# dalek-cryptography/zkp

Hardware: AMD Instinct MI355X
Metric: proofs/sec + batch-verifies/sec, CMZ13 10-attr credential, 1/2/4/8 MI355X (higher is better)
Workload: dtype u32x9 (29-bit limbs, u64 accumulate)

## Files before the change

### include/zkp_mi355x.h

```cpp
#ifndef ZKP_MI355X_H
#define ZKP_MI355X_H

#include <stddef.h>
#include <stdint.h>

#ifdef __cplusplus
extern "C" {
#endif

#define ZKP_OK 0
#define ZKP_ERR_HIP (-1)
#define ZKP_ERR_ARG (-2)
#define ZKP_ERR_NO_DEVICE (-3)
#define ZKP_ERR_OOM (-4)

#define ZKP_VARTIME 0
#define ZKP_CT 1

typedef struct zkp_ctx zkp_ctx;

int zkp_ctx_create(zkp_ctx** out, int device_id);
void zkp_ctx_destroy(zkp_ctx* ctx);
int zkp_ctx_set_stream(zkp_ctx* ctx, void* hip_stream);
int zkp_ctx_synchronize(zkp_ctx* ctx);
// ... 93 lines not shown
                                 uint8_t* d_transcripts, const uint8_t* d_table, const uint8_t* d_challenges,
                                 const uint8_t* d_responses, uint8_t* d_results);
int zkp_fused_batch_verify_dev(zkp_ctx* ctx, const zkp_fused_statement* st, uint32_t N, uint32_t strobe_pos,
                               uint8_t* d_transcripts, uint8_t* d_points, const uint8_t* d_commitments,
                               const uint8_t* d_responses, const uint8_t* d_weights16, uint8_t* d_out_point,
                               uint32_t* d_status);
int zkp_fused_verify_batchable_dev(zkp_ctx* ctx, const zkp_fused_statement* st, uint32_t N, uint32_t strobe_pos,
                                   uint8_t* d_transcripts, const uint8_t* d_table, const uint8_t* d_responses,
                                   const uint8_t* d_weights16, uint8_t* d_results);

int zkp_fused_batch_verify_many_dev(zkp_ctx* ctx, const zkp_fused_statement* st, uint32_t n_batches, uint32_t N_each, uint32_t strobe_pos,
                                    uint8_t* d_transcripts, uint8_t* d_points, const uint8_t* d_commitments, const uint8_t* d_responses,
                                    const uint8_t* d_weights16, uint8_t* d_out_points, uint32_t* d_status);

#define ZKP_JOB_SHARED_TRANSCRIPT 1u
int zkp_fused_prove_submit(zkp_ctx* ctx, const zkp_fused_statement* st, uint32_t N, uint32_t flags, const uint8_t* transcripts,
                           const uint8_t* secrets, const uint8_t* inst, uint32_t inst_stride, const uint8_t* common,
                           const uint8_t* entropy, const uint8_t* rng_seed , uint8_t* transcripts_out,
                           uint8_t* challenges, uint8_t* responses, uint8_t* commitments, int* invalid_point);
int zkp_fused_verify_compact_submit(zkp_ctx* ctx, const zkp_fused_statement* st, uint32_t N, uint32_t flags, const uint8_t* transcripts,
                                    const uint8_t* inst, uint32_t inst_stride, const uint8_t* common, const uint8_t* challenges,
                                    const uint8_t* responses, uint8_t* transcripts_out, uint8_t* results );
int zkp_fused_batch_verify_many_submit(zkp_ctx* ctx, const zkp_fused_statement* st, uint32_t n_batches, uint32_t N_each, uint32_t flags,
                                       const uint8_t* transcripts, const uint8_t* inst, uint32_t inst_stride, const uint8_t* common,
                                       const uint8_t* commitments, const uint8_t* responses, const uint8_t* weights16,
                                       uint32_t weights_stride, const uint8_t* rng_seed, uint8_t* transcripts_out, int* verdicts );
int zkp_fused_verify_batchable_submit(zkp_ctx* ctx, const zkp_fused_statement* st, uint32_t N, uint32_t flags, const uint8_t* transcripts,
                                      const uint8_t* inst, uint32_t inst_stride, const uint8_t* common, const uint8_t* commitments,
                                      const uint8_t* responses, const uint8_t* weights16 , const uint8_t* rng_seed,
                                      uint8_t* transcripts_out, uint8_t* results );
int zkp_ctx_job_wait(zkp_ctx* ctx);
int zkp_ctx_job_poll(zkp_ctx* ctx);
int zkp_ctx_job_pending(zkp_ctx* ctx);
int zkp_ctx_job_discard(zkp_ctx* ctx);
int zkp_ctx_job_timing(zkp_ctx* ctx, float ms[3]);

int zkp_host_alloc(void** out, size_t bytes);
int zkp_host_alloc_on(void** out, size_t bytes, int device);
int zkp_host_numa_node(int device);
int zkp_host_node_of(const void* p);
void zkp_host_free(void* p);
int zkp_host_register(void* p, size_t bytes);
int zkp_host_unregister(void* p);
int zkp_host_is_pinned(const void* p);

int zkp_chacha20_fill_dev(zkp_ctx* ctx, const uint8_t key[32], uint64_t nonce, uint64_t first_block, uint8_t* d_out, size_t bytes);

int zkp_decode_check(zkp_ctx* ctx, uint64_t n, const uint8_t* points , uint8_t* status ,
                     uint8_t* xyzt );

int zkp_encode_many(zkp_ctx* ctx, uint64_t n, const uint8_t* xyzt , uint8_t* out );

int zkp_from_uniform_bytes(zkp_ctx* ctx, uint64_t n, const uint8_t* in , uint8_t* out );
int zkp_from_uniform_bytes_dev(zkp_ctx* ctx, uint64_t n, const uint8_t* d_in , uint8_t* d_out );
int zkp_fused_hash_to_group(zkp_ctx* ctx, uint32_t N, uint8_t* transcripts , const char* label, uint8_t* out );
int zkp_fused_hash_to_group_ragged(zkp_ctx* ctx, uint32_t N, uint8_t* transcripts , const char* label, uint8_t* out );
int zkp_hash_from_bytes_sha512(zkp_ctx* ctx, uint64_t n, const uint8_t* msgs, const uint64_t* offsets , uint8_t* out );
int zkp_hash_from_bytes_sha512_dev(zkp_ctx* ctx, uint64_t n, const uint8_t* d_msgs, uint64_t msgs_len, const uint64_t* d_offsets ,
                                   uint8_t* d_out );

enum {
  ZKP_K_DECODE = 0,
  ZKP_K_TERMS = 1,
  ZKP_K_REDUCE = 2,
  ZKP_K_SORT = 3,
  ZKP_K_BUCKET = 4,
  ZKP_K_COMBINE = 5,
  ZKP_K_TRANSCRIPT = 6,
  ZKP_K_SCALARS = 7,
  ZKP_K_TABLES = 8,
  ZKP_K_COUNT = 9
};
int zkp_ctx_last_timing(zkp_ctx* ctx, float* kernel_ms , float* total_ms);
int zkp_ctx_last_kernels(zkp_ctx* ctx, int kind, char* buf, size_t cap);
int zkp_ctx_set_profiling(zkp_ctx* ctx, int enabled);

#ifdef ZKP_BUILD_TEST_HOOKS
int zkp_debug_quad_selftest(zkp_ctx* ctx, uint32_t n, const uint8_t* pairs , uint8_t* out );
int zkp_debug_row_selftest(zkp_ctx* ctx, uint32_t n, const uint8_t* pairs , uint8_t* out );
int zkp_debug_wave_cycles(zkp_ctx* ctx, uint64_t* out, uint32_t cap);
int zkp_debug_sha512(zkp_ctx* ctx, uint64_t n, const uint8_t* msgs, const uint64_t* offsets , uint8_t* out );
int zkp_debug_last_schedule(zkp_ctx* ctx, char* buf, size_t cap);
int zkp_debug_ragged_blocks(const uint8_t* transcripts, uint32_t N, uint32_t* idx, uint32_t* blocks, uint32_t cap);
enum { ZKP_TESTOPT_DUMMY_LAUNCHES = 1001, ZKP_TESTOPT_GENERIC_CLASSIFIER = 1002, ZKP_TESTOPT_WAVE_CYCLES = 1003 };
#endif

#ifdef __cplusplus
}
#endif
#endif
```

### zkp_amd/csrc/comb_tables.h

```cpp
#pragma once
#include "quad.h"
#include "stmt_pairs.h"

namespace zkp {

template <int TEETH>
struct comb_cfg {
  static_assert(TEETH == 4 || TEETH == 8 || TEETH == 16 || TEETH == 32, "teeth");
  static constexpr int BITS = 256 / TEETH;
  static constexpr int WINDOWS = BITS / 4;
  static constexpr int ENTRIES = 8 * TEETH + 1;
};
constexpr int comb_entries(int teeth) { return 8 * teeth + 1; }
constexpr int LADDER_ENTRIES = 8;

__device__ __forceinline__ void q_store_cached(dev_ext* dst, const qcached& c, int q) {
  uint32_t* w = reinterpret_cast<uint32_t*>(dst) + 9 * q;
#pragma unroll
  for (int i = 0; i < 9; ++i) w[i] = c.c.v[i];
}

__global__ void __launch_bounds__(256)
k_comb_slots(uint32_t n_points, const uint32_t* __restrict__ uses, uint32_t comb_min, uint32_t group_min, uint32_t max_tables,
             uint32_t* __restrict__ counter, uint32_t* __restrict__ slot_of, uint32_t* __restrict__ slot_pt, uint32_t* __restrict__ group_start,
// ... 151 lines not shown
                                              const dev_affine* __restrict__ pts, dev_ext* __restrict__ comb, uint32_t* hand) {
  using cfg = comb_cfg<TEETH>;
  const uint32_t wave = threadIdx.x >> 6, lane = threadIdx.x & 63u;
  const uint32_t ns = min(*n_slots, max_tables);
  const uint32_t slot = slot0 + lane;
  const bool have = slot < ns && !(slot_pt[slot < ns ? slot : 0u] & STMT_ABSORBED);
  dev_ext* tbl = comb + (size_t)(have ? slot : 0u) * cfg::ENTRIES;
  if (wave == 0) {
    ge_p3 base;
    ge_identity(base);
    if (have) load_affine(base, pts + slot_pt[slot]);
#pragma unroll 1
    for (int j = 0; j < TEETH; ++j) {
      uint32_t* h = hand + (j & 1) * 36 * 64 + lane;
#pragma unroll
      for (int i = 0; i < 9; ++i) { h[64 * i] = base.X.v[i]; h[64 * (9 + i)] = base.Y.v[i]; h[64 * (18 + i)] = base.Z.v[i]; h[64 * (27 + i)] = base.T.v[i]; }
      __syncthreads();
#pragma unroll 1
      for (int d = 0; d < cfg::BITS - 1; ++d) ge_double<false>(base, base);
      ge_double<true>(base, base);
    }
    if (have) {
      ge_cached c;
      ge_to_cached(c, base);
      store_comb_entry(tbl + 8 * TEETH, c);
    }
  } else {
#pragma unroll 1
    for (int j = 0; j < TEETH; ++j) {
      __syncthreads();
      const uint32_t* h = hand + (j & 1) * 36 * 64 + lane;
      ge_p3 base, m2, m3, m4, m;
#pragma unroll
      for (int i = 0; i < 9; ++i) { base.X.v[i] = h[64 * i]; base.Y.v[i] = h[64 * (9 + i)]; base.Z.v[i] = h[64 * (18 + i)]; base.T.v[i] = h[64 * (27 + i)]; }
      FE_TRACK(fe_set_ub_tight(base.X); fe_set_ub_tight(base.Y); fe_set_ub_tight(base.Z); fe_set_ub_tight(base.T));
      ge_cached c1, c;
      ge_to_cached(c1, base);
      ge_double<true>(m2, base);
      ge_add_cached(m3, m2, c1);
      ge_double<true>(m4, m2);
      if (have) {
        store_comb_entry(tbl + 8 * j + 0, c1);
        ge_to_cached(c, m2); store_comb_entry(tbl + 8 * j + 1, c);
        ge_to_cached(c, m3); store_comb_entry(tbl + 8 * j + 2, c);
        ge_to_cached(c, m4); store_comb_entry(tbl + 8 * j + 3, c);
      }
      ge_add_cached(m, m4, c1);
      if (have) { ge_to_cached(c, m); store_comb_entry(tbl + 8 * j + 4, c); }
      ge_double<true>(m, m3);
      if (have) { ge_to_cached(c, m); store_comb_entry(tbl + 8 * j + 5, c); }
      ge_add_cached(m, m, c1);
      if (have) { ge_to_cached(c, m); store_comb_entry(tbl + 8 * j + 6, c); }
      ge_double<true>(m, m4);
      if (have) { ge_to_cached(c, m); store_comb_entry(tbl + 8 * j + 7, c); }
    }
  }
}

__device__ __forceinline__ void load_comb_entry(ge_cached& c, const dev_ext* src) {
  uint32_t w[36];
  load_vec<9>(w, src);
  fe_set(c.YmX, w); fe_set(c.YpX, w + 9); fe_set(c.Z2, w + 18); fe_set(c.T2d, w + 27);
}

template <bool CT>
__device__ __forceinline__ void comb_select(ge_cached& sel, const dev_ext* __restrict__ row, uint32_t mag) {
  ge_cached_identity(sel);
  if (CT) {
#pragma unroll 1
    for (uint32_t h = 0; h < 4; ++h) {
      ge_cached c0, c1;
      load_comb_entry(c0, row + 2 * h + 0);
      load_comb_entry(c1, row + 2 * h + 1);
      ge_cached_cmov(sel, c0, (uint32_t)(mag == 2 * h + 1));
      ge_cached_cmov(sel, c1, (uint32_t)(mag == 2 * h + 2));
    }
  } else if (mag) {
    load_comb_entry(sel, row + (mag - 1));
  }
}

template <bool CT, int TEETH>
__device__ __forceinline__ void term_comb(uint32_t t, const uint8_t* __restrict__ scalars, const dev_ext* __restrict__ tbl,
                                          dev_ext* __restrict__ partial, uint32_t* ecol) {
  using cfg = comb_cfg<TEETH>;
  uint32_t s[8], e[8], top;
  load_vec<2>(s, scalars + 32 * (size_t)t);
  sc_add_pattern(e, top, s, 0x88888888u);
#pragma unroll
  for (int j = 0; j < 8; ++j) ecol[256 * j] = e[j];
  ge_p3 acc;
  ge_identity(acc);
  if (CT) {
    ge_cached n0, n1;
    load_comb_entry(n0, tbl + 0);
    load_comb_entry(n1, tbl + 1);
#pragma unroll 1
    for (int w = cfg::WINDOWS - 1; w >= 0; --w) {
      if (w != cfg::WINDOWS - 1) {
        ge_double4_flat(acc);
      }
#pragma unroll 1
      for (int j = 0; j < TEETH; ++j) {
        const int nidx = j * cfg::WINDOWS + w;
        const uint32_t nib = (ecol[256 * (nidx >> 3)] >> (4 * (nidx & 7))) & 15u;
        const uint32_t neg = (uint32_t)(nib < 8u);
        const uint32_t mag = neg ? 8u - nib : nib - 8u;
        const dev_ext* row = tbl + 8 * j;
        ge_cached sel;
        ge_cached_identity(sel);
        ge_cached_cmov(sel, n0, (uint32_t)(mag == 1));
        ge_cached_cmov(sel, n1, (uint32_t)(mag == 2));
#pragma unroll 1
        for (uint32_t h = 1; h < 4; ++h) {
          ge_cached c0, c1;
          load_comb_entry(c0, row + 2 * h + 0);
          load_comb_entry(c1, row + 2 * h + 1);
          ge_cached_cmov(sel, c0, (uint32_t)(mag == 2 * h + 1));
          ge_cached_cmov(sel, c1, (uint32_t)(mag == 2 * h + 2));
        }
        const dev_ext* next = (j + 1 < TEETH) ? row + 8 : tbl;
        load_comb_entry(n0, next + 0);
        load_comb_entry(n1, next + 1);
        ge_cached_cneg(sel, neg);
        ge_add_cached(acc, acc, sel);
      }
    }
  } else {
#pragma unroll 1
    for (int w = cfg::WINDOWS - 1; w >= 0; --w) {
      if (w != cfg::WINDOWS - 1) {
        ge_double4(acc);
      }
#pragma unroll 1
      for (int j = 0; j < TEETH; ++j) {
        const int nidx = j * cfg::WINDOWS + w;
        const uint32_t nib = (ecol[256 * (nidx >> 3)] >> (4 * (nidx & 7))) & 15u;
        const uint32_t neg = (uint32_t)(nib < 8u);
        const uint32_t mag = neg ? 8u - nib : nib - 8u;
        ge_cached sel;
        comb_select<false>(sel, tbl + 8 * j, mag);
        ge_cached_cneg(sel, neg);
        ge_add_cached(acc, acc, sel);
      }
    }
  }
  {
    ge_cached sel, c;
    ge_cached_identity(sel);
    load_comb_entry(c, tbl + 8 * TEETH);
    ge_cached_cmov(sel, c, top);
    ge_add_cached(acc, acc, sel);
  }
  store_ext(partial + t, acc);
}

__device__ __forceinline__ void ge_p3_dpp_from(ge_p3& r, const ge_p3& a, int ctrl_sel) {
  if (ctrl_sel == 0) { fe_dpp<ZKP_QP(1, 1, 3, 3)>(r.X, a.X); fe_dpp<ZKP_QP(1, 1, 3, 3)>(r.Y, a.Y); fe_dpp<ZKP_QP(1, 1, 3, 3)>(r.Z, a.Z); fe_dpp<ZKP_QP(1, 1, 3, 3)>(r.T, a.T); }
  else { fe_dpp<ZKP_QP(2, 2, 2, 2)>(r.X, a.X); fe_dpp<ZKP_QP(2, 2, 2, 2)>(r.Y, a.Y); fe_dpp<ZKP_QP(2, 2, 2, 2)>(r.Z, a.Z); fe_dpp<ZKP_QP(2, 2, 2, 2)>(r.T, a.T); }
}
template <int TEETH>
__device__ __forceinline__ void term_comb_split4(uint32_t t, uint32_t q, const uint8_t* __restrict__ scalars, const dev_ext* __restrict__ comb, uint32_t slot,
                                                 dev_ext* __restrict__ partial, uint32_t* ecol) {
  using cfg = comb_cfg<TEETH>;
  static_assert(cfg::WINDOWS == 4, "one lane of the quad per window");
  typedef __attribute__((address_space(3))) volatile uint32_t lds_word;
  lds_word* stash = (lds_word*)(ecol + 256 * 8);
  stash[0] = slot;
  stash[256] = t;
  const dev_ext* __restrict__ tbl = comb + (size_t)slot * cfg::ENTRIES;
  uint32_t s[8], e[8], top;
  load_vec<2>(s, scalars + 32 * (size_t)t);
  sc_add_pattern(e, top, s, 0x88888888u);
#pragma unroll
  for (int j = 0; j < 8; ++j) ecol[256 * j] = e[j];
  stash[512] = top;
  ge_p3 acc;
  ge_identity(acc);
  {
    ge_cached n0, n1;
    load_comb_entry(n0, tbl + 0);
    load_comb_entry(n1, tbl + 1);
#pragma unroll 1
    for (int j = 0; j < TEETH; ++j) {
      const uint32_t nidx = (uint32_t)j * cfg::WINDOWS + q;
      const uint32_t nib = (ecol[256 * (nidx >> 3)] >> (4 * (nidx & 7))) & 15u;
      const uint32_t neg = (uint32_t)(nib < 8u);
      const uint32_t mag = neg ? 8u - nib : nib - 8u;
      const dev_ext* row = tbl + 8 * j;
      ge_cached sel;
      ge_cached_identity(sel);
      ge_cached_cmov(sel, n0, (uint32_t)(mag == 1));
      ge_cached_cmov(sel, n1, (uint32_t)(mag == 2));
#pragma unroll 1
      for (uint32_t h = 1; h < 4; ++h) {
        ge_cached c0, c1;
        load_comb_entry(c0, row + 2 * h + 0);
        load_comb_entry(c1, row + 2 * h + 1);
        ge_cached_cmov(sel, c0, (uint32_t)(mag == 2 * h + 1));
        ge_cached_cmov(sel, c1, (uint32_t)(mag == 2 * h + 2));
      }
      const dev_ext* next = (j + 1 < TEETH) ? row + 8 : tbl;
      load_comb_entry(n0, next + 0);
      load_comb_entry(n1, next + 1);
      ge_cached_cneg(sel, neg);
      ge_add_cached(acc, acc, sel);
    }
  }
  {
    ge_p3 d = acc;
    ge_double4(d);
    fe_pick(acc.X, d.X, (q & 1u) != 0); fe_pick(acc.Y, d.Y, (q & 1u) != 0); fe_pick(acc.Z, d.Z, (q & 1u) != 0); fe_pick(acc.T, d.T, (q & 1u) != 0);
    ge_p3 o;
    ge_p3_dpp_from(o, acc, 0);
    ge_cached c;
    ge_to_cached(c, o);
    ge_add_cached(d, acc, c);
    fe_pick(acc.X, d.X, (q & 1u) == 0); fe_pick(acc.Y, d.Y, (q & 1u) == 0); fe_pick(acc.Z, d.Z, (q & 1u) == 0); fe_pick(acc.T, d.T, (q & 1u) == 0);
    d = acc;
    ge_double4(d);
    ge_double4(d);
    fe_pick(acc.X, d.X, q == 2u); fe_pick(acc.Y, d.Y, q == 2u); fe_pick(acc.Z, d.Z, q == 2u); fe_pick(acc.T, d.T, q == 2u);
    ge_p3_dpp_from(o, acc, 1);
    ge_to_cached(c, o);
    ge_add_cached(d, acc, c);
    fe_pick(acc.X, d.X, q == 0u); fe_pick(acc.Y, d.Y, q == 0u); fe_pick(acc.Z, d.Z, q == 0u); fe_pick(acc.T, d.T, q == 0u);
  }
  {
    ge_cached sel, c;
    ge_cached_identity(sel);
    load_comb_entry(c, comb + (size_t)stash[0] * cfg::ENTRIES + 8 * TEETH);
    ge_cached_cmov(sel, c, stash[512]);
    ge_add_cached(acc, acc, sel);
  }
  if (q == 0u) store_ext(partial + stash[256], acc);
}

constexpr int GROUP_RUNS = 3, GROUP_ROW_CHUNKS = 8 * 9, GROUP_IDENT_ROW = GROUP_RUNS * GROUP_ROW_CHUNKS, GROUP_CHUNK_ROWS = GROUP_IDENT_ROW + 9;
constexpr int GROUP_LDS_UINT4 = GROUP_CHUNK_ROWS * 16 + (256 + 16 * GROUP_RUNS) / 4;
static_assert(GROUP_MIN_USES >= 8, "a column of 16 consecutive grouped terms must span at most GROUP_RUNS points");

__device__ __forceinline__ void comb_group_block(uint32_t i0, uint32_t n_g, const uint32_t* __restrict__ list_g, const uint8_t* __restrict__ scalars,
                                                 const uint32_t* __restrict__ pidx, const uint32_t* __restrict__ slot_of,
                                                 const dev_ext* __restrict__ comb, dev_ext* __restrict__ partial, uint4* lds) {
  using cfg = comb_cfg<16>;
  constexpr uint32_t NONE = 0xffffffffu;
  const uint32_t tid = threadIdx.x, col = tid & 15u, k = tid >> 4;
  const uint32_t i = i0 + col * 16 + k;
  const bool listed = i < n_g;
  uint32_t t = 0, slot = NONE;
  if (listed) { t = list_g[i]; slot = slot_of[pidx[t]]; }
  uint32_t* slots = reinterpret_cast<uint32_t*>(lds + GROUP_CHUNK_ROWS * 16);
  uint32_t* colslot = slots + 256;
  slots[k * 16 + col] = slot;
  if (k < (uint32_t)GROUP_RUNS) colslot[col * GROUP_RUNS + k] = NONE;
  if (k < 9) {
    uint32_t w[36];
#pragma unroll
    for (int q = 0; q < 36; ++q) w[q] = (q == 0 || q == 9) ? 1u : (q == 18 ? 2u : 0u);
    uint4 v = make_uint4(0, 0, 0, 0);
#pragma unroll
    for (int q = 0; q < 9; ++q) if (k == (uint32_t)q) v = make_uint4(w[4 * q], w[4 * q + 1], w[4 * q + 2], w[4 * q + 3]);
    lds[(GROUP_IDENT_ROW + k) * 16 + col] = v;
  }
  __syncthreads();
  uint32_t run = 0;
  bool first = true;
#pragma unroll
  for (uint32_t kk = 1; kk < 16; ++kk) {
    const bool change = slots[kk * 16 + col] != slots[(kk - 1) * 16 + col];
    if (kk <= k) { run += change ? 1u : 0u; if (kk == k) first = change; }
  }
  if (first && run < (uint32_t)GROUP_RUNS) colslot[col * GROUP_RUNS + run] = slot;
  __syncthreads();
  const bool live = listed && slot != NONE && run < (uint32_t)GROUP_RUNS;
  const uint4* src[GROUP_RUNS];
  bool have[GROUP_RUNS];
#pragma unroll
  for (int r = 0; r < GROUP_RUNS; ++r) {
    const uint32_t sr = colslot[col * GROUP_RUNS + r];
    have[r] = sr != NONE;
    src[r] = reinterpret_cast<const uint4*>(comb + (size_t)(have[r] ? sr : 0u) * cfg::ENTRIES) + k;
  }
  const bool tail = k < (uint32_t)(GROUP_ROW_CHUNKS - 64);
  typedef __attribute__((address_space(1))) const void* gptr_t;
  typedef __attribute__((address_space(3))) void* lptr_t;
  const uint32_t wave = (uint32_t)__builtin_amdgcn_readfirstlane((int)(tid >> 6));
  auto issue = [&](uint32_t row) {
#pragma unroll
    for (int r = 0; r < GROUP_RUNS; ++r) {
      const uint4* p = src[r] + (size_t)row * GROUP_ROW_CHUNKS;
      uint4* d = lds + (size_t)(r * GROUP_ROW_CHUNKS + 4 * wave) * 16;
#pragma unroll
      for (int m = 0; m < 4; ++m)
        if (have[r]) __builtin_amdgcn_global_load_lds((gptr_t)(p + 16 * m), (lptr_t)(d + 16 * 16 * m), 16, 0, 0);
      if (have[r] && tail) __builtin_amdgcn_global_load_lds((gptr_t)(p + 64), (lptr_t)(d + 16 * 64), 16, 0, 0);
    }
  };
  uint32_t dlo[cfg::WINDOWS], dhi[cfg::WINDOWS], top = 0;
  {
    uint32_t sc[8], e[8];
#pragma unroll
    for (int q = 0; q < 8; ++q) sc[q] = 0;
    if (live) load_vec<2>(sc, scalars + 32 * (size_t)t);
    sc_add_pattern(e, top, sc, 0x88888888u);
#pragma unroll
    for (int w = 0; w < cfg::WINDOWS; ++w) {
      uint32_t lo = 0, hi = 0;
#pragma unroll
      for (int m = 0; m < 4; ++m) {
        lo |= (((e[m] >> (4 * w)) & 0xfu) | ((e[m] >> (12 + 4 * w)) & 0xf0u)) << (8 * m);
        hi |= (((e[m + 4] >> (4 * w)) & 0xfu) | ((e[m + 4] >> (12 + 4 * w)) & 0xf0u)) << (8 * m);
      }
      dlo[w] = lo; dhi[w] = hi;
    }
  }
  ge_p3 acc, lo;
  ge_identity(acc);
  ge_identity(lo);
  issue(0);
  auto pick = [&](uint32_t& c0, uint32_t& c1, ge_cached& sel, uint32_t& neg) {
    const uint32_t nib = c0 & 15u;
    c0 = __builtin_amdgcn_alignbit(c1, c0, 4);
    c1 >>= 4;
    neg = (uint32_t)(nib < 8u);
    const uint32_t mag = neg ? 8u - nib : nib - 8u;
    const uint32_t row = mag ? run * GROUP_ROW_CHUNKS + (mag - 1u) * 9u : (uint32_t)GROUP_IDENT_ROW;
    const uint4* ent = lds + (size_t)row * 16 + col;
    uint32_t wd[36];
#pragma unroll
    for (int q = 0; q < 9; ++q) {
      const uint4 x = ent[q * 16];
      wd[4 * q + 0] = x.x; wd[4 * q + 1] = x.y; wd[4 * q + 2] = x.z; wd[4 * q + 3] = x.w;
    }
    fe_set(sel.YmX, wd); fe_set(sel.YpX, wd + 9); fe_set(sel.Z2, wd + 18); fe_set(sel.T2d, wd + 27);
  };
#pragma unroll 1
  for (int pass = 0; pass < 2; ++pass) {
    if (live && pass) { ge_double4(acc); ge_double4(lo); }
    uint32_t alo = pass ? dlo[2] : dlo[3], ahi = pass ? dhi[2] : dhi[3];
    uint32_t blo = pass ? dlo[0] : dlo[1], bhi = pass ? dhi[0] : dhi[1];
#pragma unroll 1
    for (int j = 0; j < 16; ++j) {
      asm volatile("s_waitcnt vmcnt(0)\n\ts_barrier" ::: "memory");
      ge_cached sel;
      uint32_t neg = 0;
      if (live) {
        pick(alo, ahi, sel, neg);
        ge_cached_cneg(sel, neg);
        ge_add_cached(acc, acc, sel);
        pick(blo, bhi, sel, neg);
      }
      lds_barrier();
      if (pass == 0 || j != 15) issue((uint32_t)((j + 1) & 15));
      if (live) {
        ge_cached_cneg(sel, neg);
        ge_add_cached(lo, lo, sel);
      }
    }
  }
  if (live) {
    ge_double4(acc);
    ge_double4(acc);
    ge_cached c;
    ge_to_cached(c, lo);
    ge_add_cached(acc, acc, c);
  }
  if (live) {
    ge_cached sel, c;
    ge_cached_identity(sel);
    load_comb_entry(c, comb + (size_t)slot * cfg::ENTRIES + 8 * 16);
    ge_cached_cmov(sel, c, top);
    ge_add_cached(acc, acc, sel);
    store_ext(partial + t, acc);
  }
}

constexpr uint32_t XBAR_RUNS = 8;
constexpr uint32_t XBAR_HALF_TERMS = 31, XBAR_WAVE_TERMS = 2 * XBAR_HALF_TERMS, XBAR_BLOCK_TERMS = 4 * XBAR_WAVE_TERMS;
constexpr int XBAR_WAVE_UINT4 = 9 * 64;
constexpr int XBAR_LDS_UINT4 = 4 * XBAR_WAVE_UINT4;
static_assert(2 + (XBAR_WAVE_TERMS - 2) / GROUP_MIN_USES <= XBAR_RUNS, "a wavefront's consecutive grouped terms must span at most XBAR_RUNS points");
static_assert(2 + (XBAR_HALF_TERMS - 2) / GROUP_MIN_USES <= 4 && XBAR_HALF_TERMS <= 32,
              "the terms of one crossbar service group (a half of the wavefront) must span at most 4 points: sources 32 lanes apart never meet");

__device__ __forceinline__ void comb_group_xbar(uint32_t i0, uint32_t n_g, const uint32_t* __restrict__ list_g, const uint8_t* __restrict__ scalars,
                                                const uint32_t* __restrict__ pidx, const uint32_t* __restrict__ slot_of,
                                                const dev_ext* __restrict__ comb, dev_ext* __restrict__ partial, uint4* lds) {
  using cfg = comb_cfg<16>;
  constexpr uint32_t NONE = 0xffffffffu;
  const uint32_t tid = threadIdx.x, lane = tid & 63u;
  const uint32_t wave = (uint32_t)__builtin_amdgcn_readfirstlane((int)(tid >> 6));
  if (i0 + wave * XBAR_WAVE_TERMS >= n_g) return;
  const uint32_t hl = lane & 31u;
  const uint32_t i = i0 + wave * XBAR_WAVE_TERMS + (lane >> 5) * XBAR_HALF_TERMS + hl;
  const bool listed = hl < XBAR_HALF_TERMS && i < n_g;
  uint32_t t = 0, slot = NONE;
  if (listed) { t = list_g[i]; slot = slot_of[pidx[t]]; }
  uint32_t cur = slot;
  const uint32_t left = (uint32_t)__shfl_up((int)cur, 1);
  if (hl == 31u) cur = left;
  const uint32_t before = (uint32_t)__shfl_up((int)cur, 1);
  const bool change = lane == 0u || (listed && slot != before);
  const uint64_t cm = __ballot(change);
  const uint32_t run = (uint32_t)__popcll(cm & ((2ull << lane) - 1ull)) - 1u;
  const bool live = listed && slot != NONE && run < XBAR_RUNS;
  int first = -1;
  {
    uint64_t mm = cm;
#pragma unroll
    for (uint32_t r = 0; r < XBAR_RUNS; ++r) {
      const int f = mm ? (int)__ffsll((long long)mm) - 1 : -1;
      if ((lane >> 3) == r) first = f;
      mm &= mm - 1ull;
    }
  }
  uint32_t hslot = (uint32_t)__shfl((int)slot, first < 0 ? 0 : first);
  if (first < 0) hslot = NONE;
  const bool have = hslot != NONE;
  const uint4* hsrc = reinterpret_cast<const uint4*>(comb + (size_t)(have ? hslot : 0u) * cfg::ENTRIES + (lane & 7u));
  typedef __attribute__((address_space(1))) const void* gptr_t;
  typedef __attribute__((address_space(3))) void* lptr_t;
  uint4* wlds = lds + (size_t)wave * XBAR_WAVE_UINT4;
  const uint4* mine = wlds + lane;
  auto issue = [&](uint32_t row) {
    const uint4* p = hsrc + (size_t)row * (8 * 9);
    if (have) {
#pragma unroll
      for (int q = 0; q < 9; ++q) __builtin_amdgcn_global_load_lds((gptr_t)(p + q), (lptr_t)(wlds + 64 * q), 16, 0, 0);
    }
  };
  uint32_t dlo[cfg::WINDOWS], dhi[cfg::WINDOWS], top = 0;
  {
    uint32_t sc[8], e[8];
#pragma unroll
    for (int q = 0; q < 8; ++q) sc[q] = 0;
    if (live) load_vec<2>(sc, scalars + 32 * (size_t)t);
    sc_add_pattern(e, top, sc, 0x88888888u);
#pragma unroll
    for (int w = 0; w < cfg::WINDOWS; ++w) {
      uint32_t lo = 0, hi = 0;
#pragma unroll
      for (int m = 0; m < 4; ++m) {
        lo |= (((e[m] >> (4 * w)) & 0xfu) | ((e[m] >> (12 + 4 * w)) & 0xf0u)) << (8 * m);
        hi |= (((e[m + 4] >> (4 * w)) & 0xfu) | ((e[m + 4] >> (12 + 4 * w)) & 0xf0u)) << (8 * m);
      }
      dlo[w] = lo; dhi[w] = hi;
    }
  }
  ge_p3 acc, lo;
  ge_identity(acc);
  ge_identity(lo);
  issue(0);
  const uint32_t run8 = (run & (XBAR_RUNS - 1u)) * 8u;
  auto pick = [&](uint32_t& c0, uint32_t& c1, ge_cached& sel, uint32_t& neg) {
    const uint32_t nib = c0 & 15u;
    c0 = __builtin_amdgcn_alignbit(c1, c0, 4);
    c1 >>= 4;
    neg = (uint32_t)(nib < 8u);
    const uint32_t mag = neg ? 8u - nib : nib - 8u;
    const uint32_t nz = (uint32_t)(mag != 0u);
    const int src = (int)((run8 + mag - nz) << 2);
    uint32_t wd[36];
#pragma unroll
    for (int q = 0; q < 9; ++q) {
      const uint4 x = mine[q * 64];
      wd[4 * q + 0] = xbar_fetch(src, x.x); wd[4 * q + 1] = xbar_fetch(src, x.y);
      wd[4 * q + 2] = xbar_fetch(src, x.z); wd[4 * q + 3] = xbar_fetch(src, x.w);
    }
    const uint32_t m = 0u - nz, id = nz ^ 1u;
#pragma unroll
    for (int q = 0; q < 36; ++q) wd[q] &= m;
    wd[0] |= id; wd[9] |= id; wd[18] |= id << 1;
    fe_set(sel.YmX, wd); fe_set(sel.YpX, wd + 9); fe_set(sel.Z2, wd + 18); fe_set(sel.T2d, wd + 27);
  };
#pragma unroll 1
  for (int pass = 0; pass < 2; ++pass) {
    if (pass) { ge_double4(acc); ge_double4(lo); }
    uint32_t alo = pass ? dlo[2] : dlo[3], ahi = pass ? dhi[2] : dhi[3];
    uint32_t blo = pass ? dlo[0] : dlo[1], bhi = pass ? dhi[0] : dhi[1];
#pragma unroll 1
    for (int j = 0; j < 16; ++j) {
      asm volatile("s_waitcnt vmcnt(0)" ::: "memory");
      ge_cached sel;
      uint32_t neg = 0;
      pick(alo, ahi, sel, neg);
      ge_cached_cneg(sel, neg);
      ge_add_cached(acc, acc, sel);
      pick(blo, bhi, sel, neg);
      asm volatile("s_waitcnt lgkmcnt(0)" ::: "memory");
      if (pass == 0 || j != 15) issue((uint32_t)((j + 1) & 15));
      ge_cached_cneg(sel, neg);
      ge_add_cached(lo, lo, sel);
    }
  }
  ge_double4(acc);
  ge_double4(acc);
  {
    ge_cached c;
    ge_to_cached(c, lo);
    ge_add_cached(acc, acc, c);
  }
  if (live) {
    ge_cached sel, c;
    ge_cached_identity(sel);
    load_comb_entry(c, comb + (size_t)slot * cfg::ENTRIES + 8 * 16);
    ge_cached_cmov(sel, c, top);
    ge_add_cached(acc, acc, sel);
    store_ext(partial + t, acc);
  }
}

constexpr uint32_t LADDER_GROUP_UINT4 = 64u * LADDER_ENTRIES * 9u;
__device__ __forceinline__ void ladder_store_entry(uint4* __restrict__ g, int e, const ge_cached& c) {
  uint32_t w[36];
  fe_get(w, c.YmX); fe_get(w + 9, c.YpX); fe_get(w + 18, c.Z2); fe_get(w + 27, c.T2d);
#pragma unroll
  for (int q = 0; q < 9; ++q) g[(9 * e + q) * 64] = make_uint4(w[4 * q], w[4 * q + 1], w[4 * q + 2], w[4 * q + 3]);
}
__device__ __forceinline__ void ladder_load_entry(ge_cached& c, const uint4* __restrict__ g, uint32_t e) {
  uint32_t w[36];
#pragma unroll
  for (int q = 0; q < 9; ++q) {
    const uint4 v = g[(9u * e + (uint32_t)q) * 64u];
    w[4 * q] = v.x; w[4 * q + 1] = v.y; w[4 * q + 2] = v.z; w[4 * q + 3] = v.w;
  }
  fe_set(c.YmX, w); fe_set(c.YpX, w + 9); fe_set(c.Z2, w + 18); fe_set(c.T2d, w + 27);
}
template <bool CT>
__device__ __forceinline__ void ladder_select(ge_cached& sel, const uint4* __restrict__ g, uint32_t mag) {
  ge_cached_identity(sel);
  if (CT) {
#pragma unroll 1
    for (uint32_t h = 0; h < 4; ++h) {
      ge_cached c0, c1;
      ladder_load_entry(c0, g, 2 * h + 0);
      ladder_load_entry(c1, g, 2 * h + 1);
      ge_cached_cmov(sel, c0, (uint32_t)(mag == 2 * h + 1));
      ge_cached_cmov(sel, c1, (uint32_t)(mag == 2 * h + 2));
    }
  } else if (mag) {
    ladder_load_entry(sel, g, mag - 1);
  }
}

template <bool CT>
__device__ __forceinline__ void term_ladder16(uint32_t t, const uint8_t* __restrict__ scalars, const dev_affine* __restrict__ pt,
                                              uint4* __restrict__ tbl , dev_ext* __restrict__ partial, uint32_t* ecol) {
  uint32_t s[8], e[8], top;
  load_vec<2>(s, scalars + 32 * (size_t)t);
  sc_add_pattern(e, top, s, 0x88888888u);
#pragma unroll
  for (int j = 0; j < 8; ++j) ecol[256 * j] = e[j];
  ge_p3 acc;
  {
    ge_p3 P, m2, m3, m4, m;
    ge_cached c1, c;
    load_affine(P, pt);
    ge_to_cached(c1, P);
    ladder_store_entry(tbl, 0, c1);
    ge_double<true>(m2, P);
    ge_to_cached(c, m2); ladder_store_entry(tbl, 1, c);
    ge_add_cached(m3, m2, c1);
    ge_to_cached(c, m3); ladder_store_entry(tbl, 2, c);
    ge_double<true>(m4, m2);
    ge_to_cached(c, m4); ladder_store_entry(tbl, 3, c);
    ge_add_cached(m, m4, c1);
    ge_to_cached(c, m); ladder_store_entry(tbl, 4, c);
    ge_double<true>(m, m3);
    ge_to_cached(c, m); ladder_store_entry(tbl, 5, c);
    ge_add_cached(m, m, c1);
    ge_to_cached(c, m); ladder_store_entry(tbl, 6, c);
    ge_double<true>(m, m4);
    ge_to_cached(c, m); ladder_store_entry(tbl, 7, c);
    ge_cached sel;
    ge_cached_identity(sel);
    ge_cached_cmov(sel, c1, top);
    ge_identity(acc);
    ge_add_cached(acc, acc, sel);
  }
#pragma unroll 1
  for (int j = 7; j >= 0; --j) {
    uint32_t cur = ecol[256 * j];
#pragma unroll 1
    for (int k = 0; k < 8; ++k) {
      ge_double4(acc);
      const uint32_t nib = cur >> 28;
      cur <<= 4;
      const uint32_t neg = (uint32_t)(nib < 8u);
      const uint32_t mag = neg ? 8u - nib : nib - 8u;
      ge_cached sel;
      ladder_select<CT>(sel, tbl, mag);
      ge_cached_cneg(sel, neg);
      ge_add_cached(acc, acc, sel);
    }
  }
  store_ext(partial + t, acc);
}

__global__ void __launch_bounds__(256, 2)
k_rider_tables(const uint32_t* __restrict__ n_slots, uint32_t max_tables, const uint32_t* __restrict__ slot_pt, const dev_affine* __restrict__ pts,
               dev_ext* __restrict__ comb) {
  __shared__ uint32_t stage[4][36][64];
  __shared__ uint32_t live[4][64];
  const uint32_t wave = threadIdx.x >> 6, lane = threadIdx.x & 63u;
  const uint32_t slot = blockIdx.x * blockDim.x + threadIdx.x, ns = min(*n_slots, max_tables);
  const uint32_t pi = slot < ns ? slot_pt[slot] : 0u;
  const bool have = slot < ns && (pi & STMT_ABSORBED);
  live[wave][lane] = have ? 1u : 0u;
  if (!__ballot(have)) return;
  ge_p3 P, m;
  ge_identity(P);
  if (have) load_affine(P, pts + (pi & ~STMT_ABSORBED));
  dev_ext* tbl0 = comb + (size_t)(slot - lane) * comb_cfg<16>::ENTRIES;
  ge_cached c1, c;
  ge_to_cached(c1, P);
  c = c1;
  m = P;
#pragma unroll 1
  for (int k = 0; k < 128; ++k) {
    if (k) {
      ge_add_cached(m, m, c1);
      ge_to_cached(c, m);
    }
    store_entries_staged(stage[wave], live[wave], lane, tbl0, comb_cfg<16>::ENTRIES, (uint32_t)k, c);
  }
}

__device__ __forceinline__ void ladder_build8(uint4* __restrict__ tbl, ge_cached& c1, const dev_affine* __restrict__ pt) {
  ge_p3 P, m2, m3, m4, m;
  ge_cached c;
  load_affine(P, pt);
  ge_to_cached(c1, P);
  ladder_store_entry(tbl, 0, c1);
  ge_double<true>(m2, P);
  ge_to_cached(c, m2); ladder_store_entry(tbl, 1, c);
  ge_add_cached(m3, m2, c1);
  ge_to_cached(c, m3); ladder_store_entry(tbl, 2, c);
  ge_double<true>(m4, m2);
  ge_to_cached(c, m4); ladder_store_entry(tbl, 3, c);
  ge_add_cached(m, m4, c1);
  ge_to_cached(c, m); ladder_store_entry(tbl, 4, c);
  ge_double<true>(m, m3);
  ge_to_cached(c, m); ladder_store_entry(tbl, 5, c);
  ge_add_cached(m, m, c1);
  ge_to_cached(c, m); ladder_store_entry(tbl, 6, c);
  ge_double<true>(m, m4);
  ge_to_cached(c, m); ladder_store_entry(tbl, 7, c);
}
__device__ __forceinline__ void term_ladder16_joint(uint32_t t, uint32_t t2, const uint8_t* __restrict__ scalars, const dev_affine* __restrict__ pt,
                                                    const dev_affine* __restrict__ pt2, uint4* __restrict__ tbl, uint4* __restrict__ tbl2,
                                                    const dev_ext* __restrict__ rider, dev_ext* __restrict__ partial, uint32_t* ecol) {
  uint32_t top, top2;
  {
    uint32_t s[8], e[8];
    load_vec<2>(s, scalars + 32 * (size_t)t);
    sc_add_pattern(e, top, s, 0x88888888u);
#pragma unroll
    for (int j = 0; j < 8; ++j) ecol[256 * j] = e[j];
    load_vec<2>(s, scalars + 32 * (size_t)t2);
    sc_add_pattern(e, top2, s, rider ? 0x80808080u : 0x88888888u);
#pragma unroll
// ... 55 lines not shown
```

### zkp_amd/csrc/fe_constants.h

```cpp
#pragma once
#include "fe25519.h"
namespace zkp {
static constexpr fe_const FE_D = {{0x135978a3u, 0x0f5a6e50u, 0x10762addu, 0x00149a82u, 0x1e898007u, 0x003cbbbcu, 0x19ce331du, 0x1dc56dffu, 0x0052036cu}};
static constexpr fe_const FE_D2 = {{0x06b2f159u, 0x1eb4dca1u, 0x00ec55bau, 0x00293505u, 0x1d13000eu, 0x00797779u, 0x139c663au, 0x1b8adbffu, 0x002406d9u}};
static constexpr fe_const FE_SQRT_M1 = {{0x0a0ea0b0u, 0x0770d93au, 0x0bf91e31u, 0x06300d5au, 0x1d7a72f4u, 0x004c9efdu, 0x1c2cad34u, 0x1009f83bu, 0x002b8324u}};
static constexpr fe_const FE_INVSQRT_A_MINUS_D = {{0x005d40eau, 0x0e47ed54u, 0x105cafa6u, 0x1e2c2eb4u, 0x1d8409d2u, 0x1dc8ff00u, 0x12885b09u, 0x00b9f5ffu, 0x00786c89u}};
static constexpr fe_const FE_SQRT_AD_MINUS_ONE = {{0x097b2e1bu, 0x14bfb502u, 0x1e152f5fu, 0x1b1c1836u, 0x1d1fdaf9u, 0x1e6498fau, 0x02b03cf3u, 0x17e57069u, 0x00376931u}};
static constexpr fe_const FE_ONE_MINUS_D_SQ = {{0x145fc176u, 0x13e04e0cu, 0x178d43f8u, 0x0342719au, 0x0dfe42c8u, 0x15eedf38u, 0x035e6652u, 0x1516567cu, 0x00029072u}};
static constexpr fe_const FE_D_MINUS_ONE_SQ = {{0x04ed4d20u, 0x0d6ad552u, 0x0786664cu, 0x1c945960u, 0x14eebd29u, 0x0997a94du, 0x09053373u, 0x0f5ecd84u, 0x005968b3u}};
struct fe_words { uint32_t w[8]; };
static constexpr fe_words FE_W_ONE = {{0x00000001u, 0x00000000u, 0x00000000u, 0x00000000u, 0x00000000u, 0x00000000u, 0x00000000u, 0x00000000u}};
static constexpr fe_words FE_W_MINUS_ONE = {{0xffffffecu, 0xffffffffu, 0xffffffffu, 0xffffffffu, 0xffffffffu, 0xffffffffu, 0xffffffffu, 0x7fffffffu}};
static constexpr fe_words FE_W_MINUS_SQRT_M1 = {{0xb5f15f3du, 0x3b11e4d8u, 0x52d01b87u, 0xd0bce7f9u, 0xc2042858u, 0xd4b2ff66u, 0xb03e20f4u, 0x547cdb7fu}};
}
```

### zkp_amd/csrc/fused_flows.h

```cpp
#pragma once
#include "merlin_prog.h"
#include "transcript_kernels.h"

namespace zkp {

__global__ void __launch_bounds__(256)
k_wide_reduce(uint32_t n, const uint8_t* __restrict__ wide, uint8_t* __restrict__ out) {
  const uint32_t i = blockIdx.x * blockDim.x + threadIdx.x;
  if (i >= n) return;
  sc lo, hi, r;
  load_vec<2>(lo.v, wide + 64 * (size_t)i);
  load_vec<2>(hi.v, wide + 64 * (size_t)i + 32);
  sc_from_wide(r, lo, hi);
  store_vec<2>(out + 32 * (size_t)i, r.v);
}

__global__ void __launch_bounds__(256)
k_neg_reduce(uint32_t n, const uint8_t* in, uint8_t* out) {
  const uint32_t i = blockIdx.x * blockDim.x + threadIdx.x;
  if (i >= n) return;
  sc a, r;
  load_vec<2>(a.v, in + 32 * (size_t)i);
  sc_reduce(r, a);
  sc_neg(r, r);
// ... 204 lines not shown
  for (int i = 0; i < 9; ++i) {
    const int bit = 29 * i, wi = bit >> 5, sh = bit & 31;
    w[wi] |= t[i] << sh;
    if (sh > 3 && wi < 7) w[wi + 1] |= t[i] >> (32 - sh);
  }
}
__device__ __forceinline__ void fe_unpack256(fe& r, const uint32_t w[8]) {
#pragma unroll
  for (int i = 0; i < 9; ++i) {
    const int bit = 29 * i, wi = bit >> 5, sh = bit & 31;
    uint32_t x = w[wi] >> sh;
    if (sh > 3 && wi < 7) x |= w[wi + 1] << (32 - sh);
    r.v[i] = i == 8 ? x : (x & FE_M29);
  }
  FE_TRACK(fe_set_ub_tight(r));
}
__device__ __forceinline__ void store_straus_entry(straus_entry* dst, const ge_cached& c) {
  uint32_t w[32];
  fe_pack256(w, c.YpX); fe_pack256(w + 8, c.YmX); fe_pack256(w + 16, c.Z2); fe_pack256(w + 24, c.T2d);
  store_vec<8>(dst, w);
}
__device__ __forceinline__ void load_straus_entry(ge_cached& c, const straus_entry* src) {
  uint32_t w[32];
  load_vec<8>(w, src);
  fe_unpack256(c.YpX, w); fe_unpack256(c.YmX, w + 8); fe_unpack256(c.Z2, w + 16); fe_unpack256(c.T2d, w + 24);
}
__global__ void __launch_bounds__(256, 2)
k_straus_tables(uint32_t n_points, const dev_affine* __restrict__ pts, straus_entry* __restrict__ tab) {
  const uint32_t p = blockIdx.x * blockDim.x + threadIdx.x;
  if (p >= n_points) return;
  ge_p3 P, m2, m3, m4, m;
  ge_cached c1, c;
  load_affine(P, pts + p);
  straus_entry* t = tab + (size_t)p * 8;
  ge_to_cached(c1, P);
  store_straus_entry(t + 0, c1);
  ge_double<true>(m2, P);
  ge_to_cached(c, m2); store_straus_entry(t + 1, c);
  ge_add_cached(m3, m2, c1);
  ge_to_cached(c, m3); store_straus_entry(t + 2, c);
  ge_double<true>(m4, m2);
  ge_to_cached(c, m4); store_straus_entry(t + 3, c);
  ge_add_cached(m, m4, c1);
  ge_to_cached(c, m); store_straus_entry(t + 4, c);
  ge_double<true>(m, m3);
  ge_to_cached(c, m); store_straus_entry(t + 5, c);
  ge_add_cached(m, m, c1);
  ge_to_cached(c, m); store_straus_entry(t + 6, c);
  ge_double<true>(m, m4);
  ge_to_cached(c, m); store_straus_entry(t + 7, c);
}
__global__ void __launch_bounds__(256, 2)
k_straus_each(uint32_t N, uint32_t K, uint32_t L, uint32_t ns, uint32_t ni, uint32_t nc, const uint8_t* __restrict__ scalars ,
              const straus_entry* __restrict__ tab, uint32_t* __restrict__ digits, dev_ext* __restrict__ spart) {
  extern __shared__ uint32_t straus_lds[];
  uint32_t* col = straus_lds + threadIdx.x;
  const uint32_t g = blockIdx.x * blockDim.x + threadIdx.x;
  if (g >= N * L) return;
  const uint32_t j = g / L, l = g - j * L, np = ns + ni;
  const size_t base = (size_t)j * K;
  auto table_of = [&](uint32_t i) -> const straus_entry* {
    const size_t p = i < ns ? i : (i < np ? (size_t)ns + (size_t)(i - ns) * N + j : (size_t)ns + (size_t)ni * N + (size_t)j * nc + (i - np));
    return tab + p * 8;
  };
  ge_p3 acc;
  ge_identity(acc);
  bool started = false;
  uint64_t flipmask = 0;
  uint32_t oo = 0;
  for (uint32_t i = l; i < K; i += L, ++oo) {
    uint32_t sw[8], e[8], top;
    load_vec<2>(sw, scalars + 32 * (base + i));
    const uint32_t flip = sc_fold_sign(sw);
    sc_add_pattern(e, top, sw, 0x88888888u);
    uint32_t* d = digits + 9 * (base + i);
#pragma unroll
    for (int w = 0; w < 8; ++w) d[w] = e[w];
    d[8] = flip;
    flipmask |= (uint64_t)flip << oo;
    if (top) {
      ge_cached q;
      load_straus_entry(q, table_of(i));
      ge_cached_cneg(q, flip);
      ge_add_cached(acc, acc, q);
      started = true;
    }
  }
  ge_cached qn;
  uint32_t magn = 0, negn = 0;
  auto fetch = [&](uint32_t i, uint32_t o, int k) {
    const uint32_t nib = (col[256 * o] >> (4 * k)) & 15u;
    const uint32_t neg = (uint32_t)(nib < 8u);
    magn = neg ? 8u - nib : nib - 8u;
    negn = neg ^ (uint32_t)((flipmask >> o) & 1u);
    if (magn) load_straus_entry(qn, table_of(i) + (magn - 1));
  };
#pragma unroll 1
  for (int w = 7; w >= 0; --w) {
    uint32_t o = 0;
    for (uint32_t i = l; i < K; i += L, ++o) col[256 * o] = digits[9 * (base + i) + w];
#pragma unroll 1
    for (int k = 7; k >= 0; --k) {
      fetch(l, 0, k);
      if (started) ge_double4(acc);
      o = 0;
#pragma unroll 1
      for (uint32_t i = l; i < K; i += L, ++o) {
        ge_cached q = qn;
        const uint32_t mag = magn, neg = negn;
        if (i + L < K) fetch(i + L, o + 1, k);
        if (mag) {
          ge_cached_cneg(q, neg);
          ge_add_cached(acc, acc, q);
          started = true;
        }
      }
    }
  }
  store_ext(spart + g, acc);
}
__global__ void __launch_bounds__(256)
k_straus_recode(uint32_t NK, const uint8_t* __restrict__ scalars, uint32_t* __restrict__ digits) {
  const uint32_t g = blockIdx.x * blockDim.x + threadIdx.x;
  if (g >= NK) return;
  uint32_t sw[8], e[8], top;
  load_vec<2>(sw, scalars + 32 * (size_t)g);
  const uint32_t flip = sc_fold_sign(sw);
  sc_add_pattern(e, top, sw, 0x88888888u);
  uint32_t* d = digits + 9 * (size_t)g;
#pragma unroll
  for (int w = 0; w < 8; ++w) d[w] = e[w];
  d[8] = flip | (top << 1);
}
__global__ void __launch_bounds__(256, 2)
k_straus_each_win(uint32_t N, uint32_t K, uint32_t P, uint32_t ns, uint32_t ni, uint32_t nc, const straus_entry* __restrict__ tab,
                  const uint32_t* __restrict__ digits, dev_ext* __restrict__ spart) {
  extern __shared__ uint32_t straus_lds[];
  uint32_t* col = straus_lds + threadIdx.x;
  const uint32_t g = blockIdx.x * blockDim.x + threadIdx.x;
  if (g >= N * P) return;
  const uint32_t j = g / P, p = g - j * P, np = ns + ni, Wp = 64u / P;
  const uint32_t* dj = digits + 9 * (size_t)j * K;
  auto table_of = [&](uint32_t i) -> const straus_entry* {
    const size_t t = i < ns ? i : (i < np ? (size_t)ns + (size_t)(i - ns) * N + j : (size_t)ns + (size_t)ni * N + (size_t)j * nc + (i - np));
    return tab + t * 8;
  };
  ge_p3 acc;
  ge_identity(acc);
  bool started = false;
  uint64_t flipmask = 0;
  for (uint32_t i = 0; i < K; ++i) {
    const uint32_t f = dj[9 * i + 8];
    flipmask |= (uint64_t)(f & 1u) << i;
    if ((f >> 1) && p == P - 1) {
      ge_cached q;
      load_straus_entry(q, table_of(i));
      ge_cached_cneg(q, f & 1u);
      ge_add_cached(acc, acc, q);
      started = true;
    }
  }
  ge_cached qn;
  uint32_t magn = 0, negn = 0;
  auto fetch = [&](uint32_t i, int k) {
    const uint32_t nib = (col[256 * i] >> (4 * k)) & 15u;
    const uint32_t neg = (uint32_t)(nib < 8u);
    magn = neg ? 8u - nib : nib - 8u;
    negn = neg ^ (uint32_t)((flipmask >> i) & 1u);
    if (magn) load_straus_entry(qn, table_of(i) + (magn - 1));
  };
  const int w_hi = (int)(Wp * (p + 1)) - 1, w_lo = (int)(Wp * p);
#pragma unroll 1
  for (int w = w_hi; w >= w_lo; --w) {
    const int k = w & 7;
    if (k == 7 || w == w_hi)
      for (uint32_t i = 0; i < K; ++i) col[256 * i] = dj[9 * i + (w >> 3)];
    fetch(0, k);
    if (started) ge_double4(acc);
#pragma unroll 1
    for (uint32_t i = 0; i < K; ++i) {
      ge_cached q = qn;
      const uint32_t mag = magn, neg = negn;
      if (i + 1 < K) fetch(i + 1, k);
      if (mag) {
        ge_cached_cneg(q, neg);
        ge_add_cached(acc, acc, q);
        started = true;
      }
    }
  }
  store_ext(spart + g, acc);
}
__global__ void __launch_bounds__(256)
k_straus_combine_quad(uint32_t N, uint32_t P, const dev_ext* __restrict__ spart, dev_ext* __restrict__ out) {
  const uint32_t gt = blockIdx.x * blockDim.x + threadIdx.x, j = gt >> 2;
  const int q = (int)(gt & 3u);
  if (j >= N) return;
  const dev_ext* s = spart + (size_t)j * P;
  const uint32_t dbl = 4u * (64u / P);
  qpt acc;
  q_load_ext(acc, s + (P - 1), q);
#pragma unroll 1
  for (int p = (int)P - 2; p >= 0; --p) {
#pragma unroll 1
    for (uint32_t d = 0; d < dbl; ++d) q_double(acc, acc, q);
    qpt t;
    q_load_ext(t, s + p, q);
    q_add(acc, acc, t, q);
  }
  q_store_ext(out + j, acc, q);
}
__global__ void __launch_bounds__(256, 2)
k_straus_finish(uint32_t N, uint32_t K, uint32_t L, const uint32_t* __restrict__ pidx, const dev_affine* __restrict__ pts, const dev_ext* __restrict__ spart,
                uint8_t* __restrict__ out, uint8_t* __restrict__ status8) {
  const uint32_t j = blockIdx.x * blockDim.x + threadIdx.x;
  if (j >= N) return;
  ge_p3 acc;
  load_ext(acc, spart + (size_t)j * L);
  for (uint32_t l = 1; l < L; ++l) {
    ge_p3 q;
    load_ext(q, spart + (size_t)j * L + l);
    ge_add_p3(acc, acc, q);
  }
  uint32_t bad = 0;
  for (uint32_t i = 0; i < K; ++i) bad |= pts[pidx[(size_t)j * K + i]].valid ^ 1u;
  uint32_t w[8];
#pragma unroll
  for (int k = 0; k < 8; ++k) w[k] = 0;
  if (!bad) w[0] = (fe_iszero(acc.X) | fe_iszero(acc.Y)) ^ 1u;
  store_vec<2>(out + 32 * (size_t)j, w);
  status8[j] = (uint8_t)bad;
}

__global__ void __launch_bounds__(256)
k_batch_after_transcript(uint32_t N, uint32_t N_each, uint32_t nc, uint32_t m, const uint32_t* __restrict__ failed, uint32_t* __restrict__ any, uint32_t any_stride,
                         uint32_t any_bit, const uint8_t* __restrict__ wchal, uint8_t* __restrict__ minus_c, const uint8_t* __restrict__ coms,
                         uint8_t* __restrict__ rows, const uint8_t* __restrict__ responses) {
  const size_t g = (size_t)blockIdx.x * blockDim.x + threadIdx.x;
  if (g < N) {
    if (failed[g]) atomicOr(any + (g / N_each) * any_stride, any_bit);
    sc lo, hi, r;
    load_vec<2>(lo.v, wchal + 64 * g);
    load_vec<2>(hi.v, wchal + 64 * g + 32);
    sc_from_wide(r, lo, hi);
    sc_neg(r, r);
    store_vec<2>(minus_c + 32 * g, r.v);
  }
  if (coms && g < (size_t)N * nc) {
    const size_t j = g / nc, k = g % nc;
    uint32_t w[8];
    load_vec<2>(w, coms + 32 * g);
    store_vec<2>(rows + 32 * (k * N + j), w);
  }
  if (g < (size_t)N * m) {
    uint32_t w[8];
    load_vec<2>(w, responses + 32 * g);
    if (sc_not_canonical(w)) atomicOr(any + ((g / m) / N_each) * any_stride, any_bit);
  }
}

__global__ void k_any_nonzero(uint32_t n, const uint32_t* __restrict__ flags, uint32_t* __restrict__ any) {
  const uint32_t i = blockIdx.x * blockDim.x + threadIdx.x;
  if (i < n && flags[i]) *any = 1;
}

}

namespace {
using namespace zkp;
// ... 468 lines not shown
  c->prof_suspended = false;
  c->stream = main;
  HIP_TRY(hipEventRecord(c->ev_join, c->side_stream));
  return ZKP_OK;
}
int side_join(zkp_ctx* c, bool overlap) {
  if (side_forks(c, overlap)) HIP_TRY(hipStreamWaitEvent(c->stream, c->ev_join, 0));
  return ZKP_OK;
}

struct ws_view {
  char* base;
  uint8_t* u8(size_t o) const { return reinterpret_cast<uint8_t*>(base + o); }
  uint32_t* u32(size_t o) const { return reinterpret_cast<uint32_t*>(base + o); }
};

struct prove_inter { size_t saved, failed, wide, blind, off, sc, pidx, wchal, img, end; };
prove_inter prove_carve(const fused_plan& pl, size_t start) {
  const size_t N = pl.N, m = pl.s.m, nc = pl.s.nc, T = pl.T1;
  carve cv;
  cv.off = start;
  prove_inter o;
  o.saved = cv.take(N * 25 * 8);
  o.failed = cv.take(N * 4 + 4);
  o.wide = cv.take(N * m * 64 + 64);
  o.blind = cv.take(N * m * 32 + 32);
  o.off = cv.take((N * nc + 1) * 4);
  o.sc = cv.take(N * T * 32 + 32);
  o.pidx = cv.take(N * T * 4 + 4);
  o.wchal = cv.take(N * 64 + 64);
  o.img = cv.take(pl.img_bytes);
  o.end = cv.off;
  return o;
}
terms_cfg prove_terms_cfg(const zkp_ctx* c, const fused_plan& pl, bool throughput) {
  return cfg_from_terms(pl.tpt.data(), pl.T1, pl.s.ns, pl.s.np, pl.N, c->ct_comb_min(throughput, (size_t)pl.N * pl.T1));
}
int prove_core(zkp_ctx* c, const fused_plan& pl, const prove_inter& o, size_t ws_bound, uint8_t* d_ts, const uint8_t* d_sec, const uint8_t* d_tbl,
               const uint8_t* d_ent, uint8_t* d_chal, uint8_t* d_resp, uint8_t* d_coms, uint8_t* d_st8, bool overlap, bool throughput,
               const std::function<int()>* late_inputs = nullptr, const std::function<int()>* early_outputs = nullptr, bool late_early = false) {
  const uint32_t N = pl.N, m = pl.s.m, nc = pl.s.nc, T = pl.T1, n_points = pl.s.ns + pl.s.ni * N;
  const ws_view w{static_cast<char*>(c->ws)};
  tr_bufs hb{};
  hb.src[SRC_TABLE] = d_tbl; hb.src[SRC_SECRETS] = d_sec; hb.src[SRC_ENTROPY] = d_ent; hb.src[SRC_COMS] = d_coms;
  hb.dst[DST_WIDE] = w.u8(o.wide); hb.dst[DST_CHAL] = w.u8(o.wchal);
  uint64_t* d_saved = reinterpret_cast<uint64_t*>(w.base + o.saved);
  prof_begin(c);
  const size_t lanes = std::max<size_t>((size_t)N * T, (size_t)N * nc) + 1;
  terms_cfg tk = prove_terms_cfg(c, pl, throughput);
  if (o.end + terms_path_ws(n_points, N * T, N * nc, tk) > ws_bound)
    return fail(ZKP_ERR_ARG, "internal: prove_core's term path does not fit the workspace its caller sized");
  tk.throughput = throughput;
  if (pl.d_order) { tk.map.N = N; tk.map.nc = nc; tk.map.order = pl.d_order; }
  tk.stmt.toff = pl.d_tarr; tk.stmt.tpt = pl.d_tarr + nc + 1 + T; tk.stmt.N = N; tk.stmt.T = T; tk.stmt.nc = nc; tk.stmt.ns = pl.s.ns; tk.stmt.np = pl.s.np;
  tk.stmt.off = w.u32(o.off); tk.stmt.pidx = w.u32(o.pidx); tk.stmt.on = c->stmt_classify;
#ifdef ZKP_BUILD_TEST_HOOKS
  for (int q = 0; q < c->debug_dummy_launches; ++q) hipLaunchKernelGGL(k_noop, dim3(1), dim3(64), 0, c->stream, (uint32_t*)nullptr);
#endif
  uint64_t* d_img = pl.img_bytes ? reinterpret_cast<uint64_t*>(w.base + o.img) : nullptr;
  offer_program(c, pl.a, N, hb, d_ts, d_saved, w.u32(o.failed), throughput, overlap, d_img);
  {
    hipStream_t main;
    int rc = side_begin(c, &main, overlap);
    if (rc) { c->pending_tr.offered = c->pending_tr.active = false; return rc; }
    if (late_inputs && late_early) {
      hipStream_t cur = c->stream;
      c->stream = main;
      rc = (*late_inputs)();
      c->stream = cur;
      late_inputs = nullptr;
      if (rc) { (void)side_end(c, main, overlap); c->pending_tr.offered = c->pending_tr.active = false; return rc; }
    }
    if (!(nc && stmt_classify_applies(tk, N * T)))
      hipLaunchKernelGGL(k_stmt_index, grid1(lanes, 256), dim3(256), 0, c->stream, N, T, nc, pl.s.ns, pl.d_tarr, pl.d_tarr + nc + 1 + T, w.u32(o.off), w.u32(o.pidx));
    if (nc) rc = msm_terms_path(c, N * nc, w.u32(o.off), nullptr, w.u32(o.pidx), d_tbl, n_points, N * T, ZKP_CT, d_coms, d_st8, nullptr, o.end, false, PH_POINTS, tk);
    const int rc2 = side_end(c, main, overlap);
    if (rc || rc2) { c->pending_tr.offered = c->pending_tr.active = false; return rc ? rc : rc2; }
  }
  if (late_inputs) { const int rc = (*late_inputs)(); if (rc) return rc; }
  run_program_pending(c, pl.a, N, hb, d_ts, d_saved, w.u32(o.failed), throughput, d_img);
  prof_mark(c, ZKP_K_TRANSCRIPT);

  tk.prehalved = nc && terms_batched_encode(c, N * T, N * nc, tk.throughput);
  if (m && std::max(m, T) <= 256) {
    const uint32_t P = 256 / std::max(m, T);
    hipLaunchKernelGGL(k_blind_scalars, dim3((N + P - 1) / P), dim3(256), 0, c->stream, N, T, m, P, pl.d_tarr + nc + 1, w.u8(o.wide), w.u8(o.blind), w.u8(o.sc),
                       tk.prehalved ? 1u : 0u);
  } else if (m) {
    hipLaunchKernelGGL(k_wide_reduce, grid1((size_t)N * m, 256), dim3(256), 0, c->stream, N * m, w.u8(o.wide), w.u8(o.blind));
    if (T) hipLaunchKernelGGL(k_stmt_scalars, grid1((size_t)N * T, 256), dim3(256), 0, c->stream, N, T, m, pl.d_tarr + nc + 1, w.u8(o.blind), (const uint8_t*)nullptr, w.u8(o.sc),
                              tk.prehalved ? 1u : 0u);
  }
  prof_mark(c, ZKP_K_SCALARS);
  HIP_TRY(hipGetLastError());
  {
    int rc = side_join(c, overlap);
    if (rc) return rc;
    if (nc) rc = msm_terms_path(c, N * nc, w.u32(o.off), w.u8(o.sc), w.u32(o.pidx), d_tbl, n_points, N * T, ZKP_CT, d_coms, d_st8, nullptr, o.end, false, PH_SCALARS, tk);
    if (rc) return rc;
    if (early_outputs) { rc = (*early_outputs)(); if (rc) return rc; }
  }
  run_program(c, pl.b, N, hb, d_ts, d_saved, w.u32(o.failed), throughput, d_img);
  prof_mark(c, ZKP_K_TRANSCRIPT);
  if (m && m <= 256) {
    const uint32_t P = 256 / m;
    hipLaunchKernelGGL(k_responses, dim3((N + P - 1) / P), dim3(256), 0, c->stream, N, m, P, d_sec, w.u8(o.wchal), d_chal, w.u8(o.blind), d_resp);
  } else {
    hipLaunchKernelGGL(k_wide_reduce, grid1(N, 256), dim3(256), 0, c->stream, N, w.u8(o.wchal), d_chal);
    if (m) hipLaunchKernelGGL(k_responses_wide, grid1((size_t)N * m, 256), dim3(256), 0, c->stream, N, m, d_sec, d_chal, w.u8(o.blind), d_resp);
  }
  prof_mark(c, ZKP_K_SCALARS);
  HIP_TRY(hipGetLastError());
  return ZKP_OK;
}

struct verify_inter { size_t failed, mc, off, sc, pidx, coms, st8, wchal, chal, img, end; };
verify_inter verify_carve(const fused_plan& pl, size_t start) {
  const size_t N = pl.N, nc = pl.s.nc, T1 = pl.T1;
  carve cv;
  cv.off = start;
  verify_inter o;
  o.failed = cv.take(N * 4 + 4);
  o.mc = cv.take(N * 32 + 32);
  o.off = cv.take((N * nc + 1) * 4);
  o.sc = cv.take(N * T1 * 32 + 32);
  o.pidx = cv.take(N * T1 * 4 + 4);
  o.coms = cv.take(N * nc * 32 + 32);
  o.st8 = cv.take(N * nc + 4);
  o.wchal = cv.take(N * 64 + 64);
  o.chal = cv.take(N * 32 + 32);
  o.img = cv.take(pl.img_bytes);
  o.end = cv.off;
  return o;
}
constexpr uint32_t kRiderLatencyProofs = 16384;
inline bool verify_riders(uint32_t N, bool throughput) { return throughput || N >= kRiderLatencyProofs; }
terms_cfg verify_terms_cfg(const zkp_ctx* c, const fused_plan& pl, bool riders = true) {
  const uint32_t N = pl.N, nc = pl.s.nc, T1 = pl.T1;
  terms_cfg tk = cfg_from_terms(pl.tpt.data(), T1, pl.s.ns, pl.s.np, N, 2);
  tk.stmt.toff = pl.d_tarr; tk.stmt.tpt = pl.d_tarr + nc + 1 + T1; tk.stmt.N = N; tk.stmt.T = T1; tk.stmt.nc = nc; tk.stmt.ns = pl.s.ns; tk.stmt.np = pl.s.np;
  tk.stmt.on = c->stmt_classify;
  if (c->joint_ladder && pl.d_pair && stmt_classify_applies(tk, N * T1)) {
    riders = riders && c->rider_tables;
    const terms_cfg paired = cfg_from_terms(pl.tpt.data(), T1, pl.s.ns, pl.s.np, N, 2, pl.pair.data(), riders);
    tk.max_tables = paired.max_tables; tk.max_ladder = paired.max_ladder; tk.teeth = paired.teeth;
    tk.stmt.pair = pl.d_pair;
    tk.rider_tables = riders;
  }
  return tk;
}
int verify_core(zkp_ctx* c, const fused_plan& pl, const verify_inter& o, size_t ws_bound, uint8_t* d_ts, const uint8_t* d_tbl, const uint8_t* d_claim,
                const uint8_t* d_resp, uint8_t* d_results, bool overlap, bool throughput, const std::function<int()>* late_inputs = nullptr, bool late_early = false) {
  const uint32_t N = pl.N, m = pl.s.m, nc = pl.s.nc, T1 = pl.T1, n_points = pl.s.ns + pl.s.ni * N;
  terms_cfg tk = verify_terms_cfg(c, pl, verify_riders(N, throughput));
  if (o.end + terms_path_ws(n_points, N * T1, N * nc, tk) > ws_bound)
    return fail(ZKP_ERR_ARG, "internal: verify_core's term path does not fit the workspace its caller sized");
  const ws_view w{static_cast<char*>(c->ws)};
  tr_bufs hb{};
  hb.src[SRC_TABLE] = d_tbl; hb.src[SRC_COMS] = w.u8(o.coms);
  hb.dst[DST_CHAL] = w.u8(o.wchal);
  HIP_TRY(hipMemsetAsync(w.base + o.failed, 0, (size_t)N * 4, c->stream));
  prof_begin(c);
  const size_t lanes = std::max<size_t>((size_t)N * T1, (size_t)N * nc) + 1;
  tk.throughput = throughput;
  if (pl.d_order) { tk.map.N = N; tk.map.nc = nc; tk.map.order = pl.d_order; }
  tk.stmt.off = w.u32(o.off); tk.stmt.pidx = w.u32(o.pidx);
// ... 504 lines not shown
```

### zkp_amd/csrc/ge25519.h

```cpp
#pragma once
#include "fe25519.h"
#include "fe_constants.h"

namespace zkp {

struct ge_p3 { fe X, Y, Z, T; };
struct ge_cached { fe YpX, YmX, Z2, T2d; };
struct ge_niels { fe ypx, ymx, xy2d; };

ZKP_HD void ge_identity(ge_p3& r) {
  fe_0(r.X);
  fe_1(r.Y);
  fe_1(r.Z);
  fe_0(r.T);
}
ZKP_HD void ge_cached_identity(ge_cached& r) {
  fe_1(r.YpX);
  fe_1(r.YmX);
  fe_0(r.Z2);
  r.Z2.v[0] = 2;
  FE_TRACK(fe_set_ub_exact(r.Z2));
  fe_0(r.T2d);
}
ZKP_HD void ge_niels_identity(ge_niels& r) {
// ... 19 lines not shown
  fe_add(t, p.Y, p.X);
  fe_carry(r.ypx, t);
  fe_sub(t, p.Y, p.X);
  fe_carry(r.ymx, t);
  fe_from_const(d2, FE_D2);
  fe_mul(r.xy2d, p.T, d2);
}

ZKP_HD void ge_add_cached(ge_p3& r, const ge_p3& p, const ge_cached& q) {
  fe a, b, c, d, e, f, g, h, t;
  fe_sub(t, p.Y, p.X);
  fe_mul(a, t, q.YmX);
  fe_add(t, p.Y, p.X);
  fe_mul(b, t, q.YpX);
  fe_mul(c, p.T, q.T2d);
  fe_mul(d, p.Z, q.Z2);
  fe_sub(e, b, a);
  fe_sub(t, d, c);
  fe_carry(f, t);
  fe_add(g, d, c);
  fe_add(h, b, a);
  fe_mul(r.X, e, f);
  fe_mul(r.Y, g, h);
  fe_mul(r.Z, f, g);
  fe_mul(r.T, e, h);
}

ZKP_HD void ge_sub_cached(ge_p3& r, const ge_p3& p, const ge_cached& q) {
  fe a, b, c, d, e, f, g, h, t;
  fe_sub(t, p.Y, p.X);
  fe_mul(a, t, q.YpX);
  fe_add(t, p.Y, p.X);
  fe_mul(b, t, q.YmX);
  fe_mul(c, p.T, q.T2d);
  fe_mul(d, p.Z, q.Z2);
  fe_sub(e, b, a);
  fe_add(t, d, c);
  fe_carry(f, t);
  fe_sub(g, d, c);
  fe_add(h, b, a);
  fe_mul(r.X, e, f);
  fe_mul(r.Y, g, h);
  fe_mul(r.Z, f, g);
  fe_mul(r.T, e, h);
}

ZKP_HD void ge_madd(ge_p3& r, const ge_p3& p, const ge_niels& q) {
  fe a, b, c, d, e, f, g, h, t;
  fe_sub(t, p.Y, p.X);
  fe_mul(a, t, q.ymx);
  fe_add(t, p.Y, p.X);
  fe_mul(b, t, q.ypx);
  fe_mul(c, p.T, q.xy2d);
  fe_add(d, p.Z, p.Z);
  fe_sub(e, b, a);
  fe_sub(t, d, c);
  fe_carry(f, t);
  fe_add(g, d, c);
  fe_add(h, b, a);
  fe_mul(r.X, e, f);
  fe_mul(r.Y, g, h);
  fe_mul(r.Z, f, g);
  fe_mul(r.T, e, h);
}

ZKP_HD void ge_msub(ge_p3& r, const ge_p3& p, const ge_niels& q) {
  fe a, b, c, d, e, f, g, h, t;
  fe_sub(t, p.Y, p.X);
  fe_mul(a, t, q.ypx);
  fe_add(t, p.Y, p.X);
  fe_mul(b, t, q.ymx);
  fe_mul(c, p.T, q.xy2d);
  fe_add(d, p.Z, p.Z);
  fe_sub(e, b, a);
  fe_add(t, d, c);
  fe_carry(f, t);
  fe_sub(t, d, c);
  fe_carry(g, t);
  fe_add(h, b, a);
  fe_mul(r.X, e, f);
  fe_mul(r.Y, g, h);
  fe_mul(r.Z, f, g);
  fe_mul(r.T, e, h);
}

template <bool WITH_T = true>
ZKP_HD void ge_double(ge_p3& r, const ge_p3& p) {
  fe xx, yy, zz2, xpy, e, g, f, h, t;
  fe_sq(xx, p.X);
  fe_sq(yy, p.Y);
  fe_sq(t, p.Z);
  fe_add(zz2, t, t);
  fe_add(t, p.X, p.Y);
  fe_sq(xpy, t);
  fe_add(h, yy, xx);
  fe_sub(g, yy, xx);
  fe_sub4(t, xpy, h);
  fe_carry(e, t);
  fe_sub4(t, zz2, g);
  fe_carry(f, t);
  fe_mul(r.X, e, f);
  fe_mul(r.Y, h, g);
  fe_mul(r.Z, g, f);
  if (WITH_T) fe_mul(r.T, e, h);
}

ZKP_HD void ge_double4(ge_p3& acc) {
#pragma unroll 1
  for (int k = 0; k < 3; ++k) ge_double<false>(acc, acc);
  ge_double<true>(acc, acc);
}

ZKP_HD void ge_double4_flat(ge_p3& acc) {
  ge_double<false>(acc, acc);
  ge_double<false>(acc, acc);
  ge_double<false>(acc, acc);
  ge_double<true>(acc, acc);
}

ZKP_HD void ge_neg(ge_p3& r, const ge_p3& p) {
  fe t;
  fe_neg(t, p.X);
  fe_carry(r.X, t);
  r.Y = p.Y;
  r.Z = p.Z;
  fe_neg(t, p.T);
  fe_carry(r.T, t);
}

ZKP_HD void ge_cached_cneg(ge_cached& q, uint32_t flag) {
  fe_cswap(q.YpX, q.YmX, flag);
  fe n;
  fe_neg(n, q.T2d);
  fe_cmov(q.T2d, n, flag);
}
ZKP_HD void ge_niels_cneg(ge_niels& q, uint32_t flag) {
  fe_cswap(q.ypx, q.ymx, flag);
  fe n;
  fe_neg(n, q.xy2d);
  fe_cmov(q.xy2d, n, flag);
}
ZKP_HD void ge_cached_cmov(ge_cached& r, const ge_cached& q, uint32_t flag) {
  fe_cmov(r.YpX, q.YpX, flag);
  fe_cmov(r.YmX, q.YmX, flag);
  fe_cmov(r.Z2, q.Z2, flag);
  fe_cmov(r.T2d, q.T2d, flag);
}

ZKP_HD uint32_t fe_words_eq(const uint32_t w[8], const fe_words& c) {
  uint32_t x = 0;
#pragma unroll
  for (int i = 0; i < 8; ++i) x |= w[i] ^ c.w[i];
  return (uint32_t)(x == 0);
}

ZKP_HD uint32_t fe_invsqrt(fe& r, const fe& v) {
  fe t, v3, c;
  fe_sq(t, v);
  fe_mul(v3, t, v);
  fe_sq(t, v3);
  fe_mul(t, t, v);
  fe_pow22523(t, t);
  fe_mul(r, t, v3);
  fe_sq(t, r);
  fe_mul(t, t, v);
  uint32_t cw[8];
// ... 246 lines not shown
```

### zkp_amd/csrc/hot_tables.h

```cpp
#pragma once
#include "dev_layout.h"
#include "stmt_pairs.h"

namespace zkp {

#ifndef ZKP_HOT_W
#define ZKP_HOT_W 7
#endif
constexpr int HOT_W = ZKP_HOT_W;
constexpr int HOT_WINDOWS = (257 + HOT_W - 1) / HOT_W;
constexpr int HOT_HALF = 1 << (HOT_W - 1);
constexpr int HOT_ROW = HOT_HALF + 1;
constexpr int HOT_SLOTS = 64;
constexpr int HOT_CLASSES = HOT_SLOTS + 3;
constexpr int CLASS_COMB = HOT_SLOTS, CLASS_LADDER = HOT_SLOTS + 1, CLASS_GROUP = HOT_SLOTS + 2;
constexpr uint32_t GROUP_MIN_USES = 10;
constexpr size_t HOT_SLOT_NIELS = (size_t)HOT_WINDOWS * HOT_ROW;
constexpr int HOT_ROW_CHUNKS = HOT_ROW * (int)(sizeof(dev_niels) / 16);
constexpr int HOT_COPIES = 16;
static_assert(HOT_W >= 6 && HOT_W <= 7 && HOT_W * HOT_WINDOWS >= 258, "fixed-base window shape");
constexpr bool HOT_LDS_ROWS = HOT_ROW_CHUNKS <= 256;

constexpr uint32_t hot_pattern_word(int i) {
  uint32_t v = 0;
// ... 307 lines not shown
    const int32_t c = cls_p[p];
    const bool cold = c >= HOT_SLOTS;
    const uint64_t u = cold ? (p < ns ? (uint64_t)cnt[p] * N : cnt[p]) : 0;
    uses[g] = (uint32_t)(u > 0xffffffffull ? 0xffffffffull : u);
    uint32_t slot = NONE;
    if (rank_p[p] != NONE) slot = p < ns ? rank_p[p] : sh[0] + rank_p[p] * N + j;
    if (slot != NONE && slot >= max_tables) slot = NONE;
    const bool rider = slot != NONE && stmt_rider(rider_ok, p, ns, cnt[p], acnt[p]);
    slot_of[g] = rider ? (slot | STMT_ABSORBED) : slot;
    if (slot != NONE) slot_pt[slot] = rider ? ((uint32_t)g | STMT_ABSORBED) : (uint32_t)g;
  }
  if (g < (size_t)N * sj.nc) sj.off[g] = (uint32_t)((g / sj.nc) * T + sj.toff[g % sj.nc]);
  if (g == 0) sj.off[(size_t)N * sj.nc] = N * T;
  if (g < n_terms) {
    const uint32_t j = (uint32_t)(g / T), k = (uint32_t)(g % T);
    const uint32_t p = sj.tpt[k];
    sj.pidx[g] = p < ns ? p : ns + (p - ns) * N + j;
    if (stmt_absorbed(sj.pair, k)) return;
    const int32_t c = cls_p[p];
    size_t pos;
    if (c == CLASS_GROUP) {
      pos = p < ns ? (size_t)goff_p[p] * N + (size_t)j * cnt[p] + pos_k[k]
                   : (size_t)sh[2] * N + (size_t)j * sh[3] + goff_p[p] + pos_k[k];
    } else if (c == CLASS_LADDER) {
      pos = (pos_k[k] & STMT_ABSORBED) ? (size_t)j * sh[4] + (pos_k[k] & ~STMT_ABSORBED) : (size_t)N * sh[4] + (size_t)j * (cc[c] - sh[4]) + pos_k[k];
    } else {
      pos = (size_t)j * cc[c] + pos_k[k];
    }
    list[cstart[c] + pos] = (uint32_t)g;
  }
}

__device__ __forceinline__ void lds_barrier() { asm volatile("s_waitcnt lgkmcnt(0)\n\ts_barrier" ::: "memory"); }

template <bool SCAN = false>
__device__ __forceinline__ void fixed_base_block(ge_p3& acc, uint32_t e[9], bool live, const uint4* __restrict__ rows, uint4* rep) {
  const uint32_t tid = threadIdx.x, copy = tid & (HOT_COPIES - 1);
  const bool loader = tid < (uint32_t)HOT_ROW_CHUNKS;
  uint4 v = make_uint4(0, 0, 0, 0);
  if (loader) v = rows[tid];
#pragma unroll 1
  for (int w = 0; w < HOT_WINDOWS; ++w) {
    lds_barrier();
    if (loader) {
#pragma unroll
      for (uint32_t i = 0; i < (uint32_t)HOT_COPIES; ++i) rep[tid * HOT_COPIES + ((i + tid) & (HOT_COPIES - 1))] = v;
      if (w + 1 < HOT_WINDOWS) v = rows[(size_t)(w + 1) * HOT_ROW_CHUNKS + tid];
    }
    lds_barrier();
    if (live) {
      uint32_t mag, neg;
      hot_next_digit(e, mag, neg);
      uint32_t wd[28];
      if constexpr (SCAN) {
        const uint4* ent = rep + copy;
#pragma unroll
        for (int i = 0; i < 7; ++i) {
          const uint4 x = ent[i * HOT_COPIES];
          wd[4 * i + 0] = x.x; wd[4 * i + 1] = x.y; wd[4 * i + 2] = x.z; wd[4 * i + 3] = x.w;
        }
#pragma unroll 1
        for (uint32_t k = 1; k <= (uint32_t)HOT_HALF; ++k) {
          const uint4* ek = rep + (size_t)k * (sizeof(dev_niels) / 16) * HOT_COPIES + copy;
          const uint32_t m = 0u - (uint32_t)(k == mag);
#pragma unroll
          for (int i = 0; i < 7; ++i) {
            uint4 x = ek[i * HOT_COPIES];
            asm volatile("" : "+v"(x.x), "+v"(x.y), "+v"(x.z), "+v"(x.w));
            wd[4 * i + 0] = (wd[4 * i + 0] & ~m) | (x.x & m); wd[4 * i + 1] = (wd[4 * i + 1] & ~m) | (x.y & m);
            wd[4 * i + 2] = (wd[4 * i + 2] & ~m) | (x.z & m); wd[4 * i + 3] = (wd[4 * i + 3] & ~m) | (x.w & m);
          }
        }
      } else {
        const uint4* ent = rep + (size_t)mag * (sizeof(dev_niels) / 16) * HOT_COPIES + copy;
#pragma unroll
        for (int i = 0; i < 7; ++i) {
          const uint4 x = ent[i * HOT_COPIES];
          wd[4 * i + 0] = x.x; wd[4 * i + 1] = x.y; wd[4 * i + 2] = x.z; wd[4 * i + 3] = x.w;
        }
      }
      ge_niels q;
      fe_set(q.ypx, wd); fe_set(q.ymx, wd + 9); fe_set(q.xy2d, wd + 18);
      ge_niels_cneg(q, neg);
      ge_madd(acc, acc, q);
    }
  }
}

__device__ __forceinline__ uint32_t xbar_fetch(int src_lane_x4, uint32_t v) { return (uint32_t)__builtin_amdgcn_ds_bpermute(src_lane_x4, (int)v); }

__device__ __forceinline__ void fixed_base_xbar(ge_p3& acc, uint32_t e[9], const uint4* __restrict__ rows) {
  const uint32_t lane = threadIdx.x & 63u;
  constexpr int SETS = HOT_HALF / 32;
  static_assert(HOT_HALF == 32 * SETS && SETS >= 1 && SETS <= 2, "the crossbar walk holds sets of 32 entries");
  const uint4* my = rows + (size_t)(1u + (lane & 31u)) * 7u + (lane >> 5) * 4u;
  const uint32_t last = lane < 32u ? 3u : 2u;
  uint4 r[SETS][4];
#pragma unroll
  for (int s = 0; s < SETS; ++s)
#pragma unroll
    for (int q = 0; q < 4; ++q) r[s][q] = my[(size_t)s * 32 * 7 + (q < 3 ? (uint32_t)q : last)];
#pragma unroll 1
  for (int w = 0; w < HOT_WINDOWS; ++w) {
    uint32_t mag, neg;
    hot_next_digit(e, mag, neg);
    const uint32_t nz = (uint32_t)(mag != 0u);
    const uint32_t m1 = mag - nz;
    const int src = (int)((m1 & 31u) << 2);
    uint32_t wd[28];
#pragma unroll
    for (int s = 0; s < SETS; ++s) {
      uint32_t t[28];
#pragma unroll
      for (int q = 0; q < 4; ++q) {
        t[4 * q + 0] = xbar_fetch(src, r[s][q].x); t[4 * q + 1] = xbar_fetch(src, r[s][q].y);
        t[4 * q + 2] = xbar_fetch(src, r[s][q].z); t[4 * q + 3] = xbar_fetch(src, r[s][q].w);
      }
#pragma unroll
      for (int q = 0; q < 3; ++q) {
        t[16 + 4 * q + 0] = xbar_fetch(src + 128, r[s][q].x); t[16 + 4 * q + 1] = xbar_fetch(src + 128, r[s][q].y);
        t[16 + 4 * q + 2] = xbar_fetch(src + 128, r[s][q].z);
        if (q < 2) t[16 + 4 * q + 3] = xbar_fetch(src + 128, r[s][q].w);
      }
      if (s == 0) {
#pragma unroll
        for (int i = 0; i < 27; ++i) wd[i] = t[i];
      } else {
        const bool hi = m1 >= 32u;
#pragma unroll
        for (int i = 0; i < 27; ++i) wd[i] = hi ? t[i] : wd[i];
      }
    }
    if (w + 1 < HOT_WINDOWS) {
      const uint4* nx = my + (size_t)(w + 1) * HOT_ROW_CHUNKS;
#pragma unroll
      for (int s = 0; s < SETS; ++s)
#pragma unroll
        for (int q = 0; q < 4; ++q) r[s][q] = nx[(size_t)s * 32 * 7 + (q < 3 ? (uint32_t)q : last)];
    }
    const uint32_t m = 0u - nz;
#pragma unroll
    for (int i = 0; i < 27; ++i) wd[i] &= m;
    wd[0] |= nz ^ 1u;
    wd[9] |= nz ^ 1u;
    ge_niels q;
    fe_set(q.ypx, wd); fe_set(q.ymx, wd + 9); fe_set(q.xy2d, wd + 18);
    ge_niels_cneg(q, neg);
    ge_madd(acc, acc, q);
  }
}

}
```

### zkp_amd/csrc/zkp_kernels.hip

```cpp
#include <hip/hip_runtime.h>
#include <sys/syscall.h>
#include <unistd.h>
#include <cctype>
#include <cstdio>
#include <cstring>
#include <algorithm>
#include <atomic>
#include <functional>
#include <map>
#include <memory>
#include <mutex>
#include <set>
#include <string>
#include <vector>
#include "../../include/zkp_mi355x.h"
#include "dev_layout.h"

using namespace zkp;

__device__ __forceinline__ void sc_add_pattern(uint32_t e[8], uint32_t& top, const uint32_t s[8], uint32_t pattern) {
  uint64_t c = 0;
#pragma unroll
  for (int i = 0; i < 8; ++i) {
    c += (uint64_t)s[i] + pattern;
// ... 18 lines not shown
#include "transcript_kernels.h"
#include "sha512.h"

__global__ void __launch_bounds__(256, 2)
k_decode_affine(uint32_t n, const uint8_t* __restrict__ enc, dev_affine* __restrict__ out, const uint32_t* __restrict__ only) {
  const uint32_t i = blockIdx.x * blockDim.x + threadIdx.x;
  if (i >= n) return;
  if (only && !only[i]) { out[i].valid = 1; return; }
  uint32_t w[8];
  load_vec<2>(w, enc + 32 * (size_t)i);
  ge_p3 p;
  const uint32_t ok = ristretto_decode(p, w);
  store_affine(out + i, p, ok);
}

__device__ __forceinline__ void term_generic(uint32_t t, const uint8_t* __restrict__ scalars, const uint32_t* __restrict__ pidx,
                                             uint32_t n_points, const dev_affine* __restrict__ pts, dev_ext* __restrict__ partial) {
  uint32_t s[8], e[8], top;
  load_vec<2>(s, scalars + 32 * (size_t)t);
  sc_add_pattern(e, top, s, 0xAAAAAAAAu);
  ge_p3 P, P2, acc;
  const uint32_t pi = pidx[t];
  load_affine(P, pts + (pi < n_points ? pi : 0u));
  ge_cached c1, c2;
  ge_to_cached(c1, P);
  ge_double<true>(P2, P);
  ge_to_cached(c2, P2);
  ge_identity(acc);
  fe_cmov(acc.X, P.X, top);
  fe_cmov(acc.Y, P.Y, top);
  fe_cmov(acc.T, P.T, top);
#pragma unroll 1
  for (int j = 7; j >= 0; --j) {
    uint32_t cur = sel8(e, j);
#pragma unroll 1
    for (int k = 0; k < 16; ++k) {
      const uint32_t d = cur >> 30;
      cur <<= 2;
      ge_double<false>(acc, acc);
      ge_double<true>(acc, acc);
      const uint32_t neg = (uint32_t)(d < 2);
      const uint32_t mag = neg ? 2u - d : d - 2u;
      ge_cached sel;
      ge_cached_identity(sel);
      ge_cached_cmov(sel, c1, (uint32_t)(mag == 1));
      ge_cached_cmov(sel, c2, (uint32_t)(mag == 2));
      ge_cached_cneg(sel, neg);
      ge_add_cached(acc, acc, sel);
    }
  }
  store_ext(partial + t, acc);
}

__global__ void __launch_bounds__(256, 2)
k_terms_r4(uint32_t n_terms, const uint8_t* __restrict__ scalars, const uint32_t* __restrict__ pidx,
           uint32_t n_points, const dev_affine* __restrict__ pts, dev_ext* __restrict__ partial) {
  const uint32_t t = blockIdx.x * blockDim.x + threadIdx.x;
  if (t < n_terms) term_generic(t, scalars, pidx, n_points, pts, partial);
}

#ifdef ZKP_BUILD_TEST_HOOKS
__device__ uint64_t* g_wave_cycles = nullptr;
__device__ uint32_t g_wave_cycles_cap = 0;
#define ZKP_WAVE_T0 const uint64_t wave_t0_ = __builtin_readcyclecounter();
#define ZKP_WAVE_T1(cls) do { const uint64_t dt_ = __builtin_readcyclecounter() - wave_t0_; const uint32_t wi_ = blockIdx.x * 4 + (threadIdx.x >> 6); \
  if (g_wave_cycles && (threadIdx.x & 63u) == 0 && wi_ < g_wave_cycles_cap) g_wave_cycles[wi_] = ((uint64_t)(cls) << 56) | (dt_ & 0x00ffffffffffffffull); } while (0)
#else
#define ZKP_WAVE_T0
#define ZKP_WAVE_T1(cls)
#endif

enum : int { LOOKUP_XBAR = 0, LOOKUP_SCAN = 1, LOOKUP_LDS = 2 };
template <int LOOKUP>
constexpr int terms_lds_uint4() {
  if (LOOKUP == LOOKUP_XBAR) return XBAR_LDS_UINT4 > 512 ? XBAR_LDS_UINT4 : 512;
  return HOT_ROW_CHUNKS * HOT_COPIES > GROUP_LDS_UINT4 ? HOT_ROW_CHUNKS * HOT_COPIES : GROUP_LDS_UINT4;
}
template <bool CT, int TEETH, bool LADDER, int LOOKUP = LOOKUP_XBAR, bool SPLIT = false>
__global__ void __launch_bounds__(256, 2)
k_terms_split(const uint8_t* __restrict__ scalars, const uint32_t* __restrict__ pidx, uint32_t n_points,
              const dev_ext* __restrict__ comb, const uint32_t* __restrict__ slot_of, const uint32_t* __restrict__ class_start,
              const uint32_t* __restrict__ blk_start, const uint32_t* __restrict__ list, const dev_niels* __restrict__ tables,
              const dev_affine* __restrict__ pts, dev_ext* __restrict__ ladder_rw, uint32_t max_ladder, dev_ext* __restrict__ partial,
              uint32_t ladder_stride, const uint32_t* __restrict__ pair, uint32_t stmt_T) {
  static_assert(LOOKUP == LOOKUP_XBAR || HOT_LDS_ROWS, "7-bit fixed-base windows exist on the crossbar only");
  __shared__ uint4 hot_lds[terms_lds_uint4<LOOKUP>()];
  uint32_t* ecol = reinterpret_cast<uint32_t*>(hot_lds) + threadIdx.x;
  const uint32_t n_hot = class_start[CLASS_COMB], n_comb = class_start[CLASS_LADDER] - n_hot;
  const uint32_t n_ladder = LADDER ? class_start[CLASS_GROUP] - class_start[CLASS_LADDER] : 0u;
  const uint32_t n_group = (CT && TEETH == 16) ? class_start[HOT_CLASSES] - class_start[CLASS_GROUP] : 0u;
  const uint32_t ladder_blocks = (n_ladder + blockDim.x - 1) / blockDim.x;
  const uint32_t comb_lanes = SPLIT ? 4u * n_comb : n_comb;
  const uint32_t comb_blocks = (comb_lanes + blockDim.x - 1) / blockDim.x;
  const uint32_t group_terms = LOOKUP == LOOKUP_XBAR ? XBAR_BLOCK_TERMS : 256u;
  const uint32_t group_blocks = (n_group + group_terms - 1) / group_terms;
  uint32_t vb = blockIdx.x;
  if (LADDER && ladder_stride > 1) {
    const uint32_t q = blockIdx.x / ladder_stride, r = blockIdx.x - q * ladder_stride;
    if (r == 0 && q < ladder_blocks) vb = q;
    else vb = ladder_blocks + blockIdx.x - min((blockIdx.x + ladder_stride - 1) / ladder_stride, ladder_blocks);
  }
  ZKP_WAVE_T0
  if (LADDER && vb < ladder_blocks) {
    if constexpr (LADDER) {
      const uint32_t i = vb * blockDim.x + threadIdx.x;
      if (i < n_ladder && i < max_ladder) {
        const uint32_t t = list[n_hot + n_comb + i];
        const uint32_t pi = pidx[t];
        uint4* tbl = reinterpret_cast<uint4*>(ladder_rw) + (size_t)(i >> 6) * LADDER_GROUP_UINT4 + (i & 63u);
        bool joint = false;
        static_assert(CT || terms_lds_uint4<LOOKUP>() >= 1024, "variable-time ladder blocks need LDS for two recoded scalars");
        if constexpr (!CT && terms_lds_uint4<LOOKUP>() >= 1024) {
          const uint32_t k2 = pair ? pair[t % stmt_T] : STMT_UNPAIRED;
          if (k2 != STMT_UNPAIRED) {
            const uint32_t t2 = t - t % stmt_T + k2, i2 = i + ((max_ladder + 63u) & ~63u), pi2 = pidx[t2];
            const uint32_t s2 = slot_of[pi2];
            const dev_ext* rider = (s2 != 0xffffffffu && (s2 & STMT_ABSORBED)) ? comb + (size_t)(s2 & ~STMT_ABSORBED) * comb_cfg<16>::ENTRIES : nullptr;
            term_ladder16_joint(t, t2, scalars, pts + pi, pts + pi2, tbl, reinterpret_cast<uint4*>(ladder_rw) + (size_t)(i2 >> 6) * LADDER_GROUP_UINT4 + (i2 & 63u), rider, partial, ecol);
            joint = true;
          }
        }
        if (!joint) term_ladder16<CT>(t, scalars, pts + pi, tbl, partial, ecol);
      }
    }
    ZKP_WAVE_T1(1);
  } else if (vb < ladder_blocks + comb_blocks) {
    const uint32_t i = (vb - ladder_blocks) * blockDim.x + threadIdx.x;
    if constexpr (SPLIT) {
      {
        const uint32_t ti = i >> 2;
        if (ti < n_comb) {
          const uint32_t t = list[n_hot + ti];
          const uint32_t pi = pidx[t];
          if (pi < n_points) {
            const uint32_t slot = slot_of[pi];
            if (slot != 0xffffffffu) term_comb_split4<TEETH>(t, i & 3u, scalars, comb, slot, partial, ecol);
          }
        }
        ZKP_WAVE_T1(2);
        return;
      }
    }
    if (i < n_comb) {
      const uint32_t t = list[n_hot + i];
      const uint32_t pi = pidx[t];
      if (pi < n_points) {
        const uint32_t slot = slot_of[pi];
        if (slot != 0xffffffffu) term_comb<CT, TEETH>(t, scalars, comb + (size_t)slot * comb_cfg<TEETH>::ENTRIES, partial, ecol);
      }
    }
    ZKP_WAVE_T1(2);
  } else if (vb < ladder_blocks + comb_blocks + group_blocks) {
    if constexpr (CT && TEETH == 16) {
      if constexpr (LOOKUP == LOOKUP_XBAR)
        comb_group_xbar((vb - ladder_blocks - comb_blocks) * XBAR_BLOCK_TERMS, n_group, list + class_start[CLASS_GROUP], scalars, pidx, slot_of, comb, partial, hot_lds);
      else
        comb_group_block((vb - ladder_blocks - comb_blocks) * 256u, n_group, list + class_start[CLASS_GROUP], scalars, pidx, slot_of, comb, partial, hot_lds);
    }
    ZKP_WAVE_T1(3);
  } else {
    const uint32_t hb = vb - ladder_blocks - comb_blocks - group_blocks;
    if (hb >= blk_start[HOT_SLOTS]) return;
    uint32_t c = 0;
    while (blk_start[c + 1] <= hb) ++c;
    const uint4* src = reinterpret_cast<const uint4*>(tables + (size_t)c * HOT_SLOT_NIELS);
    const uint32_t i = (hb - blk_start[c]) * 256 + threadIdx.x;
    const bool live = i < class_start[c + 1] - class_start[c];
    const uint32_t t = live ? list[class_start[c] + i] : 0u;
    uint32_t s[8], e[9];
    ge_p3 acc;
    ge_identity(acc);
    if constexpr (LOOKUP == LOOKUP_XBAR) {
      if (hb * 256u + (threadIdx.x & ~63u) - blk_start[c] * 256u >= class_start[c + 1] - class_start[c]) return;
#pragma unroll
      for (int q = 0; q < 8; ++q) s[q] = 0;
      if (live) load_vec<2>(s, scalars + 32 * (size_t)t);
      hot_recode(e, s);
      fixed_base_xbar(acc, e, src);
    } else {
      if (live) {
        load_vec<2>(s, scalars + 32 * (size_t)t);
        hot_recode(e, s);
      }
      fixed_base_block<LOOKUP == LOOKUP_SCAN>(acc, e, live, src, hot_lds);
    }
    if (live) store_ext(partial + t, acc);
    ZKP_WAVE_T1(4);
  }
}

struct msm_map {
  uint32_t N = 0, nc = 0;
  const uint32_t* order = nullptr;
};
__device__ __forceinline__ uint32_t msm_of_lane(const msm_map& m, uint32_t p) {
  if (!m.order) return p;
  const uint32_t q = p / m.N;
  return (p - q * m.N) * m.nc + m.order[q];
}

template <typename STATUS_T>
__global__ void __launch_bounds__(256, 2)
k_reduce_encode(uint32_t n_msm, const uint32_t* __restrict__ off, const uint32_t* __restrict__ pidx,
                uint32_t n_points, const dev_affine* __restrict__ pts, const dev_ext* __restrict__ partial,
                uint8_t* __restrict__ out, STATUS_T* __restrict__ status, const msm_map map) {
  const uint32_t lane = blockIdx.x * blockDim.x + threadIdx.x;
  if (lane >= n_msm) return;
  const uint32_t i = msm_of_lane(map, lane);
  const uint32_t b = off[i], e = off[i + 1];
  ge_p3 acc;
  ge_identity(acc);
  uint32_t bad = 0;
#pragma unroll 1
  for (uint32_t t = b; t < e; ++t) {
    ge_p3 q;
    load_ext(q, partial + t);
    ge_add_p3(acc, acc, q);
    const uint32_t pi = pidx[t];
    bad |= pi < n_points ? (pts[pi].valid ^ 1u) : 1u;
  }
  uint32_t w[8];
  ristretto_encode(w, acc);
  if (bad) {
#pragma unroll
    for (int k = 0; k < 8; ++k) w[k] = 0;
  }
  store_vec<2>(out + 32 * (size_t)i, w);
  status[i] = (STATUS_T)bad;
}

__global__ void __launch_bounds__(256)
k_halve_scalars(uint32_t n, const uint8_t* __restrict__ in, uint8_t* __restrict__ out) {
  const uint32_t i = blockIdx.x * blockDim.x + threadIdx.x;
  if (i >= n) return;
  sc a, r;
  load_vec<2>(a.v, in + 32 * (size_t)i);
  sc_halve(r, a);
  store_vec<2>(out + 32 * (size_t)i, r.v);
}

constexpr int ENC_BLOCK = 256;
struct enc_tree { uint32_t node[2 * ENC_BLOCK][9]; };
__device__ __forceinline__ void tree_get(fe& r, const enc_tree& t, int n) {
#pragma unroll
  for (int i = 0; i < 9; ++i) r.v[i] = t.node[n][i];
  FE_TRACK(fe_set_ub_tight(r));
}
__device__ __forceinline__ void tree_put(enc_tree& t, int n, const fe& a) {
#pragma unroll
  for (int i = 0; i < 9; ++i) t.node[n][i] = a.v[i];
}
__device__ __forceinline__ void tree_up(enc_tree& t, int tid) {
  for (int w = ENC_BLOCK / 2; w >= 1; w >>= 1) {
    if (tid < w) {
      fe a, b, c;
      tree_get(a, t, 2 * (w + tid));
      tree_get(b, t, 2 * (w + tid) + 1);
      fe_mul(c, a, b);
      tree_put(t, w + tid, c);
    }
    __syncthreads();
  }
}
__device__ __forceinline__ void tree_down(enc_tree& t, int tid) {
  for (int w = 1; w <= ENC_BLOCK / 2; w <<= 1) {
    if (tid < w) {
      fe p, a, b, ia, ib;
      tree_get(p, t, w + tid);
      tree_get(a, t, 2 * (w + tid));
      tree_get(b, t, 2 * (w + tid) + 1);
      fe_mul(ia, p, b);
      fe_mul(ib, p, a);
      tree_put(t, 2 * (w + tid), ia);
      tree_put(t, 2 * (w + tid) + 1, ib);
    }
    __syncthreads();
  }
}

__device__ __forceinline__ uint32_t msm_sum(ge_p3& acc, uint32_t i, const uint32_t* __restrict__ off, const uint32_t* __restrict__ pidx,
                                            uint32_t n_points, const dev_affine* __restrict__ pts, const dev_ext* __restrict__ partial) {
  const uint32_t b = off[i], e = off[i + 1];
  ge_identity(acc);
  uint32_t bad = 0;
#pragma unroll 1
  for (uint32_t t = b; t < e; ++t) {
    ge_p3 q;
    load_ext(q, partial + t);
    ge_add_p3(acc, acc, q);
    const uint32_t pi = pidx[t];
    bad |= pi < n_points ? (pts[pi].valid ^ 1u) : 1u;
  }
  return bad;
}

__device__ __forceinline__ void encode_invert_block(enc_tree& tree, int tid, uint32_t b, uint32_t n_blocks, const uint32_t* __restrict__ bprod,
                                                    uint32_t* __restrict__ binv) {
  fe x;
  fe_1(x);
  if (b < n_blocks) {
#pragma unroll
    for (int k = 0; k < 9; ++k) x.v[k] = bprod[(size_t)b * 9 + k];
    FE_TRACK(fe_set_ub_tight(x));
  }
  tree_put(tree, ENC_BLOCK + tid, x);
  __syncthreads();
  tree_up(tree, tid);
#ifdef ZKP_AB_LANE_INVERT
  if (tid == 0) {
    fe r, inv;
    tree_get(r, tree, 1);
    fe_pin_vgpr(r);
    fe_invert(inv, r);
    tree_put(tree, 1, inv);
  }
#else
  if (tid < 64) {
    rowctx rc;
    row_init(rc);
    const uint32_t z = rc.live ? tree.node[1][rc.k] : 0u;
    const uint32_t inv = row_invert(rc, z);
    if (rc.live && rc.r == 0u) tree.node[1][rc.k] = inv;
  }
#endif
  __syncthreads();
  tree_down(tree, tid);
  if (b < n_blocks) {
#pragma unroll
    for (int k = 0; k < 9; ++k) binv[(size_t)b * 9 + k] = tree.node[ENC_BLOCK + tid][k];
  }
}
template <typename STATUS_T>
__global__ void __launch_bounds__(ENC_BLOCK, 2)
k_encode_prepare(uint32_t n_msm, const uint32_t* __restrict__ off, const uint32_t* __restrict__ pidx, uint32_t n_points,
                 const dev_affine* __restrict__ pts, const dev_ext* __restrict__ partial, uint32_t* __restrict__ states ,
                 uint32_t* __restrict__ xs , uint32_t* __restrict__ bprod , uint8_t* __restrict__ zflag,
                 STATUS_T* __restrict__ status, const msm_map map) {
  __shared__ enc_tree tree;
  const int tid = threadIdx.x;
  const uint32_t i = blockIdx.x * ENC_BLOCK + tid;
  fe x;
  fe_1(x);
  if (i < n_msm) {
    ge_p3 acc;
    const uint32_t g = msm_of_lane(map, i);
    const uint32_t bad = msm_sum(acc, g, off, pidx, n_points, pts, partial);
    status[g] = (STATUS_T)bad;
    ristretto_dc_state s;
    ristretto_dc_prepare(s, x, acc);
    const uint32_t zero = fe_iszero(x);
    zflag[i] = (uint8_t)zero;
    if (zero) fe_1(x);
    uint32_t* st = states + (size_t)i * 54;
#pragma unroll
    for (int k = 0; k < 9; ++k) {
      st[k] = s.e.v[k]; st[9 + k] = s.f.v[k]; st[18 + k] = s.g.v[k]; st[27 + k] = s.h.v[k]; st[36 + k] = s.eg.v[k]; st[45 + k] = s.fh.v[k];
      xs[(size_t)i * 9 + k] = x.v[k];
    }
  }
  tree_put(tree, ENC_BLOCK + tid, x);
  __syncthreads();
  tree_up(tree, tid);
  if (tid < 9) bprod[(size_t)blockIdx.x * 9 + tid] = tree.node[1][tid];
}

__global__ void __launch_bounds__(ENC_BLOCK)
k_encode_invert(uint32_t n_blocks, const uint32_t* __restrict__ bprod, uint32_t* __restrict__ binv) {
  __shared__ enc_tree tree;
  encode_invert_block(tree, threadIdx.x, blockIdx.x * ENC_BLOCK + threadIdx.x, n_blocks, bprod, binv);
}

__global__ void __launch_bounds__(ENC_BLOCK, 2)
// ... 229 lines not shown
  uint32_t run = start[g], t = 0;
  for (; t + 8 <= tiles; t += 8) {
    uint32_t v[8];
#pragma unroll
    for (int k = 0; k < 8; ++k) v[k] = p[(size_t)(t + k) * bins];
#pragma unroll
    for (int k = 0; k < 8; ++k) { p[(size_t)(t + k) * bins] = run; run += v[k]; }
  }
  for (; t < tiles; ++t) {
    const uint32_t c = p[(size_t)t * bins];
    p[(size_t)t * bins] = run;
    run += c;
  }
}

template <int C>
__global__ void __launch_bounds__(sort_cfg<C>::THREADS)
k_pip_tile_scatter(uint32_t n, const uint32_t* __restrict__ digits, const uint32_t* __restrict__ tilehist,
                   uint32_t* __restrict__ sorted) {
  using cfg = pip_cfg<C>;
  __shared__ uint32_t base[cfg::B1];
  const uint32_t tiles = gridDim.x, WK = gridDim.y, lin = blockIdx.x + blockIdx.y * tiles, full = (WK & ~7u) * tiles;
  uint32_t w, t;
#ifdef ZKP_AB_PLAIN_SCATTER
  if (false) {
#else
  if (lin < full) {
#endif
    const uint32_t grp = lin / (8u * tiles), r = lin - grp * 8u * tiles;
    w = grp * 8u + (r & 7u);
    t = r >> 3;
  } else {
    w = blockIdx.y;
    t = blockIdx.x;
  }
  const uint32_t* in = tilehist + ((size_t)w * tiles + t) * cfg::B1;
  for (uint32_t b = threadIdx.x; b < cfg::B1; b += blockDim.x) base[b] = in[b];
  __syncthreads();
  const uint32_t lo = t * sort_cfg<C>::TILE, hi = min(n, lo + sort_cfg<C>::TILE);
  const uint32_t* d = digits + (size_t)w * n;
  uint32_t* out = sorted + (size_t)w * n;
  for (uint32_t i = lo + threadIdx.x; i < hi; i += blockDim.x) {
    const uint32_t key = d[i], mag = key & 0x7fffffffu;
    if (mag) out[atomicAdd(&base[mag], 1u)] = i | (key & 0x80000000u);
  }
}

__global__ void __launch_bounds__(256)
k_pip_vmap(uint32_t bins, uint32_t total, uint32_t vmax, const uint32_t* __restrict__ vstart, uint32_t* __restrict__ vmap) {
  const uint32_t g = blockIdx.x * blockDim.x + threadIdx.x;
  uint32_t w = 0, b = 0, v0 = 0, v1 = 0;
  if (g < total) {
    w = g / bins; b = g - w * bins;
    const uint32_t* vs = vstart + (size_t)w * (bins + 1);
    v0 = vs[b]; v1 = vs[b + 1];
  }
  uint64_t bigmask = __ballot(v1 - v0 > 64u);
  while (bigmask) {
    const int src = __ffsll((unsigned long long)bigmask) - 1;
    bigmask &= bigmask - 1;
    const uint32_t bw = (uint32_t)__shfl((int)w, src), bb = (uint32_t)__shfl((int)b, src), b0 = (uint32_t)__shfl((int)v0, src), b1 = (uint32_t)__shfl((int)v1, src);
    for (uint32_t v = b0 + (threadIdx.x & 63u); v < b1; v += 64) vmap[(size_t)bw * vmax + v] = bb;
  }
  if (v1 - v0 <= 64u)
    for (uint32_t v = v0; v < v1; ++v) vmap[(size_t)w * vmax + v] = b;
}

__global__ void __launch_bounds__(256, 2)
k_pip_bucket_part(uint32_t n, uint32_t W1, uint32_t bins, uint32_t L, uint32_t vmax, const uint32_t* __restrict__ start,
                  const uint32_t* __restrict__ hist, const uint32_t* __restrict__ vstart, const uint32_t* __restrict__ vmap,
                  const uint32_t* __restrict__ sorted, const dev_niels* __restrict__ niels,
                  dev_ext* __restrict__ parts) {
  const uint32_t v = blockIdx.x * blockDim.x + threadIdx.x;
  const uint32_t w = blockIdx.y;
  const uint32_t* vs = vstart + (size_t)w * (bins + 1);
  if (v >= vs[bins]) return;
  const uint32_t b = vmap[(size_t)w * vmax + v], g = w * bins + b;
  const uint32_t pl = part_len(hist[g], L);
  const uint32_t first = (v - vs[b]) * pl;
  const uint32_t cnt = min(pl, hist[g] - first);
  const uint32_t* lst = sorted + (size_t)w * n + start[g] + first;
  niels += (size_t)(w / W1) * n;
  ge_p3 acc;
  ge_identity(acc);
  ge_niels qa, qb;
  uint32_t ia = 0, ib = 0;
  if (cnt) { ia = lst[0]; load_niels(qa, niels + (ia & 0x7fffffffu)); }
#pragma unroll 1
  for (uint32_t k = 0; k < cnt; k += 2) {
    if (k + 1 < cnt) { ib = lst[k + 1]; load_niels(qb, niels + (ib & 0x7fffffffu)); }
    ge_niels_cneg(qa, ia >> 31);
    ge_madd(acc, acc, qa);
    if (k + 1 < cnt) {
      if (k + 2 < cnt) { ia = lst[k + 2]; load_niels(qa, niels + (ia & 0x7fffffffu)); }
      ge_niels_cneg(qb, ib >> 31);
      ge_madd(acc, acc, qb);
    }
  }
  store_ext(parts + (size_t)w * vmax + v, acc);
}

constexpr uint32_t kMergeSeqParts = 128;
__global__ void __launch_bounds__(256, 2)
k_pip_bucket_merge(uint32_t bins, uint32_t total, uint32_t vmax, const uint32_t* __restrict__ vstart,
                   const dev_ext* __restrict__ parts, dev_ext* __restrict__ buckets) {
  __shared__ uint32_t big[64];
  __shared__ uint32_t n_big;
  __shared__ uint32_t red[64][4][9];
  const uint32_t gt = blockIdx.x * blockDim.x + threadIdx.x;
  const uint32_t g = gt >> 2, qi = threadIdx.x >> 2;
  const int q = (int)(gt & 3u);
  if (threadIdx.x == 0) n_big = 0;
  __syncthreads();
  if (g < total) {
    const uint32_t w = g / bins, b = g - w * bins;
    const uint32_t* vs = vstart + (size_t)w * (bins + 1);
    const uint32_t v0 = vs[b], v1 = vs[b + 1];
    const dev_ext* p = parts + (size_t)w * vmax;
    if (v1 - v0 > kMergeSeqParts) {
      if (q == 0) big[atomicAdd(&n_big, 1u)] = g;
    } else {
      qpt acc;
      if (v1 == v0) {
        q_identity(acc, q);
      } else {
        q_load_ext(acc, p + v0, q);
#pragma unroll 1
        for (uint32_t v = v0 + 1; v < v1; ++v) {
          qpt t;
          q_load_ext(t, p + v, q);
          q_add(acc, acc, t, q);
        }
      }
      q_store_ext(buckets + g, acc, q);
    }
  }
  __syncthreads();
  const uint32_t nb = n_big;
#pragma unroll 1
  for (uint32_t i = 0; i < nb; ++i) {
    const uint32_t gb = big[i], w = gb / bins, b = gb - w * bins;
    const uint32_t* vs = vstart + (size_t)w * (bins + 1);
    const uint32_t v0 = vs[b], v1 = vs[b + 1];
    const dev_ext* p = parts + (size_t)w * vmax;
    qpt acc;
    q_identity(acc, q);
    if (v0 + qi < v1) q_load_ext(acc, p + v0 + qi, q);
#pragma unroll 1
    for (uint32_t v = v0 + qi + 64; v < v1; v += 64) {
      qpt t;
      q_load_ext(t, p + v, q);
      q_add(acc, acc, t, q);
    }
#pragma unroll
    for (int k = 0; k < 9; ++k) red[qi][q][k] = acc.c.v[k];
    __syncthreads();
#pragma unroll 1
    for (uint32_t d = 32; d >= 1; d >>= 1) {
      if (qi < d) {
        qpt t;
#pragma unroll
        for (int k = 0; k < 9; ++k) t.c.v[k] = red[qi + d][q][k];
        q_add(acc, acc, t, q);
#pragma unroll
        for (int k = 0; k < 9; ++k) red[qi][q][k] = acc.c.v[k];
      }
      __syncthreads();
    }
    if (qi == 0) q_store_ext(buckets + gb, acc, q);
    __syncthreads();
  }
}

__device__ __forceinline__ void pip_reduce_quad(uint32_t g, int q, uint32_t n_out, uint32_t in_stride, uint32_t out_stride, int level, int m, int shift,
                                                const dev_ext* __restrict__ A_in, const dev_ext* __restrict__ R_in,
                                                dev_ext* __restrict__ A_out, dev_ext* __restrict__ R_out) {
  const uint32_t w = g / n_out, j = g - w * n_out;
  const dev_ext* rin = R_in + (size_t)w * in_stride + (size_t)m * j;
  qpt run, U, t;
  q_identity(run, q);
  q_identity(U, q);
  if (level == 0 && j == n_out - 1) {
    q_load_ext(run, rin + m, q);
    U = run;
  }
#pragma unroll 1
  for (int i = m - 1; i >= 1; --i) {
    q_load_ext(t, rin + i, q);
    q_add(run, run, t, q);
    q_add(U, U, run, q);
  }
  q_load_ext(t, rin, q);
  q_add(run, run, t, q);
#pragma unroll 1
  for (int k = 0; k < shift; ++k) q_double(U, U, q);
  if (level > 0) {
    const dev_ext* ain = A_in + (size_t)w * in_stride + (size_t)m * j;
#pragma unroll 1
    for (int i = 0; i < m; ++i) {
      q_load_ext(t, ain + i, q);
      q_add(U, U, t, q);
    }
  }
// ... 276 lines not shown
  ge_p3 p;
  fe_fromwords(p.X, w); fe_fromwords(p.Y, w + 8); fe_fromwords(p.Z, w + 16); fe_fromwords(p.T, w + 24);
  uint32_t o[8];
  ristretto_encode(o, p);
  store_vec<2>(out + 32 * (size_t)i, o);
}

__global__ void __launch_bounds__(256, 2)
k_from_uniform(uint32_t n, const uint8_t* __restrict__ in, uint8_t* __restrict__ out) {
  for (uint32_t i = blockIdx.x * blockDim.x + threadIdx.x; i < n; i += gridDim.x * blockDim.x) {
    uint32_t w[16];
    load_vec<4>(w, in + 64 * (size_t)i);
    ge_p3 p;
    ristretto_from_uniform_words(p, w);
    uint32_t o[8];
    ristretto_encode(o, p);
    store_vec<2>(out + 32 * (size_t)i, o);
  }
}

__global__ void __launch_bounds__(256)
k_sha512_csr(uint32_t n, const uint8_t* __restrict__ msgs, uint64_t msgs_len, const uint64_t* __restrict__ offsets, uint8_t* __restrict__ out) {
  for (uint32_t i = blockIdx.x * blockDim.x + threadIdx.x; i < n; i += gridDim.x * blockDim.x) {
    uint64_t H[8];
    sha512_range(H, msgs, msgs_len, offsets[i], offsets[i + 1]);
    uint32_t w[16];
    sha512_digest_words(w, H);
    store_vec<4>(out + 64 * (size_t)i, w);
  }
}

static thread_local std::string g_last_error = "";
struct zkp_ctx;
static std::mutex g_ctx_mu;
static std::set<zkp_ctx*> g_live_ctx;
static std::atomic<uint64_t> g_ctx_next_id{1};

static int fail(int code, const std::string& msg) {
  g_last_error = msg;
  return code;
}
#define HIP_TRY(expr)                                                                          \
  do {                                                                                         \
    hipError_t e_ = (expr);                                                                    \
    if (e_ != hipSuccess)                                                                      \
      return fail(e_ == hipErrorOutOfMemory ? ZKP_ERR_OOM : ZKP_ERR_HIP,                       \
                  std::string(#expr) + ": " + hipGetErrorString(e_));                          \
  } while (0)

constexpr int kMaxEvents = 32;
struct zkp_ctx {
  uint64_t uid = 0;
  int device = 0;
  hipStream_t own_stream = nullptr;
  hipStream_t stream = nullptr;
  hipStream_t side_stream = nullptr;
  hipEvent_t ev_fork = nullptr, ev_join = nullptr;
  bool prof_suspended = false;
  bool capturing = false;
  uint64_t batch_encode_min = 65536;
  bool batch_encode_user = false;
  int comb_teeth = 4;
  int ct_single_use_tables = -1;
  struct { bool offered = false, active = false; const tr_op* ops = nullptr; uint32_t n_ops = 0; const uint64_t* tables = nullptr; uint32_t N = 0; tr_bufs bufs{};
           uint8_t* ts = nullptr; uint32_t* saved = nullptr; uint32_t* failed = nullptr; uint32_t tail = 0;
           bool steps = false; tr_steps_dev sd; uint64_t* img = nullptr; } pending_tr;
  int debug_dummy_launches = 0;
  bool stmt_classify = true;
  int fuse_tables_transcript = -1;
  int tables_lane = -1;
  int comb_split = -1;
  int grouped_comb = -1;
  int ladder_interleave = -1;
  static constexpr uint32_t kInterleaveLadderBlocks = 256;
  bool each_straus = true;
  uint32_t each_straus_lanes = 0;
  uint32_t each_straus_wins = 0;
  int ct_lookup = 0;
#ifdef ZKP_BUILD_TEST_HOOKS
  uint64_t* wave_cycles = nullptr;
  static constexpr uint32_t kWaveCyclesCap = 1u << 20;
  enum { SCH_BATCH_ENCODE, SCH_ENC_GROUPS, SCH_OPT_PIP, SCH_PIP_C, SCH_PIP_PART, SCH_STATUS_SHARED, SCH_LAT_SPLIT, SCH_GROUPED, SCH_COMB_MIN,
         SCH_LADDER_INTERLEAVE, SCH_RIDERS, SCH_STRAUS_LANES, SCH_STRAUS_WINS, SCH_TR_LANES, SCH_TR_STEPS, SCH_FUSE_TT, SCH_TERMS_SPLIT,
         SCH_RAGGED_CLASSES, SCH_RAGGED_COMPILED, SCH_RAGGED_BASE, SCH_FUSED_PLANS, SCH_COUNT };
  int64_t sched[SCH_COUNT] = {-1, -1, -1, -1, -1, -1, -1, -1, -1, -1, -1, -1, -1, -1, -1, -1, -1, -1, -1, -1, -1};
#endif
  static constexpr size_t kGroupedCombTerms = 400000;
  static constexpr size_t kSplitCombTerms = 8192;
  bool dev_overlap = false;
  bool dev_latency = false;
  bool rider_tables = true;
  bool joint_ladder = true;
  bool tr_steps = true;
  int tr_lanes = -1;
  static constexpr size_t kWideCallTerms = 250000, kWideCallProofs = 8192;
  static constexpr size_t kVeryWideCallProofs = 65536;
  uint32_t ct_comb_min(bool throughput, size_t n_terms) const {
    return ct_single_use_tables < 0 ? (throughput && n_terms >= kWideCallTerms ? 2u : 1u) : (ct_single_use_tables ? 1u : 2u);
  }
  void* ws = nullptr;
  size_t ws_bytes = 0;
  uint64_t ws_generation = 0, plans_generation = 0;
  bool profiling = false;
  hipEvent_t ev[kMaxEvents] = {};
  int ev_kind[kMaxEvents] = {};
  int n_ev = 0;
  float kernel_ms[ZKP_K_COUNT] = {};
  float total_ms = 0;
  std::string kernel_names[ZKP_K_COUNT];
  dev_niels* hot_tables = nullptr;
  uint32_t* hot_reg_words = nullptr;
  int32_t* hot_reg_slot = nullptr;
  char* hot_scratch = nullptr;
  std::string hot_key[HOT_SLOTS];
  uint64_t hot_used[HOT_SLOTS] = {};
  uint64_t hot_tick = 0;
  uint32_t hot_nreg = 0;
  std::map<std::string, void*> fused_plans;
  std::map<std::string, void*> ragged_progs, ragged_bases;
  uint64_t ragged_tick = 0;
  struct job_t {
    char kind = 0;
    hipEvent_t done = nullptr;
    uint8_t* pin = nullptr;
    size_t pin_bytes = 0;
    uint32_t K = 0;
    int* verdicts = nullptr;
    int* invalid_point = nullptr;
    uint8_t* results = nullptr;
    size_t n_results = 0;
    hipError_t copy_err = hipSuccess;
    hipEvent_t tev[4] = {};
    bool timed = false;
    float ms[3] = {};
    struct out_copy { void* dst; const void* src; size_t bytes; };
    std::vector<out_copy> outs;
    hipEvent_t copied = nullptr;
    bool copies_issued = false;
    bool inline_out = false;
  } job;
  int defer_d2h = -1;
  bool sync_throughput = false;
  size_t ws_limit = 0;
  bool hot_registry_uploaded = false;
};
void free_fused_plans(zkp_ctx* c);
void free_ragged_progs(zkp_ctx* c);

namespace {

struct carve {
  size_t off = 0;
  size_t take(size_t bytes) {
    const size_t o = off;
    off += (bytes + 255) & ~(size_t)255;
    return o;
  }
};

int ensure_ws(zkp_ctx* c, size_t bytes) {
  if (c->job.kind) return fail(ZKP_ERR_ARG, "a submitted job is pending on this context: zkp_ctx_job_wait first");
  if (bytes <= c->ws_bytes) return ZKP_OK;
  if (c->ws_limit && bytes + bytes / 8 > c->ws_limit)
    return fail(ZKP_ERR_OOM, "the call needs a workspace of " + std::to_string(bytes + bytes / 8) + " bytes, ZKP_OPT_WS_LIMIT_BYTES allows " + std::to_string(c->ws_limit));
  if (c->capturing) return fail(ZKP_ERR_ARG, "graph capture: the workspace would grow -- run the same calls once before capturing them");
  if (c->ws) {
    HIP_TRY(hipStreamSynchronize(c->stream));
    HIP_TRY(hipFree(c->ws));
    c->ws = nullptr;
    c->ws_bytes = 0;
    ++c->ws_generation;
  }
  const size_t want = bytes + bytes / 8;
  HIP_TRY(hipMalloc(&c->ws, want));
  c->ws_bytes = want;
  return ZKP_OK;
}

void prof_note(zkp_ctx* c, int kind, const std::string& name) {
  if (!c->profiling || c->capturing || c->prof_suspended) return;
  std::string& s = c->kernel_names[kind];
  if ((";" + s + ";").find(";" + name + ";") == std::string::npos) s += (s.empty() ? "" : ";") + name;
}
#ifdef ZKP_BUILD_TEST_HOOKS
#define ZKP_SCHED(c, key, v) ((c)->sched[zkp_ctx::SCH_##key] = (int64_t)(v))
#else
#define ZKP_SCHED(c, key, v) ((void)0)
#endif
void prof_begin(zkp_ctx* c) {
#ifdef ZKP_BUILD_TEST_HOOKS
  for (int64_t& v : c->sched) v = -1;
#endif
  c->n_ev = 0;
  if (c->profiling && !c->capturing) for (auto& s : c->kernel_names) s.clear();
  if (c->profiling && !c->capturing) { hipEventRecord(c->ev[0], c->stream); c->ev_kind[0] = -1; c->n_ev = 1; }
}
void prof_mark(zkp_ctx* c, int kind) {
  if (c->profiling && !c->capturing && !c->prof_suspended && c->n_ev < kMaxEvents) {
    hipEventRecord(c->ev[c->n_ev], c->stream);
    c->ev_kind[c->n_ev] = kind;
    c->n_ev++;
  }
}

inline dim3 grid1(size_t n, int block) { return dim3((unsigned)((n + block - 1) / block)); }
inline bool aligned16(const void* p) { return (reinterpret_cast<uintptr_t>(p) & 15) == 0; }

struct terms_cfg {
  int teeth = 4;
  uint32_t max_tables = 0xffffffffu, max_ladder = 0xffffffffu;
  bool throughput = false;
  uint32_t comb_min = 2;
  msm_map map;
  bool prehalved = false;
  stmt_job stmt;
  bool rider_tables = false;
};
inline bool stmt_classify_applies(const terms_cfg& k, uint32_t n_terms) {
  return k.stmt.on && n_terms >= 1024 && k.stmt.T <= STMT_MAX_TERMS && k.stmt.np <= STMT_MAX_POINTS && k.stmt.T && k.stmt.N;
}
inline terms_cfg terms_cfg_clamped(terms_cfg k, uint32_t n_points, uint32_t n_terms) {
  if (k.comb_min != 1) k.comb_min = 2;
  k.max_tables = std::min(k.max_tables, std::min(n_points, n_terms / k.comb_min));
  k.max_ladder = k.comb_min == 1 ? 0u : std::min(k.max_ladder, std::min(n_points, n_terms));
  if (k.teeth != 16) k.teeth = 4;
  return k;
}
constexpr uint64_t kThroughputEncodeMin = 2048;
inline int pick_teeth(uint64_t n_tab, uint64_t tab_terms) {
  if (!n_tab || tab_terms < 2 * n_tab) return 4;
  return n_tab * comb_entries(16) * sizeof(dev_ext) <= (64ull << 30) ? 16 : 4;
}

struct terms_layout { size_t pts, part, hot, cls, list, needs, slot_of, slot_pt, gstart, gfill, comb, ladder, half, states, xs, bprod, zflag, end; };
terms_layout terms_carve(size_t start, uint32_t n_points, uint32_t n_terms, uint32_t n_msm, const terms_cfg& k) {
  carve cv;
  cv.off = start;
  terms_layout o;
  const bool split = n_terms >= 1024;
  o.pts = cv.take((size_t)n_points * sizeof(dev_affine));
  o.part = cv.take((size_t)n_terms * sizeof(dev_ext));
  o.hot = cv.take((size_t)n_points * 4);
  o.cls = cv.take(512 * 4);
  o.needs = cv.take((size_t)n_points * 4);
  o.gfill = cv.take(split ? (size_t)n_points * 4 : 0);
  o.list = cv.take((size_t)n_terms * 4);
  o.slot_of = cv.take(split ? (size_t)n_points * 4 : 0);
  o.slot_pt = cv.take(split ? (size_t)k.max_tables * 4 : 0);
  o.gstart = cv.take(split ? (size_t)n_points * 4 : 0);
  o.comb = cv.take(split ? (size_t)k.max_tables * comb_entries(k.teeth) * sizeof(dev_ext) : 0);
  o.ladder = cv.take(split ? (((size_t)k.max_ladder + 63) / 64) * (k.stmt.pair ? 2 : 1) * LADDER_GROUP_UINT4 * sizeof(uint4) : 0);
  const uint32_t enc_blocks = (n_msm + ENC_BLOCK - 1) / ENC_BLOCK;
  o.half = cv.take(split ? (size_t)n_terms * 32 : 0);
  o.states = cv.take(split ? (size_t)n_msm * 54 * 4 : 0);
  o.xs = cv.take(split ? (size_t)n_msm * 9 * 4 : 0);
  o.bprod = cv.take(split ? (size_t)enc_blocks * 9 * 4 * 2 : 0);
  o.zflag = cv.take(split ? (size_t)n_msm : 0);
  o.end = cv.off;
  return o;
}
size_t terms_path_ws(uint32_t n_points, uint32_t n_terms, uint32_t n_msm, const terms_cfg& k = terms_cfg()) {
  return terms_carve(0, n_points, n_terms, n_msm, terms_cfg_clamped(k, n_points, n_terms)).end;
}

inline bool terms_batched_encode(const zkp_ctx* c, uint32_t n_terms, uint32_t n_msm, bool throughput) {
  return n_terms >= 1024 && (uint64_t)n_msm >= ((throughput && !c->batch_encode_user) ? kThroughputEncodeMin : c->batch_encode_min);
}

template <bool CT, int TEETH, int LOOKUP>
void launch_terms_split(zkp_ctx* c, dim3 grid, bool ladder, const uint8_t* d_scalars, const uint32_t* d_pidx, uint32_t n_points, const dev_ext* comb,
                        const uint32_t* slot_of, const uint32_t* class_start, const uint32_t* blk_start, const uint32_t* list,
                        const dev_affine* pts, dev_ext* ladder_rw, uint32_t max_ladder, dev_ext* part, uint32_t comb_split, const uint32_t* pair, uint32_t stmt_T) {
  uint32_t stride = 0;
  const uint32_t lb = (max_ladder + 255) / 256;
  const bool interleave = ladder && lb && (c->ladder_interleave < 0 ? lb >= zkp_ctx::kInterleaveLadderBlocks : c->ladder_interleave != 0);
  if (ladder && lb) ZKP_SCHED(c, LADDER_INTERLEAVE, interleave);
  if (interleave) {
    stride = (grid.x / 2) / lb;
    if (stride % 2 == 0 && stride) --stride;
    if (stride < 2) stride = 0;
  }
  const bool split_kernel = CT && TEETH == 16 && LOOKUP == LOOKUP_XBAR && comb_split && !ladder;
  prof_note(c, ZKP_K_TERMS, std::string("k_terms_split<") + (CT ? "true" : "false") + ", " + std::to_string(TEETH) + ", " + (ladder ? "true" : "false") + ", " + std::to_string(LOOKUP) + ", " +
                            (split_kernel ? "true" : "false") + ">");
  if constexpr (CT && TEETH == 16 && LOOKUP == LOOKUP_XBAR) {
    if (comb_split && !ladder) {
      hipLaunchKernelGGL((k_terms_split<CT, TEETH, false, LOOKUP, true>), grid, dim3(256), 0, c->stream, d_scalars, d_pidx, n_points, comb, slot_of, class_start, blk_start, list,
                         c->hot_tables, pts, ladder_rw, max_ladder, part, stride, pair, stmt_T);
      return;
    }
  }
  if (ladder)
    hipLaunchKernelGGL((k_terms_split<CT, TEETH, true, LOOKUP>), grid, dim3(256), 0, c->stream, d_scalars, d_pidx, n_points, comb, slot_of, class_start, blk_start, list,
                       c->hot_tables, pts, ladder_rw, max_ladder, part, stride, pair, stmt_T);
  else
    hipLaunchKernelGGL((k_terms_split<CT, TEETH, false, LOOKUP>), grid, dim3(256), 0, c->stream, d_scalars, d_pidx, n_points, comb, slot_of, class_start, blk_start, list,
                       c->hot_tables, pts, ladder_rw, max_ladder, part, stride, pair, stmt_T);
}

enum : int { PH_POINTS = 1, PH_SCALARS = 2, PH_ALL = 3 };
int msm_terms_path(zkp_ctx* c, uint32_t n_msm, const uint32_t* d_off, const uint8_t* d_scalars,
                   const uint32_t* d_pidx, const uint8_t* d_points, uint32_t n_points, uint32_t n_terms, int flags,
                   uint8_t* d_out, uint8_t* d_status8, uint32_t* d_status32, size_t ws_reserved, bool decode_all = false,
                   int phase = PH_ALL, const terms_cfg& cfg_in = terms_cfg()) {
  const terms_cfg k = terms_cfg_clamped(cfg_in, n_points, n_terms);
  const terms_layout o = terms_carve(ws_reserved, n_points, n_terms, n_msm, k);
  const bool batched_encode = terms_batched_encode(c, n_terms, n_msm, k.throughput);
  const uint32_t enc_blocks = (n_msm + ENC_BLOCK - 1) / ENC_BLOCK;
  if (o.end > c->ws_bytes) return fail(ZKP_ERR_ARG, "internal: workspace too small");
  const bool terms_split = n_terms >= 1024;
  const uint32_t enc_groups = (enc_blocks + ENC_BLOCK - 1) / ENC_BLOCK;
  if (phase & PH_SCALARS) {
    ZKP_SCHED(c, TERMS_SPLIT, terms_split);
    ZKP_SCHED(c, BATCH_ENCODE, batched_encode);
    if (batched_encode) ZKP_SCHED(c, ENC_GROUPS, enc_groups);
  }
  char* base = static_cast<char*>(c->ws);
  dev_affine* pts = reinterpret_cast<dev_affine*>(base + o.pts);
  dev_ext* part = reinterpret_cast<dev_ext*>(base + o.part);
  if (terms_split) {
    int32_t* hotmap = reinterpret_cast<int32_t*>(base + o.hot);
    uint32_t* cls = reinterpret_cast<uint32_t*>(base + o.cls);
    uint32_t* class_cnt = cls, *class_start = cls + 80, *cursor = cls + 160, *any_hot = cls + 240, *n_slots = cls + 241, *blk_start = cls + 256;
    uint32_t* list = reinterpret_cast<uint32_t*>(base + o.list);
    uint32_t* needs = reinterpret_cast<uint32_t*>(base + o.needs);
    uint32_t* slot_of = reinterpret_cast<uint32_t*>(base + o.slot_of);
    uint32_t* slot_pt = reinterpret_cast<uint32_t*>(base + o.slot_pt);
    dev_ext* comb = reinterpret_cast<dev_ext*>(base + o.comb);
    dev_ext* ladder = reinterpret_cast<dev_ext*>(base + o.ladder);
    const uint32_t comb_min = k.comb_min;
    const bool lat_split = c->comb_split < 0 ? (!k.throughput && flags == ZKP_CT && k.teeth == 16 && n_terms >= zkp_ctx::kSplitCombTerms && n_terms < zkp_ctx::kGroupedCombTerms) : c->comb_split != 0;
    const bool group_on = (HOT_LDS_ROWS && c->ct_lookup == LOOKUP_SCAN) ? false
                          : c->grouped_comb < 0 ? (n_terms >= (k.throughput ? zkp_ctx::kWideCallTerms : zkp_ctx::kGroupedCombTerms) || lat_split) : c->grouped_comb != 0;
    const bool comb_split = lat_split && flags == ZKP_CT && k.teeth == 16 && !(HOT_LDS_ROWS && c->ct_lookup != LOOKUP_XBAR);
    const uint32_t group_min = (flags == ZKP_CT && k.teeth == 16 && group_on && k.max_tables) ? GROUP_MIN_USES : 0xffffffffu;
    ZKP_SCHED(c, LAT_SPLIT, lat_split);
    ZKP_SCHED(c, GROUPED, group_on);
    ZKP_SCHED(c, COMB_MIN, comb_min);
    const bool pair_on = k.stmt.pair && flags == ZKP_VARTIME && stmt_classify_applies(k, n_terms);
    if (k.stmt.pair && !pair_on) return fail(ZKP_ERR_ARG, "paired terms outside the statement classifier");
    if (pair_on && !decode_all) return fail(ZKP_ERR_ARG, "paired terms need decode_all");
    const bool rider_ok = pair_on && k.teeth == 16 && k.rider_tables;
    if (pair_on) ZKP_SCHED(c, RIDERS, rider_ok);
    uint32_t* gstart = reinterpret_cast<uint32_t*>(base + o.gstart);
    uint32_t* gfill = reinterpret_cast<uint32_t*>(base + o.gfill);
    if ((phase & PH_POINTS) && stmt_classify_applies(k, n_terms)) {
      const size_t lanes = std::max<size_t>(std::max<size_t>(n_terms, n_points), (size_t)k.stmt.N * k.stmt.nc + 1);
      hipLaunchKernelGGL(k_stmt_classify, grid1(lanes, 256), dim3(256), 0, c->stream, k.stmt, d_points, c->hot_nreg, c->hot_reg_words, c->hot_reg_slot, comb_min, group_min,
                         k.max_tables, needs, class_start, blk_start, n_slots, slot_of, slot_pt, list, rider_ok ? 1u : 0u);
      prof_mark(c, ZKP_K_SORT);
      hipLaunchKernelGGL(k_decode_affine, grid1(n_points, 256), dim3(256), 0, c->stream, n_points, d_points, pts, decode_all ? (const uint32_t*)nullptr : needs);
      prof_mark(c, ZKP_K_DECODE);
    } else if (phase & PH_POINTS) {
    HIP_TRY(hipMemsetAsync(cls, 0, o.list - o.cls, c->stream));
    if (c->hot_nreg)
      hipLaunchKernelGGL(k_hot_match, grid1(n_points, 256), dim3(256), 0, c->stream, n_points, d_points, c->hot_nreg, c->hot_reg_words, c->hot_reg_slot, hotmap, any_hot);
    else
      HIP_TRY(hipMemsetAsync(hotmap, 0xff, (size_t)n_points * 4, c->stream));
    hipLaunchKernelGGL(k_use_count, grid1(n_terms, 256), dim3(256), 0, c->stream, n_terms, d_pidx, n_points, hotmap, needs);
    hipLaunchKernelGGL(k_class_count, grid1(n_terms, 256), dim3(256), 0, c->stream, n_terms, d_pidx, n_points, hotmap, needs, comb_min, group_min, class_cnt);
    prof_mark(c, ZKP_K_SORT);
    hipLaunchKernelGGL(k_decode_affine, grid1(n_points, 256), dim3(256), 0, c->stream, n_points, d_points, pts, decode_all ? (const uint32_t*)nullptr : needs);
    prof_mark(c, ZKP_K_DECODE);
    hipLaunchKernelGGL(k_class_scan, dim3(1), dim3(64), 0, c->stream, class_cnt, class_start, cursor, blk_start);
    if (k.max_tables)
      hipLaunchKernelGGL(k_comb_slots, grid1(n_points, 256), dim3(256), 0, c->stream, n_points, needs, comb_min, group_min, k.max_tables, n_slots, slot_of, slot_pt, gstart, pts);
    hipLaunchKernelGGL(k_class_scatter, grid1(n_terms, 256), dim3(256), 0, c->stream, n_terms, d_pidx, n_points, hotmap, needs, comb_min, group_min, class_start, gstart, gfill,
                       cursor, list);
    prof_mark(c, ZKP_K_SORT);
    }
    if ((phase & PH_POINTS) && k.max_tables) {
      if (c->tables_lane < 0 ? k.throughput : c->tables_lane != 0) {
        if (k.teeth == 16 && c->pending_tr.active) {
          const auto& t = c->pending_tr;
          const uint32_t tr_blocks = (t.N + TR_BLOCK / 2 - 1) / (TR_BLOCK / 2);
          if (t.steps) {
            const uint32_t rows = t.sd.n_img * 3u + ((t.sd.n_chk || (t.sd.tail >> 31)) ? 1u : 0u);
            if (rows) hipLaunchKernelGGL(k_transcript_assemble, dim3((t.N + TA_BLOCK - 1) / TA_BLOCK, rows), dim3(TA_BLOCK), 0, c->stream, t.sd, t.N, t.bufs, t.img, t.failed);
            hipLaunchKernelGGL(k_tables_chain_pc<16>, dim3((tr_blocks + 1) / 2 + (k.max_tables + 63) / 64), dim3(2 * TR_BLOCK), 0, c->stream, tr_blocks, t.sd,
                               reinterpret_cast<const uint32_t*>(t.img), t.N, t.bufs, t.ts, t.saved, n_slots, k.max_tables, slot_pt, pts, comb);
          } else
            hipLaunchKernelGGL(k_tables_transcript_pc<16>, dim3((tr_blocks + 1) / 2 + (k.max_tables + 63) / 64), dim3(2 * TR_BLOCK), 0, c->stream, tr_blocks, t.ops, t.n_ops,
                               t.tables, t.N, t.bufs, t.ts, t.saved, t.failed, t.tail, n_slots, k.max_tables, slot_pt, pts, comb);
          c->pending_tr.active = false;
          prof_note(c, ZKP_K_TABLES, t.steps ? "zkp::k_tables_chain_pc<16>" : "zkp::k_tables_transcript_pc<16>");
        } else if (k.teeth == 16) hipLaunchKernelGGL(k_comb_tables_lane<16>, grid1(k.max_tables, 256), dim3(256), 0, c->stream, n_slots, k.max_tables, slot_pt, pts, comb);
        else hipLaunchKernelGGL(k_comb_tables_lane<4>, grid1(k.max_tables, 256), dim3(256), 0, c->stream, n_slots, k.max_tables, slot_pt, pts, comb);
      } else {
        if (k.teeth == 16) hipLaunchKernelGGL(k_comb_tables<16>, grid1((size_t)k.max_tables * 4, 256), dim3(256), 0, c->stream, n_slots, k.max_tables, slot_pt, pts, comb);
        else hipLaunchKernelGGL(k_comb_tables<4>, grid1((size_t)k.max_tables * 4, 256), dim3(256), 0, c->stream, n_slots, k.max_tables, slot_pt, pts, comb);
      }
    }
    if ((phase & PH_POINTS) && k.max_tables && rider_ok)
      hipLaunchKernelGGL(k_rider_tables, grid1(k.max_tables, 256), dim3(256), 0, c->stream, n_slots, k.max_tables, slot_pt, pts, comb);
    if ((phase & PH_POINTS) && k.max_tables && c->kernel_names[ZKP_K_TABLES].find("k_tables_transcript") == std::string::npos && c->kernel_names[ZKP_K_TABLES].find("k_tables_chain") == std::string::npos)
      prof_note(c, ZKP_K_TABLES, std::string((c->tables_lane < 0 ? k.throughput : c->tables_lane != 0) ? "zkp::k_comb_tables_lane<" : "zkp::k_comb_tables<") + (k.teeth == 16 ? "16>" : "4>"));
    if (phase & PH_POINTS) prof_mark(c, ZKP_K_TABLES);
    const dim3 grid((unsigned)((n_terms + XBAR_BLOCK_TERMS - 1) / XBAR_BLOCK_TERMS + 4 + HOT_SLOTS + (comb_split ? 3 * ((n_terms + 255) / 256) + 1 : 0)));
    if (batched_encode) {
      uint8_t* d_half = reinterpret_cast<uint8_t*>(base + o.half);
      if (!k.prehalved) {
        if (phase & PH_SCALARS) hipLaunchKernelGGL(k_halve_scalars, grid1(n_terms, 256), dim3(256), 0, c->stream, n_terms, d_scalars, d_half);
        d_scalars = d_half;
      }
    }
    if (phase & PH_SCALARS) {
      const int lookup = (!HOT_LDS_ROWS || c->ct_lookup == LOOKUP_XBAR) ? LOOKUP_XBAR : (flags == ZKP_CT ? c->ct_lookup : LOOKUP_LDS);
#define ZKP_LAUNCH_TERMS(CT_, TEETH_, LK_) launch_terms_split<CT_, TEETH_, LK_>(c, grid, k.max_ladder != 0, d_scalars, d_pidx, n_points, comb, slot_of, class_start, blk_start, list, pts, ladder, k.max_ladder, part, comb_split ? 1u : 0u, pair_on ? k.stmt.pair : (const uint32_t*)nullptr, k.stmt.T)
      if (lookup == LOOKUP_XBAR) {
        if (flags == ZKP_CT) { if (k.teeth == 16) ZKP_LAUNCH_TERMS(true, 16, LOOKUP_XBAR); else ZKP_LAUNCH_TERMS(true, 4, LOOKUP_XBAR); }
        else { if (k.teeth == 16) ZKP_LAUNCH_TERMS(false, 16, LOOKUP_XBAR); else ZKP_LAUNCH_TERMS(false, 4, LOOKUP_XBAR); }
      }
#if ZKP_HOT_W <= 6
      else if (lookup == LOOKUP_SCAN) {
        if (k.teeth == 16) ZKP_LAUNCH_TERMS(true, 16, LOOKUP_SCAN); else ZKP_LAUNCH_TERMS(true, 4, LOOKUP_SCAN);
      } else {
        if (flags == ZKP_CT) { if (k.teeth == 16) ZKP_LAUNCH_TERMS(true, 16, LOOKUP_LDS); else ZKP_LAUNCH_TERMS(true, 4, LOOKUP_LDS); }
        else { if (k.teeth == 16) ZKP_LAUNCH_TERMS(false, 16, LOOKUP_LDS); else ZKP_LAUNCH_TERMS(false, 4, LOOKUP_LDS); }
      }
#endif
#undef ZKP_LAUNCH_TERMS
    }
  } else {
    if (n_points && (phase & PH_POINTS)) hipLaunchKernelGGL(k_decode_affine, grid1(n_points, 256), dim3(256), 0, c->stream, n_points, d_points, pts, (const uint32_t*)nullptr);
    prof_mark(c, ZKP_K_DECODE);
    if (n_terms && (phase & PH_SCALARS)) hipLaunchKernelGGL(k_terms_r4, grid1(n_terms, 256), dim3(256), 0, c->stream, n_terms, d_scalars, d_pidx, n_points, pts, part);
  }
  if (!(phase & PH_SCALARS)) { HIP_TRY(hipGetLastError()); return ZKP_OK; }
  prof_mark(c, ZKP_K_TERMS);
  if (n_msm && batched_encode) {
    uint32_t* states = reinterpret_cast<uint32_t*>(base + o.states);
    uint32_t* xs = reinterpret_cast<uint32_t*>(base + o.xs);
    uint32_t* bprod = reinterpret_cast<uint32_t*>(base + o.bprod);
    uint32_t* binv = bprod + (size_t)enc_blocks * 9;
    uint8_t* zflag = reinterpret_cast<uint8_t*>(base + o.zflag);
    if (d_status8)
      hipLaunchKernelGGL(k_encode_prepare<uint8_t>, dim3(enc_blocks), dim3(ENC_BLOCK), 0, c->stream, n_msm, d_off, d_pidx, n_points, pts, part, states, xs, bprod, zflag, d_status8, k.map);
    else
      hipLaunchKernelGGL(k_encode_prepare<uint32_t>, dim3(enc_blocks), dim3(ENC_BLOCK), 0, c->stream, n_msm, d_off, d_pidx, n_points, pts, part, states, xs, bprod, zflag, d_status32, k.map);
    hipLaunchKernelGGL(k_encode_invert, dim3(enc_groups), dim3(ENC_BLOCK), 0, c->stream, enc_blocks, bprod, binv);
    hipLaunchKernelGGL(k_encode_finish, dim3(enc_blocks), dim3(ENC_BLOCK), 0, c->stream, n_msm, d_off, d_pidx, n_points, pts, part, states, xs, binv, zflag,
                       (const uint8_t*)d_status8, (const uint32_t*)d_status32, d_out, k.map);
  } else if (n_msm) {
    if (d_status8)
      hipLaunchKernelGGL(k_reduce_encode<uint8_t>, grid1(n_msm, 256), dim3(256), 0, c->stream, n_msm, d_off, d_pidx, n_points, pts, part, d_out, d_status8, k.map);
    else
      hipLaunchKernelGGL(k_reduce_encode<uint32_t>, grid1(n_msm, 256), dim3(256), 0, c->stream, n_msm, d_off, d_pidx, n_points, pts, part, d_out, d_status32, k.map);
  }
  prof_mark(c, ZKP_K_REDUCE);
  HIP_TRY(hipGetLastError());
  return ZKP_OK;
}

inline uint32_t pip_part_len(uint64_t n) { return n < (1u << 18) ? 16u : (n < (1u << 21) ? 32u : 64u); }
template <int C>
size_t pip_vmax(uint64_t n) { return (size_t)(n / pip_part_len(n)) + pip_cfg<C>::B1 + 1; }

template <int C>
uint32_t pip_tiles(uint64_t n) { return (uint32_t)((n + sort_cfg<C>::TILE - 1) / sort_cfg<C>::TILE); }

template <int C>
size_t pip_ws(uint64_t n, uint32_t K = 1) {
  using cfg = pip_cfg<C>;
  const size_t WK = (size_t)cfg::W1 * K;
  carve cv;
  cv.take((size_t)K * n * sizeof(dev_niels));
  cv.take(WK * n * 4);
  cv.take(WK * n * 4);
  cv.take(WK * cfg::B1 * 4 * 3);
  cv.take(WK * (cfg::B1 + 1) * 4);
  cv.take(WK * pip_tiles<C>(n) * cfg::B1 * 4);
  cv.take(WK * pip_vmax<C>(n) * sizeof(dev_ext));
  cv.take(WK * pip_vmax<C>(n) * 4);
  cv.take((size_t)K * 4 + 256);
  cv.take(WK * cfg::B1 * sizeof(dev_ext));
  cv.take(WK * (cfg::B + 8) * sizeof(dev_ext) * 2);
  return cv.off;
}

template <int C>
int pip_run(zkp_ctx* c, uint32_t n, const uint8_t* d_scalars, const uint8_t* d_points, uint8_t* d_out,
            uint32_t* d_status, size_t ws_reserved, uint32_t* shared_flags, const pip_seg seg = pip_seg(), int phases = 3) {
  using cfg = pip_cfg<C>;
  const uint32_t K = seg.K;
  const size_t WK = (size_t)cfg::W1 * K;
  if (WK > 65535) return fail(ZKP_ERR_ARG, "too many batches in one call");
  carve cv;
  cv.off = ws_reserved;
  char* base = static_cast<char*>(c->ws);
  dev_niels* niels = reinterpret_cast<dev_niels*>(base + cv.take((size_t)K * n * sizeof(dev_niels)));
  uint32_t* digits = reinterpret_cast<uint32_t*>(base + cv.take(WK * n * 4));
  uint32_t* sorted = reinterpret_cast<uint32_t*>(base + cv.take(WK * n * 4));
  const size_t nb = WK * cfg::B1;
  if (nb * 4 > 0xffffffffull) return fail(ZKP_ERR_ARG, "too many batches in one call");
  uint32_t* hist = reinterpret_cast<uint32_t*>(base + cv.take(nb * 4 * 3));
  uint32_t* start = hist + nb;
  uint32_t* cursor = start + nb;
  uint32_t* vstart = reinterpret_cast<uint32_t*>(base + cv.take(WK * (cfg::B1 + 1) * 4));
  const uint32_t tiles = pip_tiles<C>(n);
  uint32_t* tilehist = reinterpret_cast<uint32_t*>(base + cv.take(WK * tiles * cfg::B1 * 4));
  const uint32_t L = pip_part_len(n);
  const size_t vmax = pip_vmax<C>(n);
  ZKP_SCHED(c, PIP_C, C);
  ZKP_SCHED(c, PIP_PART, L);
  dev_ext* parts = reinterpret_cast<dev_ext*>(base + cv.take(WK * vmax * sizeof(dev_ext)));
  uint32_t* vmap = reinterpret_cast<uint32_t*>(base + cv.take(WK * vmax * 4));
  uint32_t* invalid = reinterpret_cast<uint32_t*>(base + cv.take((size_t)K * 4 + 256));
  if (shared_flags) invalid = shared_flags;
  dev_ext* buckets = reinterpret_cast<dev_ext*>(base + cv.take(nb * sizeof(dev_ext)));
  const size_t lvl_cap = WK * (cfg::B + 8);
  dev_ext* lvlA = reinterpret_cast<dev_ext*>(base + cv.take(lvl_cap * sizeof(dev_ext) * 2));
  dev_ext* lvlR = lvlA + lvl_cap;
  if (cv.off > c->ws_bytes) return fail(ZKP_ERR_ARG, "internal: workspace too small");

  if (phases == 1) {
    if (!shared_flags) return fail(ZKP_ERR_ARG, "internal: split prepare without the caller's flag words");
    hipLaunchKernelGGL((k_pip_prepare<C, 1>), dim3((n + 255) / 256, K), dim3(256), 0, c->stream, n, seg, d_scalars, d_points, niels, digits, invalid);
    HIP_TRY(hipGetLastError());
    return ZKP_OK;
  }
  if (!shared_flags) HIP_TRY(hipMemsetAsync(invalid, 0, (size_t)K * 4, c->stream));
  prof_note(c, ZKP_K_DECODE, "k_pip_prepare<" + std::to_string(C) + ">");
  if (phases == 2) hipLaunchKernelGGL((k_pip_prepare<C, 2>), dim3((n + 255) / 256, K), dim3(256), 0, c->stream, n, seg, d_scalars, d_points, niels, digits, invalid);
  else hipLaunchKernelGGL((k_pip_prepare<C, 3>), dim3((n + 255) / 256, K), dim3(256), 0, c->stream, n, seg, d_scalars, d_points, niels, digits, invalid);
  prof_mark(c, ZKP_K_DECODE);
  hipLaunchKernelGGL(k_pip_tile_hist<C>, dim3(tiles, (unsigned)WK), dim3(sort_cfg<C>::THREADS), 0, c->stream, n, digits, tilehist);
  hipLaunchKernelGGL(k_pip_tile_total, grid1(nb, 256), dim3(256), 0, c->stream, cfg::B1, tiles, (uint32_t)nb, tilehist, hist);
  hipLaunchKernelGGL(k_pip_scan, dim3((unsigned)WK), dim3(256), 0, c->stream, cfg::B1, L, hist, start, cursor, vstart);
  hipLaunchKernelGGL(k_pip_tile_base, grid1(nb, 256), dim3(256), 0, c->stream, cfg::B1, tiles, (uint32_t)nb, start, tilehist);
  hipLaunchKernelGGL(k_pip_tile_scatter<C>, dim3(tiles, (unsigned)WK), dim3(sort_cfg<C>::THREADS), 0, c->stream, n, digits, tilehist, sorted);
  prof_mark(c, ZKP_K_SORT);
  hipLaunchKernelGGL(k_pip_vmap, grid1(nb, 256), dim3(256), 0, c->stream, cfg::B1, (uint32_t)nb, (uint32_t)vmax, vstart, vmap);
  hipLaunchKernelGGL(k_pip_bucket_part, dim3((unsigned)((vmax + 255) / 256), (unsigned)WK), dim3(256), 0, c->stream, n, (uint32_t)cfg::W1, cfg::B1, L, (uint32_t)vmax,
                     start, hist, vstart, vmap, sorted, niels, parts);
  hipLaunchKernelGGL(k_pip_bucket_merge, grid1(nb * 4, 256), dim3(256), 0, c->stream, cfg::B1, (uint32_t)nb, (uint32_t)vmax, vstart, parts, buckets);
  prof_mark(c, ZKP_K_BUCKET);
  const dev_ext* Ain = nullptr;
  const dev_ext* Rin = buckets;
  uint32_t in_stride = cfg::B1, n_in = cfg::B;
  size_t lvl_off = 0;
  int level = 0;
  int shift = 0;
  static_assert(cfg::W1 <= 64, "k_pip_combine runs the last tree level with one quad per window in one 256-lane block");
  while (n_in > 1) {
    int lg = 0;
    while ((1u << lg) < n_in) ++lg;
    const int mbits = (level == 0 && lg % 3) ? lg % 3 : 3;
    const uint32_t m = 1u << mbits, n_out = n_in >> mbits;
    dev_ext* Aout = lvlA + lvl_off;
    dev_ext* Rout = lvlR + lvl_off;
    const uint32_t total = (uint32_t)WK * n_out;
    if (n_out == 1) {
      hipLaunchKernelGGL(k_pip_combine, dim3(K), dim3(256), 0, c->stream, cfg::W1, C, in_stride, level, (int)m, shift, Ain, Rin, Aout, invalid, d_out, d_status, shared_flags ? 1u : 0u);
      break;
    }
    hipLaunchKernelGGL(k_pip_reduce_lvl, grid1((size_t)total * 4, 256), dim3(256), 0, c->stream, n_out, total, in_stride, n_out, level, (int)m, shift,
                       Ain, Rin, Aout, Rout);
    Ain = Aout;
    Rin = Rout;
    in_stride = n_out;
    n_in = n_out;
    lvl_off += total;
    shift += mbits;
    ++level;
  }
  prof_mark(c, ZKP_K_COMBINE);
  HIP_TRY(hipGetLastError());
  return ZKP_OK;
}

int pick_c(uint64_t n) {
  if (n < (1u << 12)) return 7;
  if (n < (1u << 13)) return 10;
  if (n < (1u << 21)) return 11;
  return 16;
}
constexpr uint64_t kSmallOptional = 192;

terms_cfg host_terms_cfg(const zkp_ctx* c, uint32_t n_terms, const uint32_t* pidx, const uint8_t* points, uint32_t n_points, uint32_t comb_min) {
  std::vector<uint32_t> uses(n_points, 0);
  for (uint32_t t = 0; t < n_terms; ++t) ++uses[pidx[t]];
  std::vector<std::pair<uint64_t, int>> hot;
  for (int sl = 0; sl < HOT_SLOTS; ++sl)
    if (!c->hot_key[sl].empty()) { uint64_t w; memcpy(&w, c->hot_key[sl].data(), 8); hot.emplace_back(w, sl); }
  std::sort(hot.begin(), hot.end());
  std::vector<char> is_hot(n_points, 0);
  bool shared = false;
  for (uint32_t p = 0; p < n_points; ++p) {
    if (!uses[p] || hot.empty()) continue;
    uint64_t w;
    memcpy(&w, points + 32 * (size_t)p, 8);
    for (auto it = std::lower_bound(hot.begin(), hot.end(), std::make_pair(w, -1)); it != hot.end() && it->first == w; ++it)
      if (memcmp(c->hot_key[it->second].data(), points + 32 * (size_t)p, 32) == 0) { is_hot[p] = 1; break; }
  }
  for (uint32_t p = 0; p < n_points; ++p) shared |= !is_hot[p] && uses[p] >= 2;
  if (comb_min == 1 && !shared) comb_min = 2;
  uint64_t n_tab = 0, n_lad = 0, tab_terms = 0;
  for (uint32_t p = 0; p < n_points; ++p) {
    if (!uses[p] || is_hot[p]) continue;
    if (uses[p] >= comb_min) { ++n_tab; tab_terms += uses[p]; } else ++n_lad;
  }
  terms_cfg k;
  k.comb_min = comb_min;
  k.max_tables = (uint32_t)n_tab;
  k.max_ladder = (uint32_t)n_lad;
  k.teeth = pick_teeth(n_tab, tab_terms);
  return k;
}

int launch_from_uniform(zkp_ctx* c, uint64_t n, const uint8_t* d_in, uint8_t* d_out) {
  constexpr uint64_t kMaxBlocks = 2048;
  const unsigned blocks = (unsigned)std::min<uint64_t>(kMaxBlocks, (n + 255) / 256);
  hipLaunchKernelGGL(k_from_uniform, dim3(blocks), dim3(256), 0, c->stream, (uint32_t)n, d_in, d_out);
  prof_mark(c, ZKP_K_DECODE);
  HIP_TRY(hipGetLastError());
  return ZKP_OK;
}

// ... 41 lines not shown
  HIP_TRY(hipStreamSynchronize(c->stream));
  return ZKP_OK;
}

}

extern "C" {

const char* zkp_last_error(void) { return g_last_error.c_str(); }
#ifdef ZKP_BUILD_TEST_HOOKS
#define ZKP_VERSION_TEXT_(w) "zkp-mi355x 0.5 gfx950 (9x29-bit limbs, v_mad_u64_u32; " #w "-bit fixed-base windows)"
#define ZKP_VERSION_TEXT(w) ZKP_VERSION_TEXT_(w)
const char* zkp_version(void) { return ZKP_VERSION_TEXT(ZKP_HOT_W) " +test-hooks"; }
#else
#define ZKP_VERSION_TEXT_(w) "zkp-mi355x 0.5 gfx950 (9x29-bit limbs, v_mad_u64_u32; " #w "-bit fixed-base windows)"
#define ZKP_VERSION_TEXT(w) ZKP_VERSION_TEXT_(w)
const char* zkp_version(void) { return ZKP_VERSION_TEXT(ZKP_HOT_W); }
#endif

int zkp_ctx_create(zkp_ctx** out, int device_id) {
  if (!out) return fail(ZKP_ERR_ARG, "zkp_ctx_create: out is NULL");
  *out = nullptr;
  int count = 0;
  if (hipGetDeviceCount(&count) != hipSuccess || count == 0) return fail(ZKP_ERR_NO_DEVICE, "no HIP device visible");
  if (device_id < 0 || device_id >= count) return fail(ZKP_ERR_ARG, "device_id out of range");
  HIP_TRY(hipSetDevice(device_id));
  hipDeviceProp_t prop;
  HIP_TRY(hipGetDeviceProperties(&prop, device_id));
  if (std::string(prop.gcnArchName).rfind("gfx950", 0) != 0)
    return fail(ZKP_ERR_NO_DEVICE, std::string("device is ") + prop.gcnArchName + ", this library is built for gfx950 only");
  zkp_ctx* c = new zkp_ctx();
  c->uid = g_ctx_next_id.fetch_add(1);
  c->device = device_id;
  if (hipStreamCreateWithFlags(&c->own_stream, hipStreamNonBlocking) != hipSuccess) { delete c; return fail(ZKP_ERR_HIP, "hipStreamCreate failed"); }
  c->stream = c->own_stream;
  for (auto& e : c->ev)
    if (hipEventCreate(&e) != hipSuccess) { delete c; return fail(ZKP_ERR_HIP, "hipEventCreate failed"); }
  { std::lock_guard<std::mutex> lk(g_ctx_mu); g_live_ctx.insert(c); }
  *out = c;
  return ZKP_OK;
}

void zkp_ctx_destroy(zkp_ctx* c) {
  if (!c) return;
  { std::lock_guard<std::mutex> lk(g_ctx_mu); g_live_ctx.erase(c); }
  hipSetDevice(c->device);
  if (c->capturing) { hipGraph_t g = nullptr; hipStreamEndCapture(c->stream, &g); if (g) hipGraphDestroy(g); c->capturing = false; }
  hipStreamSynchronize(c->stream);
  if (c->job.done) hipEventDestroy(c->job.done);
  if (c->job.copied) hipEventDestroy(c->job.copied);
  for (auto& e : c->job.tev) if (e) hipEventDestroy(e);
  if (c->job.pin) hipHostFree(c->job.pin);
  if (c->ws) hipFree(c->ws);
  if (c->hot_tables) hipFree(c->hot_tables);
  if (c->hot_reg_words) hipFree(c->hot_reg_words);
  if (c->hot_reg_slot) hipFree(c->hot_reg_slot);
  if (c->hot_scratch) hipFree(c->hot_scratch);
#ifdef ZKP_BUILD_TEST_HOOKS
  if (c->wave_cycles) { uint64_t* z = nullptr; (void)hipMemcpyToSymbol(HIP_SYMBOL(g_wave_cycles), &z, sizeof(z)); hipFree(c->wave_cycles); }
#endif
  free_fused_plans(c);
  free_ragged_progs(c);
  if (c->side_stream) hipStreamDestroy(c->side_stream);
  if (c->ev_fork) hipEventDestroy(c->ev_fork);
  if (c->ev_join) hipEventDestroy(c->ev_join);
  for (auto& e : c->ev) if (e) hipEventDestroy(e);
  if (c->own_stream) hipStreamDestroy(c->own_stream);
  delete c;
}

int zkp_ctx_set_stream(zkp_ctx* c, void* s) {
  if (!c) return fail(ZKP_ERR_ARG, "ctx is NULL");
  c->stream = s ? static_cast<hipStream_t>(s) : c->own_stream;
  return ZKP_OK;
}
int zkp_ctx_set_option(zkp_ctx* c, int option, uint64_t value) {
  if (!c) return fail(ZKP_ERR_ARG, "ctx is NULL");
  switch (option) {
    case ZKP_OPT_BATCH_ENCODE_MIN: c->batch_encode_min = value; c->batch_encode_user = true; return ZKP_OK;
    case ZKP_OPT_CT_SINGLE_USE_TABLES: c->ct_single_use_tables = value == ~0ull ? -1 : (value ? 1 : 0); return ZKP_OK;
    case ZKP_OPT_DEV_OVERLAP: c->dev_overlap = value != 0 && value != ~0ull; c->dev_latency = value == 2; return ZKP_OK;
#ifdef ZKP_BUILD_TEST_HOOKS
    case ZKP_TESTOPT_GENERIC_CLASSIFIER: c->stmt_classify = value == 0; return ZKP_OK;
    case ZKP_TESTOPT_DUMMY_LAUNCHES: c->debug_dummy_launches = (int)std::min<uint64_t>(value, 1000); return ZKP_OK;
    case ZKP_TESTOPT_WAVE_CYCLES: {
      HIP_TRY(hipSetDevice(c->device));
      HIP_TRY(hipStreamSynchronize(c->stream));
      uint64_t* p = nullptr;
      uint32_t cap = 0;
      if (value) {
        if (!c->wave_cycles) HIP_TRY(hipMalloc(&c->wave_cycles, sizeof(uint64_t) * zkp_ctx::kWaveCyclesCap));
        HIP_TRY(hipMemset(c->wave_cycles, 0, sizeof(uint64_t) * zkp_ctx::kWaveCyclesCap));
        p = c->wave_cycles;
        cap = zkp_ctx::kWaveCyclesCap;
      }
      HIP_TRY(hipMemcpyToSymbol(HIP_SYMBOL(g_wave_cycles), &p, sizeof(p)));
      HIP_TRY(hipMemcpyToSymbol(HIP_SYMBOL(g_wave_cycles_cap), &cap, sizeof(cap)));
      return ZKP_OK;
    }
#endif
    case ZKP_OPT_FUSE_TABLES_TRANSCRIPT: c->fuse_tables_transcript = value == ~0ull ? -1 : (value ? 1 : 0); return ZKP_OK;
    case ZKP_OPT_TABLES_LANE: c->tables_lane = value == ~0ull ? -1 : (value ? 1 : 0); return ZKP_OK;
    case ZKP_OPT_GROUPED_COMB: c->grouped_comb = value == ~0ull ? -1 : (value ? 1 : 0); return ZKP_OK;
    case ZKP_OPT_JOINT_LADDER: c->joint_ladder = value != 0; c->rider_tables = value != 2; return ZKP_OK;
    case ZKP_OPT_COMB_SPLIT: c->comb_split = value == ~0ull ? -1 : (value ? 1 : 0); return ZKP_OK;
    case ZKP_OPT_CT_LOOKUP:
      if (value == ~0ull) value = 0;
      if (value > 2 || (value && !HOT_LDS_ROWS)) return fail(ZKP_ERR_ARG, "ZKP_OPT_CT_LOOKUP: 0 (lane crossbar), 1 (masked scans), 2 (LDS rows); 1 and 2 exist for 6-bit fixed-base windows only");
      c->ct_lookup = (int)value; return ZKP_OK;
    case ZKP_OPT_LADDER_INTERLEAVE: c->ladder_interleave = value == ~0ull ? -1 : value != 0; return ZKP_OK;
    case ZKP_OPT_JOB_DEFER_D2H: c->defer_d2h = value == ~0ull ? -1 : (value ? 1 : 0); return ZKP_OK;
    case ZKP_OPT_SYNC_SCHEDULE: c->sync_throughput = value != 0 && value != ~0ull; return ZKP_OK;
    case ZKP_OPT_WS_LIMIT_BYTES: c->ws_limit = value == ~0ull ? 0 : (size_t)value; return ZKP_OK;
    case ZKP_OPT_EACH_STRAUS:
    {
      const bool wins = value > 0x200 && value <= 0x200 + 64 && ((value - 0x200) & (value - 0x201)) == 0;
      if (value != ~0ull && value > 8 && !wins)
        return fail(ZKP_ERR_ARG, "ZKP_OPT_EACH_STRAUS: 0 (off), 1 .. 8 lanes per proof, 0x200 + (1, 2, 4 .. 64) window parts per proof, or UINT64_MAX (default)");
      c->each_straus = value != 0;
      c->each_straus_lanes = (value == ~0ull || value == 0 || value > 8) ? 0u : (uint32_t)value;
      c->each_straus_wins = wins ? (uint32_t)(value - 0x200) : 0u;
      return ZKP_OK;
    }
    case ZKP_OPT_TRANSCRIPT_STEPS: c->tr_steps = value != 0; return ZKP_OK;
    case ZKP_OPT_TRANSCRIPT_LANES:
      if (value != ~0ull && value != 1 && value != 2) return fail(ZKP_ERR_ARG, "ZKP_OPT_TRANSCRIPT_LANES: 1, 2 or UINT64_MAX");
      c->tr_lanes = value == ~0ull ? -1 : (int)value;
      return ZKP_OK;
    case ZKP_OPT_COMB_TEETH:
      if (value != 4 && value != 16) return fail(ZKP_ERR_ARG, "ZKP_OPT_COMB_TEETH must be 4 or 16");
      c->comb_teeth = (int)value;
      return ZKP_OK;
    default: return fail(ZKP_ERR_ARG, "unknown option");
  }
}
int zkp_ctx_synchronize(zkp_ctx* c) {
  if (!c) return fail(ZKP_ERR_ARG, "ctx is NULL");
  HIP_TRY(hipStreamSynchronize(c->stream));
  return ZKP_OK;
}
int zkp_ctx_set_profiling(zkp_ctx* c, int enabled) {
  if (!c) return fail(ZKP_ERR_ARG, "ctx is NULL");
  c->profiling = enabled != 0;
  return ZKP_OK;
}
struct zkp_graph {
  hipGraph_t graph = nullptr;
  hipGraphExec_t exec = nullptr;
  int device = 0;
  zkp_ctx* ctx = nullptr;
  uint64_t ctx_uid = 0;
  uint64_t ws_generation = 0, plans_generation = 0;
};

int zkp_ctx_capture_begin(zkp_ctx* c) {
  if (!c) return fail(ZKP_ERR_ARG, "ctx is NULL");
  if (c->capturing) return fail(ZKP_ERR_ARG, "capture already in progress");
  HIP_TRY(hipSetDevice(c->device));
  HIP_TRY(hipStreamBeginCapture(c->stream, hipStreamCaptureModeThreadLocal));
  c->capturing = true;
  return ZKP_OK;
}
int zkp_ctx_capture_end(zkp_ctx* c, zkp_graph** out) {
  if (!c || !out) return fail(ZKP_ERR_ARG, "NULL pointer");
  *out = nullptr;
  if (!c->capturing) return fail(ZKP_ERR_ARG, "no capture in progress");
// ... 324 lines not shown
  if (n == 0) return ZKP_OK;
  if (!points || !status) return fail(ZKP_ERR_ARG, "NULL pointer");
  if (n > 0x7fffffffull) return fail(ZKP_ERR_ARG, "n too large");
  HIP_TRY(hipSetDevice(c->device));
  carve cv;
  const size_t o_pts = cv.take((size_t)n * 32);
  const size_t o_st = cv.take((size_t)n);
  const size_t o_xyzt = cv.take(xyzt ? (size_t)n * 128 : 0);
  const int rc = ensure_ws(c, cv.off);
  if (rc) return rc;
  char* base = static_cast<char*>(c->ws);
  HIP_TRY(hipMemcpyAsync(base + o_pts, points, (size_t)n * 32, hipMemcpyHostToDevice, c->stream));
  prof_begin(c);
  hipLaunchKernelGGL(k_decode_check, grid1(n, 256), dim3(256), 0, c->stream, (uint32_t)n, reinterpret_cast<uint8_t*>(base + o_pts),
                     reinterpret_cast<uint8_t*>(base + o_st), xyzt ? reinterpret_cast<uint8_t*>(base + o_xyzt) : nullptr);
  prof_mark(c, ZKP_K_DECODE);
  HIP_TRY(hipGetLastError());
  HIP_TRY(hipMemcpyAsync(status, base + o_st, (size_t)n, hipMemcpyDeviceToHost, c->stream));
  if (xyzt) HIP_TRY(hipMemcpyAsync(xyzt, base + o_xyzt, (size_t)n * 128, hipMemcpyDeviceToHost, c->stream));
  HIP_TRY(hipStreamSynchronize(c->stream));
  return ZKP_OK;
}

int zkp_from_uniform_bytes_dev(zkp_ctx* c, uint64_t n, const uint8_t* d_in, uint8_t* d_out) {
  if (!c) return fail(ZKP_ERR_ARG, "ctx is NULL");
  if (n == 0) return ZKP_OK;
  if (!d_in || !d_out) return fail(ZKP_ERR_ARG, "NULL device pointer");
  if (n > 0x7fffffffull) return fail(ZKP_ERR_ARG, "n too large");
  if (!aligned16(d_in) || !aligned16(d_out)) return fail(ZKP_ERR_ARG, "device buffers must be 16-byte aligned");
  HIP_TRY(hipSetDevice(c->device));
  prof_begin(c);
  return launch_from_uniform(c, n, d_in, d_out);
}

int zkp_from_uniform_bytes(zkp_ctx* c, uint64_t n, const uint8_t* in, uint8_t* out) {
  if (!c) return fail(ZKP_ERR_ARG, "ctx is NULL");
  if (n == 0) return ZKP_OK;
  if (!in || !out) return fail(ZKP_ERR_ARG, "NULL pointer");
  if (n > 0x7fffffffull) return fail(ZKP_ERR_ARG, "n too large");
  HIP_TRY(hipSetDevice(c->device));
  carve cv;
  const size_t o_in = cv.take((size_t)n * 64);
  const size_t o_out = cv.take((size_t)n * 32);
  int rc = ensure_ws(c, cv.off);
  if (rc) return rc;
  char* base = static_cast<char*>(c->ws);
  HIP_TRY(hipMemcpyAsync(base + o_in, in, (size_t)n * 64, hipMemcpyHostToDevice, c->stream));
  prof_begin(c);
  rc = launch_from_uniform(c, n, reinterpret_cast<uint8_t*>(base + o_in), reinterpret_cast<uint8_t*>(base + o_out));
  if (rc) return rc;
  HIP_TRY(hipMemcpyAsync(out, base + o_out, (size_t)n * 32, hipMemcpyDeviceToHost, c->stream));
  HIP_TRY(hipStreamSynchronize(c->stream));
  return ZKP_OK;
}

int zkp_hash_from_bytes_sha512(zkp_ctx* c, uint64_t n, const uint8_t* msgs, const uint64_t* offsets, uint8_t* out) {
  return hash_from_bytes_host(c, n, msgs, offsets, out, true);
}

int zkp_hash_from_bytes_sha512_dev(zkp_ctx* c, uint64_t n, const uint8_t* d_msgs, uint64_t msgs_len, const uint64_t* d_offsets, uint8_t* d_out) {
  if (!c) return fail(ZKP_ERR_ARG, "ctx is NULL");
  if (n == 0) return ZKP_OK;
  if ((!d_msgs && msgs_len) || !d_offsets || !d_out) return fail(ZKP_ERR_ARG, "NULL device pointer");
  if (n > 0x7fffffffull) return fail(ZKP_ERR_ARG, "n too large");
  if ((reinterpret_cast<uintptr_t>(d_offsets) & 7) || !aligned16(d_out))
    return fail(ZKP_ERR_ARG, "d_offsets must be 8-byte and d_out 16-byte aligned");
  HIP_TRY(hipSetDevice(c->device));
  carve cv;
  const size_t o_wide = cv.take((size_t)n * 64);
  int rc = ensure_ws(c, cv.off);
  if (rc) return rc;
  uint8_t* d_wide = static_cast<uint8_t*>(c->ws) + o_wide;
  prof_begin(c);
  rc = launch_sha512(c, n, d_msgs, msgs_len, d_offsets, d_wide);
  if (rc) return rc;
  return launch_from_uniform(c, n, d_wide, d_out);
}

#ifdef ZKP_BUILD_TEST_HOOKS
int zkp_debug_last_schedule(zkp_ctx* c, char* buf, size_t cap) {
  if (!c || !buf || !cap) return fail(ZKP_ERR_ARG, "bad argument");
  static const char* const names[zkp_ctx::SCH_COUNT] = {"batch_encode", "enc_groups", "opt_pip", "pip_c", "pip_part", "status_shared", "lat_split", "grouped", "comb_min",
                                                        "ladder_interleave", "riders", "straus_lanes", "straus_wins", "tr_lanes", "tr_steps", "fuse_tt", "terms_split",
                                                        "ragged_classes", "ragged_compiled", "ragged_base", "fused_plans"};
  std::string s;
  for (int i = 0; i < zkp_ctx::SCH_COUNT; ++i)
    if (c->sched[i] >= 0) s += (s.empty() ? "" : " ") + std::string(names[i]) + "=" + std::to_string(c->sched[i]);
  const size_t n = std::min(s.size(), cap - 1);
  memcpy(buf, s.data(), n);
  buf[n] = 0;
  return (int)s.size();
}

int zkp_debug_sha512(zkp_ctx* c, uint64_t n, const uint8_t* msgs, const uint64_t* offsets, uint8_t* out) {
  return hash_from_bytes_host(c, n, msgs, offsets, out, false);
}
#endif

#ifdef ZKP_BUILD_TEST_HOOKS
int zkp_debug_quad_selftest(zkp_ctx* c, uint32_t n, const uint8_t* pairs, uint8_t* out) {
  if (!c || !pairs || !out) return fail(ZKP_ERR_ARG, "NULL pointer");
  if (n == 0) return ZKP_OK;
  HIP_TRY(hipSetDevice(c->device));
  carve cv;
  const size_t o_in = cv.take((size_t)n * 64);
  const size_t o_out = cv.take((size_t)n * 128);
  const int rc = ensure_ws(c, cv.off);
  if (rc) return rc;
  char* base = static_cast<char*>(c->ws);
  HIP_TRY(hipMemcpyAsync(base + o_in, pairs, (size_t)n * 64, hipMemcpyHostToDevice, c->stream));
  hipLaunchKernelGGL(k_debug_quad, grid1((size_t)n * 4, 256), dim3(256), 0, c->stream, n, reinterpret_cast<uint8_t*>(base + o_in), reinterpret_cast<uint8_t*>(base + o_out));
  HIP_TRY(hipGetLastError());
  HIP_TRY(hipMemcpyAsync(out, base + o_out, (size_t)n * 128, hipMemcpyDeviceToHost, c->stream));
  HIP_TRY(hipStreamSynchronize(c->stream));
  return ZKP_OK;
}
#endif

#ifdef ZKP_BUILD_TEST_HOOKS
int zkp_debug_row_selftest(zkp_ctx* c, uint32_t n, const uint8_t* pairs, uint8_t* out) {
  if (!c || !pairs || !out) return fail(ZKP_ERR_ARG, "NULL pointer");
  if (n == 0) return ZKP_OK;
  HIP_TRY(hipSetDevice(c->device));
  carve cv;
  const size_t o_in = cv.take((size_t)n * 64);
  const size_t o_out = cv.take((size_t)n * 96);
  const int rc = ensure_ws(c, cv.off);
  if (rc) return rc;
  char* base = static_cast<char*>(c->ws);
  HIP_TRY(hipMemcpyAsync(base + o_in, pairs, (size_t)n * 64, hipMemcpyHostToDevice, c->stream));
  hipLaunchKernelGGL(k_debug_row, dim3(n), dim3(64), 0, c->stream, n, reinterpret_cast<uint8_t*>(base + o_in), reinterpret_cast<uint8_t*>(base + o_out));
  HIP_TRY(hipGetLastError());
  HIP_TRY(hipMemcpyAsync(out, base + o_out, (size_t)n * 96, hipMemcpyDeviceToHost, c->stream));
  HIP_TRY(hipStreamSynchronize(c->stream));
  return ZKP_OK;
}
#endif

#ifdef ZKP_BUILD_TEST_HOOKS
int zkp_debug_wave_cycles(zkp_ctx* c, uint64_t* out, uint32_t cap) {
  if (!c || !out) return fail(ZKP_ERR_ARG, "NULL pointer");
  if (!c->wave_cycles) return fail(ZKP_ERR_ARG, "ZKP_TESTOPT_WAVE_CYCLES is off");
  HIP_TRY(hipSetDevice(c->device));
  HIP_TRY(hipStreamSynchronize(c->stream));
  const uint32_t n = std::min(cap, zkp_ctx::kWaveCyclesCap);
  HIP_TRY(hipMemcpy(out, c->wave_cycles, sizeof(uint64_t) * n, hipMemcpyDeviceToHost));
  HIP_TRY(hipMemset(c->wave_cycles, 0, sizeof(uint64_t) * zkp_ctx::kWaveCyclesCap));
  return (int)n;
}
#endif

int zkp_encode_many(zkp_ctx* c, uint64_t n, const uint8_t* xyzt, uint8_t* out) {
  if (!c) return fail(ZKP_ERR_ARG, "ctx is NULL");
  if (n == 0) return ZKP_OK;
  if (!xyzt || !out) return fail(ZKP_ERR_ARG, "NULL pointer");
  if (n > 0x7fffffffull) return fail(ZKP_ERR_ARG, "n too large");
  HIP_TRY(hipSetDevice(c->device));
  carve cv;
  const size_t o_in = cv.take((size_t)n * 128);
  const size_t o_out = cv.take((size_t)n * 32);
  const int rc = ensure_ws(c, cv.off);
  if (rc) return rc;
  char* base = static_cast<char*>(c->ws);
  HIP_TRY(hipMemcpyAsync(base + o_in, xyzt, (size_t)n * 128, hipMemcpyHostToDevice, c->stream));
  prof_begin(c);
  hipLaunchKernelGGL(k_encode_many, grid1(n, 256), dim3(256), 0, c->stream, (uint32_t)n, reinterpret_cast<uint8_t*>(base + o_in), reinterpret_cast<uint8_t*>(base + o_out));
  prof_mark(c, ZKP_K_REDUCE);
// ... 12 lines not shown
```

### zkp_amd/engine.py

```python
from __future__ import annotations

import ctypes
import os
from typing import Optional, Sequence, Tuple

import numpy as np

from . import cabi

_HERE = os.path.dirname(os.path.abspath(__file__))
LIB_PATH = os.path.join(_HERE, "libzkp_mi355x.so")
TESTHOOKS_LIB_PATH = os.path.join(_HERE, "libzkp_mi355x_testhooks.so")
ZKP_TESTOPT_DUMMY_LAUNCHES, ZKP_TESTOPT_GENERIC_CLASSIFIER, ZKP_TESTOPT_WAVE_CYCLES = 1001, 1002, 1003
ZKP_OPT_CT_LOOKUP, ZKP_OPT_EACH_STRAUS, ZKP_OPT_LADDER_INTERLEAVE = 9, 10, 11
ZKP_OPT_CT_MASKED_SCANS = ZKP_OPT_CT_LOOKUP
ZKP_CT_LOOKUP_XBAR, ZKP_CT_LOOKUP_SCAN, ZKP_CT_LOOKUP_LDS = 0, 1, 2
ZKP_OPT_WS_LIMIT_BYTES, ZKP_OPT_JOB_DEFER_D2H, ZKP_OPT_SYNC_SCHEDULE, ZKP_OPT_TRANSCRIPT_STEPS, ZKP_OPT_COMB_SPLIT, ZKP_OPT_JOINT_LADDER = 12, 13, 14, 15, 16, 17

ZKP_VARTIME = 0
ZKP_CT = 1
ZKP_OPT_BATCH_ENCODE_MIN = 1
(ZKP_OPT_COMB_TEETH, ZKP_OPT_CT_SINGLE_USE_TABLES, ZKP_OPT_TRANSCRIPT_LANES, ZKP_OPT_DEV_OVERLAP, ZKP_OPT_GROUPED_COMB, ZKP_OPT_TABLES_LANE,
 ZKP_OPT_FUSE_TABLES_TRANSCRIPT) = 2, 3, 4, 5, 6, 7, 8
K_NAMES = ("decode", "terms", "reduce", "sort", "bucket", "combine", "transcript", "scalars", "tables")

EXPORTS = tuple(cabi.signatures("zkp_mi355x.h"))
TEST_HOOK_EXPORTS = tuple(cabi.signatures("zkp_mi355x.h", test_hooks=True))


class ZkpError(RuntimeError):
    pass


_lib = None
_hooks_lib = None


def load_library(test_hooks: bool = False) -> ctypes.CDLL:
    global _lib, _hooks_lib
    if test_hooks and _hooks_lib is not None:
        return _hooks_lib
    if not test_hooks and _lib is not None:
        return _lib
    path = TESTHOOKS_LIB_PATH if test_hooks else LIB_PATH
    if not os.path.exists(path):
        raise ZkpError(f"{path} is missing: run `python -c 'import __graft_entry__ as g; g.build()'` "
                       "(hipcc --offload-arch=gfx950); there is no CPU fallback")
    lib = cabi.bind(ctypes.CDLL(path), "zkp_mi355x.h", test_hooks)
    if test_hooks:
        _hooks_lib = lib
    else:
        _lib = lib
    return lib


def _check(rc: int, what: str) -> None:
    if rc != 0:
        raise ZkpError(f"{what} failed with code {rc}: {load_library().zkp_last_error().decode()}")


def _u8(a, shape_last: int) -> np.ndarray:
    if len(a) == 0:
        return np.zeros((0, shape_last), np.uint8)
    a = np.ascontiguousarray(a, dtype=np.uint8)
    if a.ndim != 2 or a.shape[1] != shape_last:
        raise ValueError(f"expected uint8 array of shape [n][{shape_last}], got {a.shape}")
    return a


def _ptr(a: Optional[np.ndarray]):
    return None if a is None else a.ctypes.data_as(ctypes.c_void_p)


def messages_csr(messages) -> Tuple[np.ndarray, np.ndarray]:
    msgs = [bytes(m) for m in messages]
    offsets = np.zeros(len(msgs) + 1, np.uint64)
    offsets[1:] = np.cumsum([len(m) for m in msgs], dtype=np.uint64)
    data = np.frombuffer(b"".join(msgs) or b"\0", np.uint8).copy()
    return data, offsets


def ragged_blocks(transcripts) -> Tuple[np.ndarray, np.ndarray]:
    lib = load_library(test_hooks=True)
    ts = _u8(transcripts, 208)
    idx = np.zeros(len(ts), np.uint32)
    cap = len(ts) + 1
    blocks = np.zeros((cap, 3), np.uint32)
    n = lib.zkp_debug_ragged_blocks(_ptr(ts), len(ts), _ptr(idx), _ptr(blocks), cap)
    if n < 0:
        _check(n, "zkp_debug_ragged_blocks")
    return idx, blocks[:n]


def _csr_args(data, offsets) -> Tuple[np.ndarray, np.ndarray]:
    data = np.ascontiguousarray(data, dtype=np.uint8).reshape(-1)
    offsets = np.ascontiguousarray(offsets, dtype=np.uint64).reshape(-1)
# ... 381 lines not shown
```

Before: 4.361 million.

## Seed accumulators from first point, skip carry term for canonical scalars, lane-merge PIP buckets

The first addition into an identity accumulator is replaced by a direct conversion from cached or Niels form, using a new 1/d constant, across the comb, ladder, Straus, hot-table, bucket and reduce paths. Scalars in the fused flow are marked canonical so the CT terms kernels can skip the final top-carry table add. A lane-per-bucket variant of the PIP bucket merge is added and selected for large bucket counts. Each trick removes one point addition per accumulation chain, but it relies on the canonical-scalar assumption holding and on the no-identity conversion being correct for every table entry.

After: 4.424 million (median of 6 runs). 1.01x the previous value.

```diff
diff --git a/include/zkp_mi355x.h b/include/zkp_mi355x.h
--- a/include/zkp_mi355x.h
+++ b/include/zkp_mi355x.h
@@ -199,7 +199,7 @@
 int zkp_debug_sha512(zkp_ctx* ctx, uint64_t n, const uint8_t* msgs, const uint64_t* offsets , uint8_t* out );
 int zkp_debug_last_schedule(zkp_ctx* ctx, char* buf, size_t cap);
 int zkp_debug_ragged_blocks(const uint8_t* transcripts, uint32_t N, uint32_t* idx, uint32_t* blocks, uint32_t cap);
-enum { ZKP_TESTOPT_DUMMY_LAUNCHES = 1001, ZKP_TESTOPT_GENERIC_CLASSIFIER = 1002, ZKP_TESTOPT_WAVE_CYCLES = 1003 };
+enum { ZKP_TESTOPT_DUMMY_LAUNCHES = 1001, ZKP_TESTOPT_GENERIC_CLASSIFIER = 1002, ZKP_TESTOPT_WAVE_CYCLES = 1003, ZKP_TESTOPT_PIP_MERGE = 1004 };
 #endif
 
 #ifdef __cplusplus
diff --git a/zkp_amd/csrc/comb_tables.h b/zkp_amd/csrc/comb_tables.h
--- a/zkp_amd/csrc/comb_tables.h
+++ b/zkp_amd/csrc/comb_tables.h
@@ -257,7 +257,7 @@
 
 template <bool CT, int TEETH>
 __device__ __forceinline__ void term_comb(uint32_t t, const uint8_t* __restrict__ scalars, const dev_ext* __restrict__ tbl,
-                                          dev_ext* __restrict__ partial, uint32_t* ecol) {
+                                          dev_ext* __restrict__ partial, uint32_t* ecol, bool no_carry = false) {
   using cfg = comb_cfg<TEETH>;
   uint32_t s[8], e[8], top;
   load_vec<2>(s, scalars + 32 * (size_t)t);
@@ -298,7 +298,8 @@
         load_comb_entry(n0, next + 0);
         load_comb_entry(n1, next + 1);
         ge_cached_cneg(sel, neg);
-        ge_add_cached(acc, acc, sel);
+        if (w == cfg::WINDOWS - 1 && j == 0) ge_from_cached(acc, sel);
+        else ge_add_cached(acc, acc, sel);
       }
     }
   } else {
@@ -316,11 +317,12 @@
         ge_cached sel;
         comb_select<false>(sel, tbl + 8 * j, mag);
         ge_cached_cneg(sel, neg);
-        ge_add_cached(acc, acc, sel);
-      }
-    }
-  }
-  {
+        if (w == cfg::WINDOWS - 1 && j == 0) ge_from_cached(acc, sel);
+        else ge_add_cached(acc, acc, sel);
+      }
+    }
+  }
+  if (!no_carry) {
     ge_cached sel, c;
     ge_cached_identity(sel);
     load_comb_entry(c, tbl + 8 * TEETH);
@@ -336,7 +338,7 @@
 }
 template <int TEETH>
 __device__ __forceinline__ void term_comb_split4(uint32_t t, uint32_t q, const uint8_t* __restrict__ scalars, const dev_ext* __restrict__ comb, uint32_t slot,
-                                                 dev_ext* __restrict__ partial, uint32_t* ecol) {
+                                                 dev_ext* __restrict__ partial, uint32_t* ecol, bool no_carry = false) {
   using cfg = comb_cfg<TEETH>;
   static_assert(cfg::WINDOWS == 4, "one lane of the quad per window");
   typedef __attribute__((address_space(3))) volatile uint32_t lds_word;
@@ -379,7 +381,8 @@
       load_comb_entry(n0, next + 0);
       load_comb_entry(n1, next + 1);
       ge_cached_cneg(sel, neg);
-      ge_add_cached(acc, acc, sel);
+      if (j == 0) ge_from_cached(acc, sel);
+      else ge_add_cached(acc, acc, sel);
     }
   }
   {
@@ -401,7 +404,7 @@
     ge_add_cached(d, acc, c);
     fe_pick(acc.X, d.X, q == 0u); fe_pick(acc.Y, d.Y, q == 0u); fe_pick(acc.Z, d.Z, q == 0u); fe_pick(acc.T, d.T, q == 0u);
   }
-  {
+  if (!no_carry) {
     ge_cached sel, c;
     ge_cached_identity(sel);
     load_comb_entry(c, comb + (size_t)stash[0] * cfg::ENTRIES + 8 * TEETH);
@@ -520,17 +523,20 @@
       asm volatile("s_waitcnt vmcnt(0)\n\ts_barrier" ::: "memory");
       ge_cached sel;
       uint32_t neg = 0;
+      const bool first = pass == 0 && j == 0;
       if (live) {
         pick(alo, ahi, sel, neg);
         ge_cached_cneg(sel, neg);
-        ge_add_cached(acc, acc, sel);
+        if (first) ge_from_cached(acc, sel);
+        else ge_add_cached(acc, acc, sel);
         pick(blo, bhi, sel, neg);
       }
       lds_barrier();
       if (pass == 0 || j != 15) issue((uint32_t)((j + 1) & 15));
       if (live) {
         ge_cached_cneg(sel, neg);
-        ge_add_cached(lo, lo, sel);
+        if (first) ge_from_cached(lo, sel);
+        else ge_add_cached(lo, lo, sel);
       }
     }
   }
@@ -561,7 +567,7 @@
 
 __device__ __forceinline__ void comb_group_xbar(uint32_t i0, uint32_t n_g, const uint32_t* __restrict__ list_g, const uint8_t* __restrict__ scalars,
                                                 const uint32_t* __restrict__ pidx, const uint32_t* __restrict__ slot_of,
-                                                const dev_ext* __restrict__ comb, dev_ext* __restrict__ partial, uint4* lds) {
+                                                const dev_ext* __restrict__ comb, dev_ext* __restrict__ partial, uint4* lds, bool no_carry = false) {
   using cfg = comb_cfg<16>;
   constexpr uint32_t NONE = 0xffffffffu;
   const uint32_t tid = threadIdx.x, lane = tid & 63u;
@@ -659,14 +665,17 @@
       asm volatile("s_waitcnt vmcnt(0)" ::: "memory");
       ge_cached sel;
       uint32_t neg = 0;
+      const bool first = pass == 0 && j == 0;
       pick(alo, ahi, sel, neg);
       ge_cached_cneg(sel, neg);
-      ge_add_cached(acc, acc, sel);
+      if (first) ge_from_cached(acc, sel);
+      else ge_add_cached(acc, acc, sel);
       pick(blo, bhi, sel, neg);
       asm volatile("s_waitcnt lgkmcnt(0)" ::: "memory");
       if (pass == 0 || j != 15) issue((uint32_t)((j + 1) & 15));
       ge_cached_cneg(sel, neg);
-      ge_add_cached(lo, lo, sel);
+      if (first) ge_from_cached(lo, sel);
+      else ge_add_cached(lo, lo, sel);
     }
   }
   ge_double4(acc);
@@ -676,14 +685,14 @@
     ge_to_cached(c, lo);
     ge_add_cached(acc, acc, c);
   }
-  if (live) {
+  if (live && !no_carry) {
     ge_cached sel, c;
     ge_cached_identity(sel);
     load_comb_entry(c, comb + (size_t)slot * cfg::ENTRIES + 8 * 16);
     ge_cached_cmov(sel, c, top);
     ge_add_cached(acc, acc, sel);
-    store_ext(partial + t, acc);
-  }
+  }
+  if (live) store_ext(partial + t, acc);
 }
 
 constexpr uint32_t LADDER_GROUP_UINT4 = 64u * LADDER_ENTRIES * 9u;
@@ -721,7 +730,8 @@
 
 template <bool CT>
 __device__ __forceinline__ void term_ladder16(uint32_t t, const uint8_t* __restrict__ scalars, const dev_affine* __restrict__ pt,
-                                              uint4* __restrict__ tbl , dev_ext* __restrict__ partial, uint32_t* ecol) {
+                                              uint4* __restrict__ tbl , dev_ext* __restrict__ partial, uint32_t* ecol,
+                                              bool no_carry = false) {
   uint32_t s[8], e[8], top;
   load_vec<2>(s, scalars + 32 * (size_t)t);
   sc_add_pattern(e, top, s, 0x88888888u);
@@ -748,11 +758,13 @@
     ge_to_cached(c, m); ladder_store_entry(tbl, 6, c);
     ge_double<true>(m, m4);
     ge_to_cached(c, m); ladder_store_entry(tbl, 7, c);
-    ge_cached sel;
-    ge_cached_identity(sel);
-    ge_cached_cmov(sel, c1, top);
     ge_identity(acc);
-    ge_add_cached(acc, acc, sel);
+    if (!no_carry) {
+      ge_cached sel;
+      ge_cached_identity(sel);
+      ge_cached_cmov(sel, c1, top);
+      ge_from_cached(acc, sel);
+    }
   }
 #pragma unroll 1
   for (int j = 7; j >= 0; --j) {
diff --git a/zkp_amd/csrc/fe_constants.h b/zkp_amd/csrc/fe_constants.h
--- a/zkp_amd/csrc/fe_constants.h
+++ b/zkp_amd/csrc/fe_constants.h
@@ -3,6 +3,7 @@
 namespace zkp {
 static constexpr fe_const FE_D = {{0x135978a3u, 0x0f5a6e50u, 0x10762addu, 0x00149a82u, 0x1e898007u, 0x003cbbbcu, 0x19ce331du, 0x1dc56dffu, 0x0052036cu}};
 static constexpr fe_const FE_D2 = {{0x06b2f159u, 0x1eb4dca1u, 0x00ec55bau, 0x00293505u, 0x1d13000eu, 0x00797779u, 0x139c663au, 0x1b8adbffu, 0x002406d9u}};
+static constexpr fe_const FE_D_INV = {{0x0dc9f843u, 0x0f0793b6u, 0x1e550b89u, 0x1bad3084u, 0x1cf660b5u, 0x108a66dcu, 0x190cac58u, 0x1a429ab9u, 0x0040907eu}};
 static constexpr fe_const FE_SQRT_M1 = {{0x0a0ea0b0u, 0x0770d93au, 0x0bf91e31u, 0x06300d5au, 0x1d7a72f4u, 0x004c9efdu, 0x1c2cad34u, 0x1009f83bu, 0x002b8324u}};
 static constexpr fe_const FE_INVSQRT_A_MINUS_D = {{0x005d40eau, 0x0e47ed54u, 0x105cafa6u, 0x1e2c2eb4u, 0x1d8409d2u, 0x1dc8ff00u, 0x12885b09u, 0x00b9f5ffu, 0x00786c89u}};
 static constexpr fe_const FE_SQRT_AD_MINUS_ONE = {{0x097b2e1bu, 0x14bfb502u, 0x1e152f5fu, 0x1b1c1836u, 0x1d1fdaf9u, 0x1e6498fau, 0x02b03cf3u, 0x17e57069u, 0x00376931u}};
diff --git a/zkp_amd/csrc/fused_flows.h b/zkp_amd/csrc/fused_flows.h
--- a/zkp_amd/csrc/fused_flows.h
+++ b/zkp_amd/csrc/fused_flows.h
@@ -310,7 +310,8 @@
       ge_cached q;
       load_straus_entry(q, table_of(i));
       ge_cached_cneg(q, flip);
-      ge_add_cached(acc, acc, q);
+      if (started) ge_add_cached(acc, acc, q);
+      else ge_from_cached(acc, q);
       started = true;
     }
   }
@@ -339,7 +340,8 @@
         if (i + L < K) fetch(i + L, o + 1, k);
         if (mag) {
           ge_cached_cneg(q, neg);
-          ge_add_cached(acc, acc, q);
+          if (started) ge_add_cached(acc, acc, q);
+          else ge_from_cached(acc, q);
           started = true;
         }
       }
@@ -384,7 +386,8 @@
       ge_cached q;
       load_straus_entry(q, table_of(i));
       ge_cached_cneg(q, f & 1u);
-      ge_add_cached(acc, acc, q);
+      if (started) ge_add_cached(acc, acc, q);
+      else ge_from_cached(acc, q);
       started = true;
     }
   }
@@ -412,7 +415,8 @@
       if (i + 1 < K) fetch(i + 1, k);
       if (mag) {
         ge_cached_cneg(q, neg);
-        ge_add_cached(acc, acc, q);
+        if (started) ge_add_cached(acc, acc, q);
+        else ge_from_cached(acc, q);
         started = true;
       }
     }
@@ -1047,6 +1051,7 @@
   prof_mark(c, ZKP_K_TRANSCRIPT);
 
   tk.prehalved = nc && terms_batched_encode(c, N * T, N * nc, tk.throughput);
+  tk.canonical = true;
   if (m && std::max(m, T) <= 256) {
     const uint32_t P = 256 / std::max(m, T);
     hipLaunchKernelGGL(k_blind_scalars, dim3((N + P - 1) / P), dim3(256), 0, c->stream, N, T, m, P, pl.d_tarr + nc + 1, w.u8(o.wide), w.u8(o.blind), w.u8(o.sc),
diff --git a/zkp_amd/csrc/ge25519.h b/zkp_amd/csrc/ge25519.h
--- a/zkp_amd/csrc/ge25519.h
+++ b/zkp_amd/csrc/ge25519.h
@@ -125,6 +125,53 @@
   fe_mul(r.Y, g, h);
   fe_mul(r.Z, f, g);
   fe_mul(r.T, e, h);
+}
+
+ZKP_HD void ge_from_niels(ge_p3& r, const ge_niels& q) {
+  fe t, dinv;
+  fe_sub(t, q.ypx, q.ymx);
+  fe_carry(r.X, t);
+  fe_add(t, q.ypx, q.ymx);
+  fe_carry(r.Y, t);
+  fe_0(r.Z);
+  r.Z.v[0] = 2;
+  FE_TRACK(fe_set_ub_exact(r.Z));
+  fe_from_const(dinv, FE_D_INV);
+  fe_mul(r.T, q.xy2d, dinv);
+}
+ZKP_HD void ge_from_niels_neg(ge_p3& r, const ge_niels& q) {
+  fe t, dinv;
+  fe_sub(t, q.ymx, q.ypx);
+  fe_carry(r.X, t);
+  fe_add(t, q.ypx, q.ymx);
+  fe_carry(r.Y, t);
+  fe_0(r.Z);
+  r.Z.v[0] = 2;
+  FE_TRACK(fe_set_ub_exact(r.Z));
+  fe_from_const(dinv, FE_D_INV);
+  fe_neg(t, q.xy2d);
+  fe_mul(r.T, t, dinv);
+}
+ZKP_HD void ge_from_cached(ge_p3& r, const ge_cached& q) {
+  fe t, dinv;
+  fe_sub(t, q.YpX, q.YmX);
+  fe_carry(r.X, t);
+  fe_add(t, q.YpX, q.YmX);
+  fe_carry(r.Y, t);
+  r.Z = q.Z2;
+  fe_from_const(dinv, FE_D_INV);
+  fe_mul(r.T, q.T2d, dinv);
+}
+ZKP_HD void ge_from_cached_neg(ge_p3& r, const ge_cached& q) {
+  fe t, dinv;
+  fe_sub(t, q.YmX, q.YpX);
+  fe_carry(r.X, t);
+  fe_add(t, q.YpX, q.YmX);
+  fe_carry(r.Y, t);
+  r.Z = q.Z2;
+  fe_from_const(dinv, FE_D_INV);
+  fe_neg(t, q.T2d);
+  fe_mul(r.T, t, dinv);
 }
 
 template <bool WITH_T = true>
diff --git a/zkp_amd/csrc/hot_tables.h b/zkp_amd/csrc/hot_tables.h
--- a/zkp_amd/csrc/hot_tables.h
+++ b/zkp_amd/csrc/hot_tables.h
@@ -413,7 +413,8 @@
       ge_niels q;
       fe_set(q.ypx, wd); fe_set(q.ymx, wd + 9); fe_set(q.xy2d, wd + 18);
       ge_niels_cneg(q, neg);
-      ge_madd(acc, acc, q);
+      if (w == 0) ge_from_niels(acc, q);
+      else ge_madd(acc, acc, q);
     }
   }
 }
@@ -477,8 +478,9 @@
     ge_niels q;
     fe_set(q.ypx, wd); fe_set(q.ymx, wd + 9); fe_set(q.xy2d, wd + 18);
     ge_niels_cneg(q, neg);
-    ge_madd(acc, acc, q);
-  }
-}
-
-}
+    if (w == 0) ge_from_niels(acc, q);
+    else ge_madd(acc, acc, q);
+  }
+}
+
+}
diff --git a/zkp_amd/csrc/zkp_kernels.hip b/zkp_amd/csrc/zkp_kernels.hip
--- a/zkp_amd/csrc/zkp_kernels.hip
+++ b/zkp_amd/csrc/zkp_kernels.hip
@@ -124,7 +124,7 @@
               const dev_ext* __restrict__ comb, const uint32_t* __restrict__ slot_of, const uint32_t* __restrict__ class_start,
               const uint32_t* __restrict__ blk_start, const uint32_t* __restrict__ list, const dev_niels* __restrict__ tables,
               const dev_affine* __restrict__ pts, dev_ext* __restrict__ ladder_rw, uint32_t max_ladder, dev_ext* __restrict__ partial,
-              uint32_t ladder_stride, const uint32_t* __restrict__ pair, uint32_t stmt_T) {
+              uint32_t ladder_stride, const uint32_t* __restrict__ pair, uint32_t stmt_T, uint32_t no_carry) {
   static_assert(LOOKUP == LOOKUP_XBAR || HOT_LDS_ROWS, "7-bit fixed-base windows exist on the crossbar only");
   __shared__ uint4 hot_lds[terms_lds_uint4<LOOKUP>()];
   uint32_t* ecol = reinterpret_cast<uint32_t*>(hot_lds) + threadIdx.x;
@@ -162,7 +162,7 @@
             joint = true;
           }
         }
-        if (!joint) term_ladder16<CT>(t, scalars, pts + pi, tbl, partial, ecol);
+        if (!joint) term_ladder16<CT>(t, scalars, pts + pi, tbl, partial, ecol, CT && no_carry);
       }
     }
     ZKP_WAVE_T1(1);
@@ -176,7 +176,7 @@
           const uint32_t pi = pidx[t];
           if (pi < n_points) {
             const uint32_t slot = slot_of[pi];
-            if (slot != 0xffffffffu) term_comb_split4<TEETH>(t, i & 3u, scalars, comb, slot, partial, ecol);
+            if (slot != 0xffffffffu) term_comb_split4<TEETH>(t, i & 3u, scalars, comb, slot, partial, ecol, CT && no_carry);
           }
         }
         ZKP_WAVE_T1(2);
@@ -188,14 +188,14 @@
       const uint32_t pi = pidx[t];
       if (pi < n_points) {
         const uint32_t slot = slot_of[pi];
-        if (slot != 0xffffffffu) term_comb<CT, TEETH>(t, scalars, comb + (size_t)slot * comb_cfg<TEETH>::ENTRIES, partial, ecol);
+        if (slot != 0xffffffffu) term_comb<CT, TEETH>(t, scalars, comb + (size_t)slot * comb_cfg<TEETH>::ENTRIES, partial, ecol, CT && no_carry);
       }
     }
     ZKP_WAVE_T1(2);
   } else if (vb < ladder_blocks + comb_blocks + group_blocks) {
     if constexpr (CT && TEETH == 16) {
       if constexpr (LOOKUP == LOOKUP_XBAR)
-        comb_group_xbar((vb - ladder_blocks - comb_blocks) * XBAR_BLOCK_TERMS, n_group, list + class_start[CLASS_GROUP], scalars, pidx, slot_of, comb, partial, hot_lds);
+        comb_group_xbar((vb - ladder_blocks - comb_blocks) * XBAR_BLOCK_TERMS, n_group, list + class_start[CLASS_GROUP], scalars, pidx, slot_of, comb, partial, hot_lds, no_carry != 0);
       else
         comb_group_block((vb - ladder_blocks - comb_blocks) * 256u, n_group, list + class_start[CLASS_GROUP], scalars, pidx, slot_of, comb, partial, hot_lds);
     }
@@ -253,11 +253,14 @@
   ge_p3 acc;
   ge_identity(acc);
   uint32_t bad = 0;
+  if (b < e) load_ext(acc, partial + b);
 #pragma unroll 1
   for (uint32_t t = b; t < e; ++t) {
-    ge_p3 q;
-    load_ext(q, partial + t);
-    ge_add_p3(acc, acc, q);
+    if (t != b) {
+      ge_p3 q;
+      load_ext(q, partial + t);
+      ge_add_p3(acc, acc, q);
+    }
     const uint32_t pi = pidx[t];
     bad |= pi < n_points ? (pts[pi].valid ^ 1u) : 1u;
   }
@@ -325,11 +328,14 @@
   const uint32_t b = off[i], e = off[i + 1];
   ge_identity(acc);
   uint32_t bad = 0;
+  if (b < e) load_ext(acc, partial + b);
 #pragma unroll 1
   for (uint32_t t = b; t < e; ++t) {
-    ge_p3 q;
-    load_ext(q, partial + t);
-    ge_add_p3(acc, acc, q);
+    if (t != b) {
+      ge_p3 q;
+      load_ext(q, partial + t);
+      ge_add_p3(acc, acc, q);
+    }
     const uint32_t pi = pidx[t];
     bad |= pi < n_points ? (pts[pi].valid ^ 1u) : 1u;
   }
@@ -725,34 +731,37 @@
   const uint32_t* lst = sorted + (size_t)w * n + start[g] + first;
   niels += (size_t)(w / W1) * n;
   ge_p3 acc;
-  ge_identity(acc);
   ge_niels qa, qb;
-  uint32_t ia = 0, ib = 0;
-  if (cnt) { ia = lst[0]; load_niels(qa, niels + (ia & 0x7fffffffu)); }
+  uint32_t ia = lst[0], ib = 0;
+  load_niels(qa, niels + (ia & 0x7fffffffu));
+  if (1 < cnt) { ib = lst[1]; load_niels(qb, niels + (ib & 0x7fffffffu)); }
+  ge_niels_cneg(qa, ia >> 31);
+  ge_from_niels(acc, qa);
 #pragma unroll 1
-  for (uint32_t k = 0; k < cnt; k += 2) {
-    if (k + 1 < cnt) { ib = lst[k + 1]; load_niels(qb, niels + (ib & 0x7fffffffu)); }
-    ge_niels_cneg(qa, ia >> 31);
-    ge_madd(acc, acc, qa);
+  for (uint32_t k = 1; k < cnt; k += 2) {
+    if (k + 1 < cnt) { ia = lst[k + 1]; load_niels(qa, niels + (ia & 0x7fffffffu)); }
+    ge_niels_cneg(qb, ib >> 31);
+    ge_madd(acc, acc, qb);
     if (k + 1 < cnt) {
-      if (k + 2 < cnt) { ia = lst[k + 2]; load_niels(qa, niels + (ia & 0x7fffffffu)); }
-      ge_niels_cneg(qb, ib >> 31);
-      ge_madd(acc, acc, qb);
+      if (k + 2 < cnt) { ib = lst[k + 2]; load_niels(qb, niels + (ib & 0x7fffffffu)); }
+      ge_niels_cneg(qa, ia >> 31);
+      ge_madd(acc, acc, qa);
     }
   }
   store_ext(parts + (size_t)w * vmax + v, acc);
 }
 
 constexpr uint32_t kMergeSeqParts = 128;
+template <bool LANE>
 __global__ void __launch_bounds__(256, 2)
 k_pip_bucket_merge(uint32_t bins, uint32_t total, uint32_t vmax, const uint32_t* __restrict__ vstart,
                    const dev_ext* __restrict__ parts, dev_ext* __restrict__ buckets) {
-  __shared__ uint32_t big[64];
+  __shared__ uint32_t big[LANE ? 256 : 64];
   __shared__ uint32_t n_big;
   __shared__ uint32_t red[64][4][9];
   const uint32_t gt = blockIdx.x * blockDim.x + threadIdx.x;
-  const uint32_t g = gt >> 2, qi = threadIdx.x >> 2;
-  const int q = (int)(gt & 3u);
+  const uint32_t g = LANE ? gt : gt >> 2, qi = threadIdx.x >> 2;
+  const int q = (int)(threadIdx.x & 3u);
   if (threadIdx.x == 0) n_big = 0;
   __syncthreads();
   if (g < total) {
@@ -761,7 +770,24 @@
     const uint32_t v0 = vs[b], v1 = vs[b + 1];
     const dev_ext* p = parts + (size_t)w * vmax;
     if (v1 - v0 > kMergeSeqParts) {
-      if (q == 0) big[atomicAdd(&n_big, 1u)] = g;
+      if (LANE || q == 0) big[atomicAdd(&n_big, 1u)] = g;
+    } else if constexpr (LANE) {
+      ge_p3 acc;
+      if (v1 == v0) {
+        ge_identity(acc);
+      } else {
+        load_ext(acc, p + v0);
+        ge_p3 nx = acc;
+        if (v0 + 1 < v1) load_ext(nx, p + v0 + 1);
+#pragma unroll 1
+        for (uint32_t v = v0 + 1; v < v1; ++v) {
+          ge_cached c;
+          ge_to_cached(c, nx);
+          if (v + 1 < v1) load_ext(nx, p + v + 1);
+          ge_add_cached(acc, acc, c);
+        }
+      }
+      store_ext(buckets + g, acc);
     } else {
       qpt acc;
       if (v1 == v0) {
@@ -1204,8 +1230,9 @@
   static constexpr uint32_t kWaveCyclesCap = 1u << 20;
   enum { SCH_BATCH_ENCODE, SCH_ENC_GROUPS, SCH_OPT_PIP, SCH_PIP_C, SCH_PIP_PART, SCH_STATUS_SHARED, SCH_LAT_SPLIT, SCH_GROUPED, SCH_COMB_MIN,
          SCH_LADDER_INTERLEAVE, SCH_RIDERS, SCH_STRAUS_LANES, SCH_STRAUS_WINS, SCH_TR_LANES, SCH_TR_STEPS, SCH_FUSE_TT, SCH_TERMS_SPLIT,
-         SCH_RAGGED_CLASSES, SCH_RAGGED_COMPILED, SCH_RAGGED_BASE, SCH_FUSED_PLANS, SCH_COUNT };
-  int64_t sched[SCH_COUNT] = {-1, -1, -1, -1, -1, -1, -1, -1, -1, -1, -1, -1, -1, -1, -1, -1, -1, -1, -1, -1, -1};
+         SCH_RAGGED_CLASSES, SCH_RAGGED_COMPILED, SCH_RAGGED_BASE, SCH_FUSED_PLANS, SCH_PIP_MERGE, SCH_PIP_BUCKETS, SCH_NO_CARRY, SCH_COUNT };
+  int64_t sched[SCH_COUNT] = {-1, -1, -1, -1, -1, -1, -1, -1, -1, -1, -1, -1, -1, -1, -1, -1, -1, -1, -1, -1, -1, -1, -1, -1};
+  int debug_pip_merge = 0;
 #endif
   static constexpr size_t kGroupedCombTerms = 400000;
   static constexpr size_t kSplitCombTerms = 8192;
@@ -1336,6 +1363,7 @@
   msm_map map;
   bool prehalved = false;
   stmt_job stmt;
+  bool canonical = false;
   bool rider_tables = false;
 };
 inline bool stmt_classify_applies(const terms_cfg& k, uint32_t n_terms) {
@@ -1392,7 +1420,8 @@
 template <bool CT, int TEETH, int LOOKUP>
 void launch_terms_split(zkp_ctx* c, dim3 grid, bool ladder, const uint8_t* d_scalars, const uint32_t* d_pidx, uint32_t n_points, const dev_ext* comb,
                         const uint32_t* slot_of, const uint32_t* class_start, const uint32_t* blk_start, const uint32_t* list,
-                        const dev_affine* pts, dev_ext* ladder_rw, uint32_t max_ladder, dev_ext* part, uint32_t comb_split, const uint32_t* pair, uint32_t stmt_T) {
+                        const dev_affine* pts, dev_ext* ladder_rw, uint32_t max_ladder, dev_ext* part, uint32_t comb_split, const uint32_t* pair, uint32_t stmt_T,
+                        uint32_t no_carry) {
   uint32_t stride = 0;
   const uint32_t lb = (max_ladder + 255) / 256;
   const bool interleave = ladder && lb && (c->ladder_interleave < 0 ? lb >= zkp_ctx::kInterleaveLadderBlocks : c->ladder_interleave != 0);
@@ -1408,16 +1437,16 @@
   if constexpr (CT && TEETH == 16 && LOOKUP == LOOKUP_XBAR) {
     if (comb_split && !ladder) {
       hipLaunchKernelGGL((k_terms_split<CT, TEETH, false, LOOKUP, true>), grid, dim3(256), 0, c->stream, d_scalars, d_pidx, n_points, comb, slot_of, class_start, blk_start, list,
-                         c->hot_tables, pts, ladder_rw, max_ladder, part, stride, pair, stmt_T);
+                         c->hot_tables, pts, ladder_rw, max_ladder, part, stride, pair, stmt_T, no_carry);
       return;
     }
   }
   if (ladder)
     hipLaunchKernelGGL((k_terms_split<CT, TEETH, true, LOOKUP>), grid, dim3(256), 0, c->stream, d_scalars, d_pidx, n_points, comb, slot_of, class_start, blk_start, list,
-                       c->hot_tables, pts, ladder_rw, max_ladder, part, stride, pair, stmt_T);
+                       c->hot_tables, pts, ladder_rw, max_ladder, part, stride, pair, stmt_T, no_carry);
   else
     hipLaunchKernelGGL((k_terms_split<CT, TEETH, false, LOOKUP>), grid, dim3(256), 0, c->stream, d_scalars, d_pidx, n_points, comb, slot_of, class_start, blk_start, list,
-                       c->hot_tables, pts, ladder_rw, max_ladder, part, stride, pair, stmt_T);
+                       c->hot_tables, pts, ladder_rw, max_ladder, part, stride, pair, stmt_T, no_carry);
 }
 
 enum : int { PH_POINTS = 1, PH_SCALARS = 2, PH_ALL = 3 };
@@ -1527,8 +1556,10 @@
       }
     }
     if (phase & PH_SCALARS) {
+      const uint32_t no_carry = (k.canonical && flags == ZKP_CT) ? 1u : 0u;
+      ZKP_SCHED(c, NO_CARRY, no_carry);
       const int lookup = (!HOT_LDS_ROWS || c->ct_lookup == LOOKUP_XBAR) ? LOOKUP_XBAR : (flags == ZKP_CT ? c->ct_lookup : LOOKUP_LDS);
-#define ZKP_LAUNCH_TERMS(CT_, TEETH_, LK_) launch_terms_split<CT_, TEETH_, LK_>(c, grid, k.max_ladder != 0, d_scalars, d_pidx, n_points, comb, slot_of, class_start, blk_start, list, pts, ladder, k.max_ladder, part, comb_split ? 1u : 0u, pair_on ? k.stmt.pair : (const uint32_t*)nullptr, k.stmt.T)
+#define ZKP_LAUNCH_TERMS(CT_, TEETH_, LK_) launch_terms_split<CT_, TEETH_, LK_>(c, grid, k.max_ladder != 0, d_scalars, d_pidx, n_points, comb, slot_of, class_start, blk_start, list, pts, ladder, k.max_ladder, part, comb_split ? 1u : 0u, pair_on ? k.stmt.pair : (const uint32_t*)nullptr, k.stmt.T, no_carry)
       if (lookup == LOOKUP_XBAR) {
         if (flags == ZKP_CT) { if (k.teeth == 16) ZKP_LAUNCH_TERMS(true, 16, LOOKUP_XBAR); else ZKP_LAUNCH_TERMS(true, 4, LOOKUP_XBAR); }
         else { if (k.teeth == 16) ZKP_LAUNCH_TERMS(false, 16, LOOKUP_XBAR); else ZKP_LAUNCH_TERMS(false, 4, LOOKUP_XBAR); }
@@ -1655,7 +1686,16 @@
   hipLaunchKernelGGL(k_pip_vmap, grid1(nb, 256), dim3(256), 0, c->stream, cfg::B1, (uint32_t)nb, (uint32_t)vmax, vstart, vmap);
   hipLaunchKernelGGL(k_pip_bucket_part, dim3((unsigned)((vmax + 255) / 256), (unsigned)WK), dim3(256), 0, c->stream, n, (uint32_t)cfg::W1, cfg::B1, L, (uint32_t)vmax,
                      start, hist, vstart, vmap, sorted, niels, parts);
-  hipLaunchKernelGGL(k_pip_bucket_merge, grid1(nb * 4, 256), dim3(256), 0, c->stream, cfg::B1, (uint32_t)nb, (uint32_t)vmax, vstart, parts, buckets);
+  constexpr size_t MERGE_LANE_MIN_BUCKETS = (size_t)1 << 19;
+#ifdef ZKP_BUILD_TEST_HOOKS
+  const bool lane_merge = c->debug_pip_merge ? c->debug_pip_merge == 2 : nb >= MERGE_LANE_MIN_BUCKETS;
+#else
+  const bool lane_merge = nb >= MERGE_LANE_MIN_BUCKETS;
+#endif
+  ZKP_SCHED(c, PIP_MERGE, lane_merge ? 1 : 0);
+  ZKP_SCHED(c, PIP_BUCKETS, nb);
+  if (lane_merge) hipLaunchKernelGGL(k_pip_bucket_merge<true>, grid1(nb, 256), dim3(256), 0, c->stream, cfg::B1, (uint32_t)nb, (uint32_t)vmax, vstart, parts, buckets);
+  else hipLaunchKernelGGL(k_pip_bucket_merge<false>, grid1(nb * 4, 256), dim3(256), 0, c->stream, cfg::B1, (uint32_t)nb, (uint32_t)vmax, vstart, parts, buckets);
   prof_mark(c, ZKP_K_BUCKET);
   const dev_ext* Ain = nullptr;
   const dev_ext* Rin = buckets;
@@ -1863,6 +1903,7 @@
     case ZKP_OPT_DEV_OVERLAP: c->dev_overlap = value != 0 && value != ~0ull; c->dev_latency = value == 2; return ZKP_OK;
 #ifdef ZKP_BUILD_TEST_HOOKS
     case ZKP_TESTOPT_GENERIC_CLASSIFIER: c->stmt_classify = value == 0; return ZKP_OK;
+    case ZKP_TESTOPT_PIP_MERGE: c->debug_pip_merge = value <= 2 ? (int)value : 0; return ZKP_OK;
     case ZKP_TESTOPT_DUMMY_LAUNCHES: c->debug_dummy_launches = (int)std::min<uint64_t>(value, 1000); return ZKP_OK;
     case ZKP_TESTOPT_WAVE_CYCLES: {
       HIP_TRY(hipSetDevice(c->device));
@@ -2353,7 +2394,7 @@
   if (!c || !buf || !cap) return fail(ZKP_ERR_ARG, "bad argument");
   static const char* const names[zkp_ctx::SCH_COUNT] = {"batch_encode", "enc_groups", "opt_pip", "pip_c", "pip_part", "status_shared", "lat_split", "grouped", "comb_min",
                                                         "ladder_interleave", "riders", "straus_lanes", "straus_wins", "tr_lanes", "tr_steps", "fuse_tt", "terms_split",
-                                                        "ragged_classes", "ragged_compiled", "ragged_base", "fused_plans"};
+                                                        "ragged_classes", "ragged_compiled", "ragged_base", "fused_plans", "pip_merge", "pip_buckets", "no_carry"};
   std::string s;
   for (int i = 0; i < zkp_ctx::SCH_COUNT; ++i)
     if (c->sched[i] >= 0) s += (s.empty() ? "" : " ") + std::string(names[i]) + "=" + std::to_string(c->sched[i]);
diff --git a/zkp_amd/engine.py b/zkp_amd/engine.py
--- a/zkp_amd/engine.py
+++ b/zkp_amd/engine.py
@@ -11,7 +11,7 @@
 _HERE = os.path.dirname(os.path.abspath(__file__))
 LIB_PATH = os.path.join(_HERE, "libzkp_mi355x.so")
 TESTHOOKS_LIB_PATH = os.path.join(_HERE, "libzkp_mi355x_testhooks.so")
-ZKP_TESTOPT_DUMMY_LAUNCHES, ZKP_TESTOPT_GENERIC_CLASSIFIER, ZKP_TESTOPT_WAVE_CYCLES = 1001, 1002, 1003
+ZKP_TESTOPT_DUMMY_LAUNCHES, ZKP_TESTOPT_GENERIC_CLASSIFIER, ZKP_TESTOPT_WAVE_CYCLES, ZKP_TESTOPT_PIP_MERGE = 1001, 1002, 1003, 1004
 ZKP_OPT_CT_LOOKUP, ZKP_OPT_EACH_STRAUS, ZKP_OPT_LADDER_INTERLEAVE = 9, 10, 11
 ZKP_OPT_CT_MASKED_SCANS = ZKP_OPT_CT_LOOKUP
 ZKP_CT_LOOKUP_XBAR, ZKP_CT_LOOKUP_SCAN, ZKP_CT_LOOKUP_LDS = 0, 1, 2
```
